# ferdean/lsa-fw

Hardware: AMD Instinct MI355X
Metric: converged eigenpairs/sec (k=20, shift-invert) (higher is better)
Workload: dtype c128

## Files before the change

include/lsa_hip.h:

```cpp
#ifndef LSA_HIP_H
#define LSA_HIP_H

#include <stdint.h>

#ifdef __cplusplus
extern "C" {
#endif

typedef enum { LSA_F64 = 0, LSA_C128 = 1 } lsa_dtype;

typedef enum {
    LSA_OK = 0,
    LSA_ERR_ARG = -1,
    LSA_ERR_HIP = -2,
    LSA_ERR_ZERO_PIVOT = -3,
    LSA_ERR_DIVERGED = -4,
    LSA_ERR_NONFINITE = -5,
    LSA_ERR_TIMEOUT = -6,
    LSA_ERR_COMM = -7,
    LSA_ERR_OOM = -8
} lsa_status;

typedef struct lsa_ctx lsa_ctx;
typedef struct lsa_mat lsa_mat;
typedef struct lsa_vec lsa_vec;
typedef struct lsa_ilu lsa_ilu;
typedef struct lsa_op lsa_op;
typedef struct lsa_krylov lsa_krylov;

typedef struct {
    int64_t op_applies;
    int64_t gmres_iters;
    int64_t spmv_calls;
    int64_t sptrsv_calls;
    double last_rel_res;
    double max_rel_res;
    double seconds_factor;
    double seconds_solve;
    int32_t stagnated_solves;
    int32_t pc_fallback;
    int32_t backward_accepted;
    int32_t analysis_reused;
    int32_t refined_solves;
    int32_t reserved0;
} lsa_stats;

int lsa_ctx_create(int device, lsa_ctx **out);
void lsa_ctx_destroy(lsa_ctx *ctx);
const char *lsa_last_error(const lsa_ctx *ctx);
int lsa_ctx_synchronize(lsa_ctx *ctx);
int lsa_ctx_mem_info(lsa_ctx *ctx, int64_t *free_bytes, int64_t *total_bytes);
const char *lsa_ctx_arch(const lsa_ctx *ctx);

int lsa_vec_create(lsa_ctx *ctx, int64_t n, int dtype, lsa_vec **out);
void lsa_vec_destroy(lsa_vec *v);
int lsa_vec_upload(lsa_ctx *ctx, lsa_vec *v, const void *host);
int lsa_vec_download(lsa_ctx *ctx, const lsa_vec *v, void *host);

int lsa_csr_upload(lsa_ctx *ctx, int32_t n, int64_t nnz, const int32_t *rowptr, const int32_t *col,
                   const void *val, int dtype, lsa_mat **out);
void lsa_mat_destroy(lsa_mat *m);
int lsa_mat_download_values(lsa_ctx *ctx, const lsa_mat *m, void *host_val);
int lsa_csr_axpby(lsa_ctx *ctx, const lsa_mat *A, const lsa_mat *B, const double alpha[2], const double beta[2],
                  int out_dtype, lsa_mat **out);
int lsa_csr_window(lsa_ctx *ctx, const lsa_mat *M, const double *left, const double *right, lsa_mat **out);
int lsa_spmv(lsa_ctx *ctx, const lsa_mat *A, const lsa_vec *x, lsa_vec *y);
int lsa_spmv_transpose(lsa_ctx *ctx, const lsa_mat *A, int conj, const lsa_vec *x, lsa_vec *y);
int lsa_spmv_transpose_batch(lsa_ctx *ctx, int32_t J, const lsa_mat *const *A, int conj, const lsa_vec *const *x, lsa_vec *const *y);
int lsa_spmv_info(lsa_ctx *ctx, const lsa_mat *A, int xdtype, char *kernel, int32_t kernel_len, int64_t *bytes_moved);
int lsa_spmv_time(lsa_ctx *ctx, const lsa_mat *A, const lsa_vec *x, lsa_vec *y, int iters, double *avg_ms);

int lsa_ilu_create(lsa_ctx *ctx, const lsa_mat *C, int levels, double shift_tol, lsa_ilu **out);
void lsa_ilu_destroy(lsa_ilu *pc);
int lsa_ilu_set_algorithm(lsa_ctx *ctx, lsa_ilu *pc, int algo, int32_t block_size);
int lsa_ilu_solve(lsa_ctx *ctx, lsa_ilu *pc, int which, const lsa_vec *b, lsa_vec *x);
int lsa_ilu_solve_time(lsa_ctx *ctx, lsa_ilu *pc, int which, const lsa_vec *b, lsa_vec *x, int iters, double *avg_ms);
int lsa_ilu_info(const lsa_ilu *pc, int64_t *nnz, int32_t *levels_lower, int32_t *levels_upper, int32_t *nshift);
int lsa_ilu_download(lsa_ctx *ctx, const lsa_ilu *pc, int32_t *rowptr, int32_t *col, void *val);

typedef struct lsa_nd_sym lsa_nd_sym;
typedef struct lsa_ndlu lsa_ndlu;
int lsa_nd_analyse(int32_t n, const int32_t *rowptr, const int32_t *col, int32_t leaf_size, const int8_t *constraint, lsa_nd_sym **out);
int lsa_nd_order(int32_t n, const int32_t *rowptr, const int32_t *col, int32_t leaf_size, const int8_t *constraint, lsa_nd_sym **out);
int lsa_nd_analyse_tree(int32_t n, const int32_t *rowptr, const int32_t *col, int32_t ntree, const int32_t *first, const int32_t *size,
                        const int32_t *parent, const int32_t *owner, int32_t rank, int32_t nranks, lsa_nd_sym **out);
const char *lsa_nd_sym_error(const lsa_nd_sym *h);
void lsa_nd_sym_destroy(lsa_nd_sym *h);
int lsa_nd_sym_info(const lsa_nd_sym *h, int32_t *ntree, int32_t *nlevels, int32_t *max_front, int64_t *index_entries,
                    int64_t *factor_entries, int64_t *front_entries, double *flops);
int lsa_nd_sym_memory(const lsa_nd_sym *h, int32_t scalar_bytes, int64_t work_budget_bytes, int64_t *out, int64_t *upd_off, int64_t *work_off,
                      int32_t *chunk_of);
int lsa_nd_sym_export(const lsa_nd_sym *h, int32_t *perm, int32_t *node_start, int32_t *parent, int32_t *level, int32_t *front_size,
                      int32_t *idx);
int lsa_nd_sym_export_tables(const lsa_nd_sym *h, int32_t *cmap, int32_t *gptr, int32_t *gidx, int64_t *asm_dst, int32_t *lvl_ptr,
                             int32_t *lvl_nodes);
int lsa_nd_sym_export_dist(const lsa_nd_sym *h, int32_t *kind, int64_t *front_off, int64_t *u_off, int32_t *asm_src, int32_t *children_ptr,
                           int32_t *children_idx, int64_t *scalars);
int lsa_nd_sym_export_top(const lsa_nd_sym *h, int32_t *owner, int32_t *rows, int64_t *exch, int64_t *totals);
int lsa_ndlu_create(lsa_ctx *ctx, const lsa_mat *C, int32_t leaf_size, lsa_ndlu **out);
int lsa_ndlu_prepare(lsa_ctx *ctx, const lsa_mat *P, int dtype, int32_t leaf_size, const int8_t *constraint);
int lsa_ndlu_prepare_tree(lsa_ctx *ctx, const lsa_mat *P, int dtype, int32_t ntree, const int32_t *first, const int32_t *size,
                          const int32_t *parent);
int lsa_ndlu_create_tree(lsa_ctx *ctx, const lsa_mat *C, int32_t ntree, const int32_t *first, const int32_t *size, const int32_t *parent,
                         const int32_t *owner, lsa_ndlu **out);
int lsa_ndlu_refactor(lsa_ctx *ctx, lsa_ndlu *f, const lsa_mat *C);
void lsa_ndlu_destroy(lsa_ndlu *f);
int lsa_ndlu_solve(lsa_ctx *ctx, lsa_ndlu *f, const lsa_vec *b, lsa_vec *x);
int lsa_ndlu_solve_batch(lsa_ctx *ctx, int32_t J, lsa_ndlu *const *f, const lsa_vec *const *b, lsa_vec *const *x);
int lsa_ndlu_solve_adjoint(lsa_ctx *ctx, lsa_ndlu *f, int conj, const lsa_vec *b, lsa_vec *x);
int lsa_ndlu_solve_batch_adjoint(lsa_ctx *ctx, int32_t J, lsa_ndlu *const *f, int conj, const lsa_vec *const *b, lsa_vec *const *x);
int lsa_ndlu_solve_time(lsa_ctx *ctx, lsa_ndlu *f, const lsa_vec *b, lsa_vec *x, int iters, double *avg_ms);
int lsa_ndlu_solve_multi(lsa_ctx *ctx, lsa_ndlu *f, int trans, int32_t nrhs, const lsa_vec *B, int64_t ldb, lsa_vec *X, int64_t ldx);
int lsa_ndlu_solve_multi_time(lsa_ctx *ctx, lsa_ndlu *f, int trans, int32_t nrhs, const lsa_vec *B, int64_t ldb, lsa_vec *X, int64_t ldx,
                              int iters, double *avg_ms);
int lsa_ndlu_set_multi_transposed(lsa_ctx *ctx, lsa_ndlu *f, int on);
int lsa_ndlu_multi_info(const lsa_ndlu *f, int32_t *width, int64_t *extra_bytes, int32_t *launches_per_pass);
int lsa_ndlu_solve_multi_batch(lsa_ctx *ctx, int32_t J, lsa_ndlu *const *f, int trans, int32_t nrhs, const lsa_vec *const *B, int64_t ldb,
                               lsa_vec *const *X, int64_t ldx);
int lsa_ndlu_solve_multi_batch_time(lsa_ctx *ctx, int32_t J, lsa_ndlu *const *f, int trans, int32_t nrhs, const lsa_vec *const *B,
                                    int64_t ldb, lsa_vec *const *X, int64_t ldx, int iters, double *avg_ms);
int lsa_ndlu_solve_multi_batch_adjoint(lsa_ctx *ctx, int32_t J, lsa_ndlu *const *f, int conj, int32_t nrhs, const lsa_vec *const *B,
                                       int64_t ldb, lsa_vec *const *X, int64_t ldx);
int lsa_ndlu_solve_multi_batch_adjoint_time(lsa_ctx *ctx, int32_t J, lsa_ndlu *const *f, int conj, int32_t nrhs, const lsa_vec *const *B,
                                            int64_t ldb, lsa_vec *const *X, int64_t ldx, int iters, double *avg_ms);
int lsa_ndlu_inertia(lsa_ctx *ctx, lsa_ndlu *f, int64_t *negative, int64_t *zero, int64_t *positive);
int lsa_ndlu_prepared_memory(lsa_ctx *ctx, int64_t *out);
int lsa_ndlu_info(const lsa_ndlu *f, int32_t *ntree, int32_t *nlevels, int32_t *max_front, int64_t *factor_entries,
                  int64_t *front_entries, int64_t *apply_bytes, int32_t *apply_launches, double *seconds_analyse,
                  double *seconds_numeric, int32_t *factor_launches);
int lsa_ndlu_sweep_level(const lsa_ndlu *f, int32_t level, int32_t *nodes, int32_t *max_pivot, int32_t *fwd_rows, int32_t *bwd_rows,
                         int32_t *fwd_tiles, int32_t *bwd_tiles);

int lsa_gmres(lsa_ctx *ctx, const lsa_mat *C, lsa_ilu *pc, const lsa_vec *b, lsa_vec *x, int use_x0, double rtol,
              int restart, int maxit, int32_t *iters, double *rel_res);

typedef struct {
    int32_t ilu_levels;
    double ilu_shift;
    double ksp_rtol;
    int32_t ksp_restart;
    int32_t ksp_maxit;
    int32_t pc_type;
    double antishift[2];
} lsa_op_options;

int lsa_op_create(lsa_ctx *ctx, const lsa_mat *A, const lsa_mat *M, const double sigma[2], int mode,
                  const lsa_op_options *opts, lsa_op **out);
void lsa_op_destroy(lsa_op *op);
int lsa_op_apply(lsa_ctx *ctx, lsa_op *op, const lsa_vec *x, lsa_vec *y);
int lsa_op_stats(const lsa_op *op, lsa_stats *out);
int lsa_op_set_adjoint(lsa_ctx *ctx, lsa_op *op, int on);
int lsa_op_set_projection(lsa_ctx *ctx, lsa_op *op, const double *keep);

int lsa_krylov_create(lsa_ctx *ctx, lsa_op *op, int32_t ncv, lsa_krylov **out);
void lsa_krylov_destroy(lsa_krylov *k);
int lsa_krylov_set_row_permutation(lsa_ctx *ctx, lsa_krylov *k, const int32_t *perm);
int lsa_krylov_set_start(lsa_ctx *ctx, lsa_krylov *k, const void *host_v);
int lsa_krylov_inject(lsa_ctx *ctx, lsa_krylov *k, int32_t j, const void *host_v);
int lsa_krylov_extend(lsa_ctx *ctx, lsa_krylov *k, int32_t j0, int32_t j1, void *H, int32_t ldh, int32_t *breakdown);
int lsa_krylov_restart(lsa_ctx *ctx, lsa_krylov *k, int32_t m, int32_t knew, const void *Q, int32_t ldq);
int lsa_krylov_ritz_vectors(lsa_ctx *ctx, lsa_krylov *k, int32_t m, int32_t nvec, const void *Y, int32_t ldy,
                            int normalise, void *X);
int lsa_krylov_imag_norms(const lsa_krylov *k, int32_t nvec, double *out);
int lsa_eig_residuals(lsa_ctx *ctx, const lsa_mat *A, const lsa_mat *M, int32_t nvec, const void *lam, const void *X,
                      double *res);
int lsa_eig_biorth(lsa_ctx *ctx, const lsa_mat *M, int64_t n, int32_t nvec, const void *X, const void *Z, void *G,
                   double *norm_z, double *norm_mx);

typedef enum {
    LSA_WHICH_LARGEST_MAGNITUDE = 1,
    LSA_WHICH_LARGEST_REAL = 3,
    LSA_WHICH_SMALLEST_REAL = 4,
    LSA_WHICH_LARGEST_IMAGINARY = 5,
    LSA_WHICH_SMALLEST_IMAGINARY = 6,
    LSA_WHICH_TARGET_MAGNITUDE = 7,
    LSA_WHICH_TARGET_REAL = 8,
    LSA_WHICH_TARGET_IMAGINARY = 9
} lsa_which;
typedef struct {
    int32_t nev;
    int32_t max_restarts;
    double tol;
    int32_t which;
    int32_t transform;
    double sigma[2];
    double antishift[2];
    double target[2];
    uint64_t seed;
    double keep_fraction;
} lsa_ks_options;
typedef struct {
    int32_t nconv;
    int32_t nout;
    int32_t restarts;
    int32_t pad;
    int64_t op_applies;
    double next_unconverged;
    double seconds_expand;
    double seconds_dense;
    double seconds_restart;
} lsa_ks_result;
int lsa_krylov_shape(const lsa_krylov *k, int64_t *n, int32_t *ncv);
int64_t lsa_mat_rows(const lsa_mat *m);
int lsa_krylov_solve(lsa_ctx *ctx, lsa_krylov *k, const lsa_ks_options *opts, const void *v0, const double *mask, int32_t max_out,
                     void *theta_out, void *lambda_out, void *X_out, double *est_out, lsa_ks_result *result);
typedef struct {
    int64_t rounds;
    int64_t launches;
    int64_t periods;
    double launches_per_round;
    int64_t lockstep_steps[16];
    int64_t solo_steps[16];
// ... 171 lines not shown
```

lsa-fw_amd/csrc/blas.hip:

```cpp
#include "lsa_internal.h"

namespace {

constexpr int kThreads = 256;
constexpr int kColTile = 8;

template <typename T>
__device__ __forceinline__ T wave_sum(T v);
template <>
__device__ __forceinline__ double wave_sum<double>(double v) {
#pragma unroll
    for (int m = 32; m > 0; m >>= 1) v += __shfl_xor(v, m, 64);
    return v;
}
template <>
__device__ __forceinline__ cplx wave_sum<cplx>(cplx v) {
#pragma unroll
    for (int m = 32; m > 0; m >>= 1) {
        v.re += __shfl_xor(v.re, m, 64);
        v.im += __shfl_xor(v.im, m, 64);
    }
    return v;
}

// ... 354 lines not shown
    }
    T a1, a2, a3;
    if constexpr (sizeof(T) == 16) {
        a1 = cplx{__shfl(acc.re, (lane & 15) + 16), __shfl(acc.im, (lane & 15) + 16)};
        a2 = cplx{__shfl(acc.re, (lane & 15) + 32), __shfl(acc.im, (lane & 15) + 32)};
        a3 = cplx{__shfl(acc.re, (lane & 15) + 48), __shfl(acc.im, (lane & 15) + 48)};
    } else {
        a1 = __shfl(acc, (lane & 15) + 16);
        a2 = __shfl(acc, (lane & 15) + 32);
        a3 = __shfl(acc, (lane & 15) + 48);
    }
    double nrm = 0.0;
    if (q == 0 && i < n) {
        const T tot = s_add(s_add(acc, a1), s_add(a2, a3));
        const T r = s_sub(w_in[i], tot);
        w[i] = r;
        nrm = s_abs2(r);
    }
    if (nrm_part) {
        nrm = wave_sum_dpp(nrm);
        if (lane == 0) wn[wave] = nrm;
        __syncthreads();
        if (threadIdx.x == 0) nrm_part[blockIdx.x] = (wn[0] + wn[1]) + (wn[2] + wn[3]);
    }
}

template <typename T>
__global__ __launch_bounds__(kThreads) void cgs_scale_kernel(int64_t n, const T* __restrict__ x, const double* __restrict__ nrm_part, int nparts,
                                                             T* __restrict__ y, int j, const T* __restrict__ h1, const T* __restrict__ h2,
                                                             T* __restrict__ hout) {
    __shared__ double smem[4];
    __shared__ double tot_s;
    double a = 0.0;
    for (int k = threadIdx.x; k < nparts; k += kThreads) a += nrm_part[k];
    const double t = block_sum<double>(a, smem);
    if (threadIdx.x == 0) tot_s = t;
    __syncthreads();
    const double tot = tot_s;
    if (blockIdx.x == 0) {
        for (int c = threadIdx.x; c < j; c += kThreads) hout[c] = s_add(h1[c], h2[c]);
        if (threadIdx.x == 0) s_from(hout[j], sqrt(tot), 0.0);
    }
    const double s = 1.0 / sqrt(tot);
    const int64_t stride = (int64_t)gridDim.x * blockDim.x;
    for (int64_t i = (int64_t)blockIdx.x * blockDim.x + threadIdx.x; i < n; i += stride) y[i] = s_mul(s, x[i]);
}

__device__ __forceinline__ double parts_sum(const double* __restrict__ nrm_part, int nparts, double* smem ) {
    double a = 0.0;
    for (int k = threadIdx.x; k < nparts; k += kThreads) a += nrm_part[k];
    return block_sum<double>(a, smem);
}

template <typename MT, int LPR, bool DELAYED = false>
__global__ __launch_bounds__(kThreads) void cgs_tail_kernel(int32_t n, const int32_t* __restrict__ rp, const int32_t* __restrict__ ci,
                                                            const MT* __restrict__ mval, const cplx* __restrict__ cval,
                                                            const cplx* __restrict__ w, const cplx* __restrict__ y,
                                                            const double* __restrict__ nrm_part, int nparts, cplx* __restrict__ vnext, cplx* t,
                                                            int j, const cplx* __restrict__ h1, const cplx* __restrict__ h2,
                                                            cplx* __restrict__ hout, double* __restrict__ chk_part) {
    __shared__ double smem[4];
    __shared__ double tot_s;
    __shared__ double csum[4][2];
    double s = 1.0;
    if constexpr (DELAYED) {
        if (blockIdx.x == 0) {
            const double tsum = parts_sum(nrm_part, nparts, smem);
            if (threadIdx.x == 0) s_from(hout[0], sqrt(tsum), 0.0);
        }
    } else {
        const double tsum = parts_sum(nrm_part, nparts, smem);
        if (threadIdx.x == 0) tot_s = tsum;
        __syncthreads();
        const double tot = tot_s;
        if (blockIdx.x == 0) {
            for (int c = threadIdx.x; c < j; c += kThreads) hout[c] = s_add(h1[c], h2[c]);
            if (threadIdx.x == 0) s_from(hout[j], sqrt(tot), 0.0);
        }
        s = 1.0 / sqrt(tot);
    }
    const int64_t gid = (int64_t)blockIdx.x * blockDim.x + threadIdx.x;
    const int32_t lane = (int32_t)(gid % LPR);
    const int64_t row_stride = ((int64_t)gridDim.x * blockDim.x) / LPR;
    double rw = 0.0, rb = 0.0;
    for (int64_t row = gid / LPR; row < n; row += row_stride) {
        const int32_t p0 = rp[row], p1 = rp[row + 1];
        cplx am = cplx{0.0, 0.0}, ac = cplx{0.0, 0.0};
        for (int32_t p = p0 + lane; p < p1; p += 3 * LPR) {
            int32_t c[3];
            MT vm[3];
            cplx vc[3], xw[3], xy[3];
#pragma unroll
            for (int u = 0; u < 3; ++u) {
                const bool in = p + u * LPR < p1;
                c[u] = in ? ci[p + u * LPR] : 0;
                vm[u] = in ? mval[p + u * LPR] : scalar_traits<MT>::zero();
                vc[u] = in ? cval[p + u * LPR] : cplx{0.0, 0.0};
            }
#pragma unroll
            for (int u = 0; u < 3; ++u) {
                const bool in = p + u * LPR < p1;
                xw[u] = in ? w[c[u]] : cplx{0.0, 0.0};
                xy[u] = in ? y[c[u]] : cplx{0.0, 0.0};
            }
#pragma unroll
            for (int u = 0; u < 3; ++u)
                if (p + u * LPR < p1) {
                    if constexpr (DELAYED) fma_acc(am, vm[u], xw[u]);
                    else fma_acc(am, vm[u], s_mul(s, xw[u]));
                    fma_acc(ac, vc[u], xy[u]);
                }
        }
#pragma unroll
        for (int m = LPR / 2; m > 0; m >>= 1) {
            am = s_add(am, cplx{__shfl_xor(am.re, m, 64), __shfl_xor(am.im, m, 64)});
            ac = s_add(ac, cplx{__shfl_xor(ac.re, m, 64), __shfl_xor(ac.im, m, 64)});
        }
        if (lane == 0) {
            const cplx told = t[row];
            rw += s_abs2(s_sub(told, ac));
            rb += s_abs2(told);
            t[row] = am;
            if constexpr (!DELAYED) vnext[row] = s_mul(s, w[row]);
        }
    }
    rw = wave_sum_dpp(rw);
    rb = wave_sum_dpp(rb);
    const int wave = threadIdx.x >> 6;
    if ((threadIdx.x & 63) == 0) {
        csum[wave][0] = rw;
        csum[wave][1] = rb;
    }
    __syncthreads();
    if (threadIdx.x < 2) chk_part[2 * blockIdx.x + threadIdx.x] = (csum[0][threadIdx.x] + csum[1][threadIdx.x]) + (csum[2][threadIdx.x] + csum[3][threadIdx.x]);
}

struct DcgsBatchArgs {
    cplx* V[kKrylovGroupMax];
    const cplx* y[kKrylovGroupMax];
    cplx* part[kKrylovGroupMax];
    cplx* slot[kKrylovGroupMax];
    double* nrm_part[kKrylovGroupMax];
    int32_t j[kKrylovGroupMax];
    int32_t first[kKrylovGroupMax];
};
struct TailBatchArgs {
    const int32_t* rp[kKrylovGroupMax];
    const int32_t* ci[kKrylovGroupMax];
    const void* mval[kKrylovGroupMax];
    const cplx* cval[kKrylovGroupMax];
    const cplx* w[kKrylovGroupMax];
    const cplx* y[kKrylovGroupMax];
    const double* nrm_part[kKrylovGroupMax];
    cplx* t[kKrylovGroupMax];
    cplx* hout[kKrylovGroupMax];
    double* chk_part[kKrylovGroupMax];
};

template <typename MT, int LPR>
__global__ __launch_bounds__(kThreads) void cgs_tail_batch_kernel(int32_t n, int nparts, TailBatchArgs a) {
    __shared__ double smem[4];
    __shared__ double csum[4][2];
    const int z = blockIdx.z;
    const int32_t* __restrict__ rp = a.rp[z];
    const int32_t* __restrict__ ci = a.ci[z];
    const MT* __restrict__ mval = (const MT*)a.mval[z];
    const cplx* __restrict__ cval = a.cval[z];
    const cplx* __restrict__ w = a.w[z];
    const cplx* __restrict__ y = a.y[z];
    cplx* t = a.t[z];
    if (blockIdx.x == 0) {
        const double tsum = parts_sum(a.nrm_part[z], nparts, smem);
        if (threadIdx.x == 0) s_from(a.hout[z][0], sqrt(tsum), 0.0);
    }
    const int64_t gid = (int64_t)blockIdx.x * blockDim.x + threadIdx.x;
    const int32_t lane = (int32_t)(gid % LPR);
    const int64_t row_stride = ((int64_t)gridDim.x * blockDim.x) / LPR;
    double rw = 0.0, rb = 0.0;
    for (int64_t row = gid / LPR; row < n; row += row_stride) {
        const int32_t p0 = rp[row], p1 = rp[row + 1];
        cplx am = cplx{0.0, 0.0}, ac = cplx{0.0, 0.0};
        for (int32_t p = p0 + lane; p < p1; p += 3 * LPR) {
            int32_t c[3];
            MT vm[3];
            cplx vc[3], xw[3], xy[3];
#pragma unroll
            for (int u = 0; u < 3; ++u) {
                const bool in = p + u * LPR < p1;
                c[u] = in ? ci[p + u * LPR] : 0;
                vm[u] = in ? mval[p + u * LPR] : scalar_traits<MT>::zero();
                vc[u] = in ? cval[p + u * LPR] : cplx{0.0, 0.0};
            }
#pragma unroll
            for (int u = 0; u < 3; ++u) {
                const bool in = p + u * LPR < p1;
                xw[u] = in ? w[c[u]] : cplx{0.0, 0.0};
                xy[u] = in ? y[c[u]] : cplx{0.0, 0.0};
            }
#pragma unroll
            for (int u = 0; u < 3; ++u)
                if (p + u * LPR < p1) {
                    fma_acc(am, vm[u], xw[u]);
                    fma_acc(ac, vc[u], xy[u]);
                }
        }
#pragma unroll
        for (int m = LPR / 2; m > 0; m >>= 1) {
            am = s_add(am, cplx{__shfl_xor(am.re, m, 64), __shfl_xor(am.im, m, 64)});
            ac = s_add(ac, cplx{__shfl_xor(ac.re, m, 64), __shfl_xor(ac.im, m, 64)});
        }
        if (lane == 0) {
            const cplx told = t[row];
            rw += s_abs2(s_sub(told, ac));
            rb += s_abs2(told);
            t[row] = am;
        }
    }
    rw = wave_sum_dpp(rw);
    rb = wave_sum_dpp(rb);
    const int wave = threadIdx.x >> 6;
    if ((threadIdx.x & 63) == 0) {
        csum[wave][0] = rw;
        csum[wave][1] = rb;
    }
    __syncthreads();
    if (threadIdx.x < 2) a.chk_part[z][2 * blockIdx.x + threadIdx.x] = (csum[0][threadIdx.x] + csum[1][threadIdx.x]) + (csum[2][threadIdx.x] + csum[3][threadIdx.x]);
}

__global__ __launch_bounds__(kThreads) void cgs_tail_checks_kernel(int nparts, const double* __restrict__ parts, double* __restrict__ checks) {
    __shared__ double smem[4];
    const double* p = parts + (size_t)blockIdx.x * 2 * (size_t)nparts;
    double a = 0.0, b = 0.0;
    for (int k = threadIdx.x; k < nparts; k += kThreads) {
        a += p[2 * k];
        b += p[2 * k + 1];
    }
    const double sa = block_sum<double>(a, smem);
    const double sb = block_sum<double>(b, smem);
    if (threadIdx.x == 0) {
        checks[2 * blockIdx.x] = sa;
        checks[2 * blockIdx.x + 1] = sb;
    }
}

template <bool Y>
__device__ __forceinline__ void dcgs_dot_body(const int bx, const int by, int64_t n, int jc, int64_t rows_per_block, const cplx* __restrict__ V,
                                              int64_t ldv, const cplx* __restrict__ y, cplx* __restrict__ part, int ldp,
                                              const cplx* __restrict__ chk_b, const cplx* __restrict__ chk_z, double* __restrict__ chk_part) {
    __shared__ cplx wsum[4][2 * kColTile];
    __shared__ double dsm[4][2];
    const cplx* __restrict__ p = V + (int64_t)(jc - 1) * ldv;
    const int chunk = bx;
    const int c0 = by * kColTile;
    const int wave = threadIdx.x >> 6, lane = threadIdx.x & 63;
    const int64_t r0 = (int64_t)chunk * rows_per_block;
    const int64_t r1 = (r0 + rows_per_block < n) ? r0 + rows_per_block : n;
    cplx ap[kColTile], ay[kColTile];
#pragma unroll
    for (int c = 0; c < kColTile; ++c) ap[c] = ay[c] = cplx{0.0, 0.0};
    const int nc = (jc - c0 < kColTile) ? (jc - c0) : kColTile;
    if (nc == kColTile) {
        int64_t i = r0 + threadIdx.x;
        for (; i + kThreads < r1; i += 2 * kThreads) {
// ... 703 lines not shown
    static size_t head_bytes(size_t esz) { return 2 * part_bytes(esz) + 2 * esz * kFuseCols + sizeof(double) * 2 * kFuseChunks; }
    FusedWork(void* work, size_t esz) {
        char* p = (char*)work;
        part1 = p;
        part2 = p + part_bytes(esz);
        h1 = p + 2 * part_bytes(esz);
        h2 = p + 2 * part_bytes(esz) + esz * kFuseCols;
        nrm_part = (double*)(p + head_bytes(esz));
        chk_part = nrm_part - 2 * kFuseChunks;
    }
};

size_t k_cgs2_fused_work_bytes(lsa_ctx* ctx, int64_t n, int jmax) {
    (void)ctx;
    (void)jmax;
    return FusedWork::head_bytes(16) + sizeof(double) * (size_t)((n + 63) / 64 + 8);
}

static bool cgs2_fused_shape(int64_t n, int j, int64_t* rpb_out) {
    if (j <= 0 || j > kFuseCols || n <= 0) return false;
    int64_t rpb = (n + kFuseChunks - 1) / kFuseChunks;
    rpb = ((rpb + kThreads - 1) / kThreads) * kThreads;
    if (rpb < 1024) rpb = 1024;
    if (rpb > 4096) return false;
    if (rpb_out) *rpb_out = rpb;
    return true;
}

int k_cgs2_fused(lsa_ctx* ctx, int dtype, int64_t n, int j, const void* V, int64_t ldv, void* w, void* vnext, void* hcol_dev, void* work,
                 const void* chk_b, const void* chk_z, double* chk_out) {
    int64_t rpb = 0;
    if (!cgs2_fused_shape(n, j, &rpb)) return 1;
    const int nchunks = (int)((n + rpb - 1) / rpb);
    const int blocks = (int)((n + 63) / 64);
    const FusedWork fw(work, dtype == LSA_C128 ? 16 : 8);
    void *part1 = fw.part1, *part2 = fw.part2, *h1 = fw.h1, *h2 = fw.h2;
    double *chk_part = fw.chk_part, *nrm_part = fw.nrm_part;
    const dim3 dgrid(nchunks, (j + kColTile - 1) / kColTile);
    DISPATCH_T(dtype, {
        hipLaunchKernelGGL((cgs_dot_kernel<T>), dgrid, dim3(kThreads), 0, ctx->stream, n, j, rpb, (const T*)V, ldv, (const T*)w, (T*)part1, kFuseCols,
                           (const T*)chk_b, (const T*)chk_z, chk_out ? chk_part : (double*)nullptr);
        hipLaunchKernelGGL((cgs_axpy_kernel<T>), dim3(blocks), dim3(kThreads), 0, ctx->stream, n, j, (const T*)V, ldv, (const T*)part1, nchunks, kFuseCols,
                           (const T*)w, (T*)w, (T*)h1, (double*)nullptr, (const double*)chk_part, chk_out);
        hipLaunchKernelGGL((cgs_dot_kernel<T>), dgrid, dim3(kThreads), 0, ctx->stream, n, j, rpb, (const T*)V, ldv, (const T*)w, (T*)part2, kFuseCols,
                           (const T*)nullptr, (const T*)nullptr, (double*)nullptr);
        hipLaunchKernelGGL((cgs_axpy_kernel<T>), dim3(blocks), dim3(kThreads), 0, ctx->stream, n, j, (const T*)V, ldv, (const T*)part2, nchunks, kFuseCols,
                           (const T*)w, (T*)w, (T*)h2, nrm_part, (const double*)nullptr, (double*)nullptr);
        hipLaunchKernelGGL((cgs_scale_kernel<T>), dim3(stream_blocks(ctx, n)), dim3(kThreads), 0, ctx->stream, n, (const T*)w, (const double*)nrm_part, blocks, (T*)vnext,
                           j, (const T*)h1, (const T*)h2, (T*)hcol_dev);
    });
    return check_launch(ctx, "cgs2_fused");
}

bool k_cgs2_tail_fits(lsa_ctx* ctx, int64_t n, int jmax, const lsa_mat* M, const lsa_mat* C) {
    (void)ctx;
    if (!M || !C || !cgs2_fused_shape(n, jmax, nullptr)) return false;
    if (C->dtype != LSA_C128 || M->n != n || C->n != n || M->ncols != n || C->ncols != n || M->row0 != 0 || C->row0 != 0) return false;
    const bool same_dev = M->rp == C->rp && M->ci == C->ci;
    const bool same_host = M->h_rp.size() > 0 && M->h_rp.same_object(C->h_rp) && M->h_ci.same_object(C->h_ci);
    if (M->nnz != C->nnz || !(same_dev || same_host)) return false;
    return k_spmv_plain_subwave_lanes(M) == 16 && k_spmv_plain_subwave_lanes(C) == 16;
}

int k_cgs2_tail_parts(int64_t n) { return (int)((n * 16 + kThreads - 1) / kThreads); }

int k_cgs2_fused_tail(lsa_ctx* ctx, int64_t n, int j, const void* V, int64_t ldv, const void* y, void* w, void* vnext, void* hcol_dev, void* work,
                      const lsa_mat* M, const lsa_mat* C, void* t, double* tail_part) {
    typedef cplx T;
    int64_t rpb = 0;
    if (!cgs2_fused_shape(n, j, &rpb)) return lsa_set_error(ctx, LSA_ERR_ARG, "k_cgs2_fused_tail: shape outside the fused form");
    const int nchunks = (int)((n + rpb - 1) / rpb);
    const int blocks = (int)((n + 63) / 64);
    const FusedWork fw(work, 16);
    void *part1 = fw.part1, *part2 = fw.part2, *h1 = fw.h1, *h2 = fw.h2;
    double* nrm_part = fw.nrm_part;
    const dim3 dgrid(nchunks, (j + kColTile - 1) / kColTile);
    hipLaunchKernelGGL((cgs_dot_kernel<T>), dgrid, dim3(kThreads), 0, ctx->stream, n, j, rpb, (const T*)V, ldv, (const T*)y, (T*)part1, kFuseCols,
                       (const T*)nullptr, (const T*)nullptr, (double*)nullptr);
    hipLaunchKernelGGL((cgs_axpy_kernel<T>), dim3(blocks), dim3(kThreads), 0, ctx->stream, n, j, (const T*)V, ldv, (const T*)part1, nchunks, kFuseCols,
                       (const T*)y, (T*)w, (T*)h1, (double*)nullptr, (const double*)nullptr, (double*)nullptr);
    hipLaunchKernelGGL((cgs_dot_kernel<T>), dgrid, dim3(kThreads), 0, ctx->stream, n, j, rpb, (const T*)V, ldv, (const T*)w, (T*)part2, kFuseCols,
                       (const T*)nullptr, (const T*)nullptr, (double*)nullptr);
    hipLaunchKernelGGL((cgs_axpy_kernel<T>), dim3(blocks), dim3(kThreads), 0, ctx->stream, n, j, (const T*)V, ldv, (const T*)part2, nchunks, kFuseCols,
                       (const T*)w, (T*)w, (T*)h2, nrm_part, (const double*)nullptr, (double*)nullptr);
    const int tparts = k_cgs2_tail_parts(n);
    if (M->dtype == LSA_C128)
        hipLaunchKernelGGL((cgs_tail_kernel<cplx, 16>), dim3(tparts), dim3(kThreads), 0, ctx->stream, (int32_t)n, C->rp, C->ci, (const cplx*)M->val,
                           (const cplx*)C->val, (const T*)w, (const T*)y, (const double*)nrm_part, blocks, (T*)vnext, (T*)t, j, (const T*)h1, (const T*)h2,
                           (T*)hcol_dev, tail_part);
    else
        hipLaunchKernelGGL((cgs_tail_kernel<double, 16>), dim3(tparts), dim3(kThreads), 0, ctx->stream, (int32_t)n, C->rp, C->ci, (const double*)M->val,
                           (const cplx*)C->val, (const T*)w, (const T*)y, (const double*)nrm_part, blocks, (T*)vnext, (T*)t, j, (const T*)h1, (const T*)h2,
                           (T*)hcol_dev, tail_part);
    return check_launch(ctx, "cgs2_fused_tail");
}

int k_cgs2_tail_checks(lsa_ctx* ctx, int nslots, int nparts, const double* tail_parts, double* checks) {
    if (nslots <= 0) return LSA_OK;
    hipLaunchKernelGGL(cgs_tail_checks_kernel, dim3(nslots), dim3(kThreads), 0, ctx->stream, nparts, tail_parts, checks);
    return check_launch(ctx, "cgs2_tail_checks");
}

bool k_dcgs2_fits(int64_t n, int ncv) { return cgs2_fused_shape(n, ncv + 1, nullptr); }

int k_dcgs2_step(lsa_ctx* ctx, int64_t n, int j, void* V, int64_t ldv, const void* y, int first, void* slot, int lds, void* work,
                 const void* chk_b, const void* chk_z, double* chk_out) {
    int64_t rpb = 0;
    if (!cgs2_fused_shape(n, j + 1, &rpb) || j < 0 || j + 1 > lds + 1 || (first && !y))
        return lsa_set_error(ctx, LSA_ERR_ARG, "k_dcgs2_step: shape outside the fused form");
    const int nchunks = (int)((n + rpb - 1) / rpb);
    const int blocks = (int)((n + 63) / 64);
    const FusedWork fw(work, 16);
    cplx* part = (cplx*)fw.part1;
    double *chk_part = fw.chk_part, *nrm_part = fw.nrm_part;
    const dim3 dgrid(nchunks, (j + 1 + kColTile - 1) / kColTile);
    const int ldp = 2 * kFuseCols;
    if (y) {
        hipLaunchKernelGGL((dcgs_dot_kernel<true>), dgrid, dim3(kThreads), 0, ctx->stream, n, j + 1, rpb, (const cplx*)V, ldv, (const cplx*)y, part, ldp,
                           (const cplx*)chk_b, (const cplx*)chk_z, chk_out ? chk_part : (double*)nullptr);
        hipLaunchKernelGGL((dcgs_update_kernel<true>), dim3(blocks), dim3(kThreads), 0, ctx->stream, n, j, (cplx*)V, ldv, (const cplx*)part, nchunks, ldp,
                           (const cplx*)y, first, nrm_part, (cplx*)slot, lds, (const double*)chk_part, chk_out);
    } else {
        hipLaunchKernelGGL((dcgs_dot_kernel<false>), dgrid, dim3(kThreads), 0, ctx->stream, n, j + 1, rpb, (const cplx*)V, ldv, (const cplx*)nullptr, part,
                           ldp, (const cplx*)nullptr, (const cplx*)nullptr, (double*)nullptr);
        hipLaunchKernelGGL((dcgs_update_kernel<false>), dim3(blocks), dim3(kThreads), 0, ctx->stream, n, j, (cplx*)V, ldv, (const cplx*)part, nchunks, ldp,
                           (const cplx*)nullptr, 0, (double*)nullptr, (cplx*)slot, lds, (const double*)nullptr, (double*)nullptr);
    }
    return check_launch(ctx, "dcgs2_step");
}

int k_dcgs2_norm(lsa_ctx* ctx, int64_t n, void* work, void* slot, int lds) {
    double* nrm_part = FusedWork(work, 16).nrm_part;
    hipLaunchKernelGGL(dcgs_norm_kernel, dim3(1), dim3(kThreads), 0, ctx->stream, (const double*)nrm_part, (int)((n + 63) / 64),
                       (cplx*)slot + 2 * (size_t)lds + 2);
    return check_launch(ctx, "dcgs2_norm");
}

int k_dcgs2_tail(lsa_ctx* ctx, int64_t n, int j, const void* V, int64_t ldv, const void* y, void* work, const lsa_mat* M, const lsa_mat* C, void* t,
                 double* tail_part, void* slot, int lds) {
    const int blocks = (int)((n + 63) / 64);
    double* nrm_part = FusedWork(work, 16).nrm_part;
    const cplx* w = (const cplx*)V + (size_t)(j + 1) * (size_t)ldv;
    cplx* nout = (cplx*)slot + 2 * (size_t)lds + 2;
    const int tparts = k_cgs2_tail_parts(n);
    if (M->dtype == LSA_C128)
        hipLaunchKernelGGL((cgs_tail_kernel<cplx, 16, true>), dim3(tparts), dim3(kThreads), 0, ctx->stream, (int32_t)n, C->rp, C->ci, (const cplx*)M->val,
                           (const cplx*)C->val, w, (const cplx*)y, (const double*)nrm_part, blocks, (cplx*)nullptr, (cplx*)t, 0, (const cplx*)nullptr,
                           (const cplx*)nullptr, nout, tail_part);
    else
        hipLaunchKernelGGL((cgs_tail_kernel<double, 16, true>), dim3(tparts), dim3(kThreads), 0, ctx->stream, (int32_t)n, C->rp, C->ci,
                           (const double*)M->val, (const cplx*)C->val, w, (const cplx*)y, (const double*)nrm_part, blocks, (cplx*)nullptr, (cplx*)t, 0,
                           (const cplx*)nullptr, (const cplx*)nullptr, nout, tail_part);
    return check_launch(ctx, "dcgs2_tail");
}

int k_dcgs2_step_batch(lsa_ctx* ctx, int J, int64_t n, const int32_t* j, void* const* V, int64_t ldv, const void* const* y, const int32_t* first,
                       void* const* slot, int lds, void* const* work) {
    if (J < 1 || J > kKrylovGroupMax) return lsa_set_error(ctx, LSA_ERR_ARG, "k_dcgs2_step_batch: J = %d outside [1, %d]", J, kKrylovGroupMax);
    int64_t rpb = 0;
    int jmax = 0;
    DcgsBatchArgs a;
    memset(&a, 0, sizeof a);
    for (int z = 0; z < J; ++z) {
        if (j[z] < 0 || j[z] + 1 > lds + 1 || !cgs2_fused_shape(n, j[z] + 1, &rpb) || !y[z])
            return lsa_set_error(ctx, LSA_ERR_ARG, "k_dcgs2_step_batch: shape outside the fused form (problem %d)", z);
        jmax = std::max(jmax, (int)j[z]);
        const FusedWork fw(work[z], 16);
        a.V[z] = (cplx*)V[z];
        a.y[z] = (const cplx*)y[z];
        a.part[z] = (cplx*)fw.part1;
        a.slot[z] = (cplx*)slot[z];
        a.nrm_part[z] = fw.nrm_part;
        a.j[z] = j[z];
        a.first[z] = first[z];
    }
    const int nchunks = (int)((n + rpb - 1) / rpb);
    const int blocks = (int)((n + 63) / 64);
    const int ldp = 2 * kFuseCols;
    hipLaunchKernelGGL(dcgs_dot_batch_kernel, dim3(nchunks, (jmax + 1 + kColTile - 1) / kColTile, J), dim3(kThreads), 0, ctx->stream, n, rpb, ldv, ldp, a);
    hipLaunchKernelGGL(dcgs_update_batch_kernel, dim3(blocks, 1, J), dim3(kThreads), 0, ctx->stream, n, ldv, nchunks, ldp, lds, a);
    return check_launch(ctx, "dcgs2_step_batch");
}

int k_dcgs2_tail_batch(lsa_ctx* ctx, int J, int64_t n, const int32_t* j, void* const* V, int64_t ldv, const void* const* y, void* const* work,
                       const lsa_mat* const* M, const lsa_mat* const* C, void* const* t, double* const* tail_part, void* const* slot, int lds) {
    if (J < 1 || J > kKrylovGroupMax) return lsa_set_error(ctx, LSA_ERR_ARG, "k_dcgs2_tail_batch: J = %d outside [1, %d]", J, kKrylovGroupMax);
    TailBatchArgs a;
    memset(&a, 0, sizeof a);
    for (int z = 0; z < J; ++z) {
        if (M[z]->dtype != M[0]->dtype) return lsa_set_error(ctx, LSA_ERR_ARG, "k_dcgs2_tail_batch: real and complex M in one round (problem %d)", z);
        a.rp[z] = C[z]->rp;
        a.ci[z] = C[z]->ci;
        a.mval[z] = M[z]->val;
        a.cval[z] = (const cplx*)C[z]->val;
        a.w[z] = (const cplx*)V[z] + (size_t)(j[z] + 1) * (size_t)ldv;
        a.y[z] = (const cplx*)y[z];
        a.nrm_part[z] = FusedWork(work[z], 16).nrm_part;
        a.t[z] = (cplx*)t[z];
        a.hout[z] = (cplx*)slot[z] + 2 * (size_t)lds + 2;
        a.chk_part[z] = tail_part[z];
    }
    const int blocks = (int)((n + 63) / 64);
    const dim3 grid(k_cgs2_tail_parts(n), 1, J);
    if (M[0]->dtype == LSA_C128) hipLaunchKernelGGL((cgs_tail_batch_kernel<cplx, 16>), grid, dim3(kThreads), 0, ctx->stream, (int32_t)n, blocks, a);
    else hipLaunchKernelGGL((cgs_tail_batch_kernel<double, 16>), grid, dim3(kThreads), 0, ctx->stream, (int32_t)n, blocks, a);
    return check_launch(ctx, "dcgs2_tail_batch");
}
```

lsa-fw_amd/csrc/core.hip:

```cpp
#include <algorithm>
#include <cmath>

#include "lsa_internal.h"

int lsa_set_error(lsa_ctx* ctx, int code, const char* fmt, ...) {
    char buf[1024];
    va_list ap;
    va_start(ap, fmt);
    vsnprintf(buf, sizeof buf, fmt, ap);
    va_end(ap);
    if (ctx) ctx->err = buf;
    return code;
}

void lsa_name_problem(lsa_ctx* ctx, int32_t z) {
    if (ctx) ctx->err = "problem " + std::to_string(z) + ": " + ctx->err;
}

int lsa_ensure_scratch(lsa_ctx* ctx, size_t dbytes, size_t hbytes) {
    if (dbytes > ctx->dscratch_bytes) {
        LSA_HIP_CHECK(ctx, hipStreamSynchronize(ctx->stream));
        if (ctx->dscratch) (void)hipFree(ctx->dscratch);
        ctx->dscratch = nullptr;
        ctx->dscratch_bytes = 0;
// ... 163 lines not shown
    m->nnz = nnz;
    m->dtype = dtype;
    m->owns_index = true;
    m->rp = nullptr;
    m->ci = nullptr;
    m->val = nullptr;
    m->h_rp.assign(rowptr, rowptr + n_local + 1);
    m->h_ci.assign(col, col + nnz);
    size_t vb = (size_t)(nnz > 0 ? nnz : 1) * dtype_size(dtype);
    hipError_t e1 = hipMalloc(&m->rp, sizeof(int32_t) * (size_t)(n_local + 1));
    hipError_t e2 = hipMalloc(&m->ci, sizeof(int32_t) * (size_t)(nnz > 0 ? nnz : 1));
    hipError_t e3 = hipMalloc(&m->val, vb);
    if (e1 != hipSuccess || e2 != hipSuccess || e3 != hipSuccess) {
        lsa_mat_destroy(m);
        return lsa_set_error(ctx, LSA_ERR_HIP, "hipMalloc(CSR n=%d nnz=%lld) failed", n_local, (long long)nnz);
    }
    hipError_t e = hipMemcpyAsync(m->rp, rowptr, sizeof(int32_t) * (size_t)(n_local + 1), hipMemcpyHostToDevice, ctx->stream);
    if (e == hipSuccess && nnz > 0) e = hipMemcpyAsync(m->ci, col, sizeof(int32_t) * (size_t)nnz, hipMemcpyHostToDevice, ctx->stream);
    if (e == hipSuccess && nnz > 0) e = hipMemcpyAsync(m->val, val, (size_t)nnz * dtype_size(dtype), hipMemcpyHostToDevice, ctx->stream);
    if (e == hipSuccess) e = hipStreamSynchronize(ctx->stream);
    if (e != hipSuccess) {
        lsa_mat_destroy(m);
        return lsa_set_error(ctx, LSA_ERR_HIP, "CSR upload failed: %s", hipGetErrorString(e));
    }
    *out = m;
    return LSA_OK;
}

int lsa_csr_upload(lsa_ctx* ctx, int32_t n, int64_t nnz, const int32_t* rowptr, const int32_t* col, const void* val,
                   int dtype, lsa_mat** out) {
    return csr_upload_impl(ctx, n, n, 0, nnz, rowptr, col, val, dtype, out);
}

int lsa_csr_upload_shard(lsa_ctx* ctx, int32_t n_global, int32_t row0, int32_t row1, int64_t nnz_local,
                         const int32_t* rowptr_local, const int32_t* col, const void* val, int dtype, lsa_mat** out) {
    if (row0 < 0 || row1 < row0 || row1 > n_global) return lsa_set_error(ctx, LSA_ERR_ARG, "lsa_csr_upload_shard: bad row range");
    return csr_upload_impl(ctx, row1 - row0, n_global, row0, nnz_local, rowptr_local, col, val, dtype, out);
}

int64_t lsa_mat_rows(const lsa_mat* m) { return m ? (int64_t)m->n : 0; }

void lsa_mat_destroy(lsa_mat* m) {
    if (!m) return;
    if (m->ctx && m->ctx->stream) (void)hipStreamSynchronize(m->ctx->stream);
    if (m->owns_index) {
        if (m->rp) (void)hipFree(m->rp);
        if (m->ci) (void)hipFree(m->ci);
    }
    if (m->val && m->owns_values) (void)hipFree(m->val);
    if (!m->owns_extras) m->ci16 = nullptr, m->cbase = nullptr, m->grp_start = nullptr;
    if (m->grp_start) (void)hipFree(m->grp_start);
    if (m->ci16) (void)hipFree(m->ci16);
    if (m->cbase) (void)hipFree(m->cbase);
    delete m;
}

int lsa_mat_download_values(lsa_ctx* ctx, const lsa_mat* m, void* host_val) {
    if (!ctx || !m || !host_val) return lsa_set_error(ctx, LSA_ERR_ARG, "lsa_mat_download_values: null argument");
    LSA_HIP_CHECK(ctx, hipMemcpyAsync(host_val, m->val, (size_t)m->nnz * dtype_size(m->dtype), hipMemcpyDeviceToHost, ctx->stream));
    LSA_HIP_CHECK(ctx, hipStreamSynchronize(ctx->stream));
    return LSA_OK;
}

}

template <typename TA, typename TB, typename TC>
__global__ void axpby_kernel(int64_t nnz, const TA* __restrict__ a, const TB* __restrict__ b, cplx alpha, cplx beta,
                             TC* __restrict__ c) {
    int64_t stride = (int64_t)gridDim.x * blockDim.x;
    for (int64_t p = (int64_t)blockIdx.x * blockDim.x + threadIdx.x; p < nnz; p += stride) {
        cplx acc{0.0, 0.0};
        fma_acc(acc, alpha, to_cplx(a[p]));
        fma_acc(acc, beta, to_cplx(b[p]));
        s_from(c[p], acc.re, acc.im);
    }
}

template <typename TA, typename TB, typename TC>
static void launch_axpby(lsa_ctx* ctx, int64_t nnz, const void* a, const void* b, cplx alpha, cplx beta, void* c) {
    int threads = 256;
    int64_t want = (nnz + threads - 1) / threads;
    int blocks = (int)(want < 1 ? 1 : (want > 4096 ? 4096 : want));
    hipLaunchKernelGGL((axpby_kernel<TA, TB, TC>), dim3(blocks), dim3(threads), 0, ctx->stream, nnz, (const TA*)a, (const TB*)b,
                       alpha, beta, (TC*)c);
}

extern "C" int lsa_csr_axpby(lsa_ctx* ctx, const lsa_mat* A, const lsa_mat* B, const double alpha[2], const double beta[2],
                             int out_dtype, lsa_mat** out) {
    if (!ctx || !A || !B || !alpha || !beta || !out) return lsa_set_error(ctx, LSA_ERR_ARG, "lsa_csr_axpby: null argument");
    if (A->n != B->n || A->nnz != B->nnz || A->ncols != B->ncols || A->row0 != B->row0)
        return lsa_set_error(ctx, LSA_ERR_ARG, "lsa_csr_axpby: operands must share one sparsity pattern (n %d vs %d, nnz %lld vs %lld)",
                             A->n, B->n, (long long)A->nnz, (long long)B->nnz);
    if (!A->h_rp.same_object(B->h_rp) || !A->h_ci.same_object(B->h_ci)) {
        if (A->h_rp != B->h_rp || A->h_ci != B->h_ci)
            return lsa_set_error(ctx, LSA_ERR_ARG, "lsa_csr_axpby: operands must share one sparsity pattern (index arrays differ)");
        B->h_rp = A->h_rp;
        B->h_ci = A->h_ci;
        if (!A->h_hash) A->h_hash = B->h_hash ? B->h_hash : std::make_shared<uint64_t>(0);
        B->h_hash = A->h_hash;
        if (!A->h_shared) A->h_shared = B->h_shared ? B->h_shared : std::make_shared<PatternShared>();
        B->h_shared = A->h_shared;
    }
    if (out_dtype == LSA_F64 && (A->dtype != LSA_F64 || B->dtype != LSA_F64 || alpha[1] != 0.0 || beta[1] != 0.0))
        return lsa_set_error(ctx, LSA_ERR_ARG, "lsa_csr_axpby: a real result needs real operands and real coefficients");
    lsa_mat* C = new lsa_mat();
    C->ctx = ctx;
// ... 53 lines not shown
extern "C" int lsa_csr_window(lsa_ctx* ctx, const lsa_mat* M, const double* left, const double* right, lsa_mat** out) {
    if (!ctx || !M || !left || !out) return lsa_set_error(ctx, LSA_ERR_ARG, "lsa_csr_window: null argument");
    if (M->dtype != LSA_F64) return lsa_set_error(ctx, LSA_ERR_ARG, "lsa_csr_window: the matrix is complex: a window weighs a real symmetric matrix");
    if (M->row0 != 0 || M->n != M->ncols || !M->owns_values)
        return lsa_set_error(ctx, LSA_ERR_ARG, "lsa_csr_window: the matrix is a shard or a row view (%d rows of %d from row %d): whole square matrices only",
                             M->n, M->ncols, M->row0);
    const int32_t n = M->n;
    for (const double* v : {left, right})
        for (int32_t i = 0; v && i < n; ++i)
            if (!std::isfinite(v[i]))
                return lsa_set_error(ctx, LSA_ERR_ARG, "lsa_csr_window: %s[%d] = %.3e is not finite", v == left ? "left" : "right", i, v[i]);
    lsa_mat* W = new lsa_mat();
    W->ctx = ctx;
    W->n = n;
    W->ncols = M->ncols;
    W->row0 = 0;
    W->nnz = M->nnz;
    W->dtype = LSA_F64;
    W->rp = M->rp;
    W->ci = M->ci;
    W->owns_index = false;
    W->h_rp = M->h_rp;
    W->h_ci = M->h_ci;
    if (!M->h_hash) M->h_hash = std::make_shared<uint64_t>(0);
    W->h_hash = M->h_hash;
    if (!M->h_shared) M->h_shared = std::make_shared<PatternShared>();
    W->h_shared = M->h_shared;
    W->val = nullptr;
    spmv_share_extras(M, W);
    double* dwin = nullptr;
    const size_t wb = (size_t)std::max(n, 1) * sizeof(double);
    hipError_t e = hipMalloc(&W->val, (size_t)(W->nnz > 0 ? W->nnz : 1) * sizeof(double));
    if (e == hipSuccess) e = hipMalloc((void**)&dwin, 2 * wb);
    if (e == hipSuccess && n > 0) e = hipMemcpyAsync(dwin, left, (size_t)n * sizeof(double), hipMemcpyHostToDevice, ctx->stream);
    if (e == hipSuccess && n > 0) e = hipMemcpyAsync(dwin + n, right ? right : left, (size_t)n * sizeof(double), hipMemcpyHostToDevice, ctx->stream);
    if (e == hipSuccess && n > 0 && W->nnz > 0) {
        const int threads = 256;
        const int64_t want = ((int64_t)n * kWindowLanes + threads - 1) / threads;
        const int blocks = (int)(want < 1 ? 1 : (want > 4096 ? 4096 : want));
        hipLaunchKernelGGL(window_values_kernel, dim3(blocks), dim3(threads), 0, ctx->stream, n, M->rp, M->ci, (const double*)M->val, (const double*)dwin,
                           (const double*)(dwin + n), (double*)W->val);
        e = hipGetLastError();
    }
    if (e == hipSuccess) e = hipStreamSynchronize(ctx->stream);
    if (dwin) (void)hipFree(dwin);
    if (e != hipSuccess) {
        (void)hipGetLastError();
        lsa_mat_destroy(W);
        return lsa_set_error(ctx, e == hipErrorOutOfMemory ? LSA_ERR_OOM : LSA_ERR_HIP, "lsa_csr_window: %s", hipGetErrorString(e));
    }
    *out = W;
    return LSA_OK;
}
```

lsa-fw_amd/csrc/lsa_internal.h:

```cpp
#pragma once

#include <hip/hip_runtime.h>

#include <algorithm>
#include <cmath>
#include <cstdarg>
#include <cstdint>
#include <cstdio>
#include <cstdlib>
#include <cstring>
#include <memory>
#include <string>
#include <vector>

#include "../../include/lsa_hip.h"

struct cplx {
    double re, im;
};
static_assert(sizeof(cplx) == 16, "complex128 layout");

__host__ __device__ inline cplx make_cplx(double r, double i) { return cplx{r, i}; }

template <typename T>
// ... 95 lines not shown
};

struct SharedInts {
    std::shared_ptr<const std::vector<int32_t>> p;
    const int32_t* data() const { return p ? p->data() : nullptr; }
    size_t size() const { return p ? p->size() : 0; }
    const int32_t& operator[](size_t i) const { return (*p)[i]; }
    const std::vector<int32_t>& vec() const {
        static const std::vector<int32_t> none;
        return p ? *p : none;
    }
    void assign(const int32_t* b, const int32_t* e) { p = std::make_shared<const std::vector<int32_t>>(b, e); }
    bool same_object(const SharedInts& o) const { return p == o.p; }
    bool operator==(const SharedInts& o) const { return p == o.p || vec() == o.vec(); }
    bool operator!=(const SharedInts& o) const { return !(*this == o); }
};

struct TransposeIndex {
    int32_t *rp = nullptr, *ci = nullptr, *src = nullptr;
    int32_t ncols = 0;
    int64_t nnz = 0;
    ~TransposeIndex() {
        for (void* p : {(void*)rp, (void*)ci, (void*)src})
            if (p) (void)hipFree(p);
    }
};

struct PatternShared {
    std::shared_ptr<TransposeIndex> tr;
};

struct lsa_mat {
    lsa_ctx* ctx;
    int32_t n;
    int32_t ncols;
    int32_t row0;
    int64_t nnz;
    int dtype;
    int32_t* rp;
    int32_t* ci;
    void* val;
    bool owns_index;
    bool owns_values = true;
    mutable SharedInts h_rp, h_ci;
    mutable std::shared_ptr<uint64_t> h_hash;
    mutable std::shared_ptr<PatternShared> h_shared;
    mutable uint16_t* ci16 = nullptr;
    mutable int32_t* cbase = nullptr;
    mutable int ci16_state = 0;
    mutable int32_t* grp_start = nullptr;
    mutable int32_t ngroups = 0;
    mutable int grp_state = 0;
    bool owns_extras = true;
};

int lsa_set_error(lsa_ctx* ctx, int code, const char* fmt, ...);
lsa_mat* mat_row_view(const lsa_mat* full, int32_t r0, int32_t r1);
void comm_release(lsa_ctx* ctx);
int k_agree_status(lsa_ctx* ctx, int rc);
int k_agree_min_i64(lsa_ctx* ctx, int64_t* value);
int k_agree_in_step(lsa_ctx* ctx, const char* where);
int lsa_ensure_scratch(lsa_ctx* ctx, size_t dbytes, size_t hbytes);
inline bool env_flag(const char* name, bool dflt) {
    const char* e = getenv(name);
    return e ? atoi(e) != 0 : dflt;
}
inline int lsa_check_launch(lsa_ctx* ctx, const char* what) {
    const hipError_t e = hipGetLastError();
    if (e != hipSuccess) return lsa_set_error(ctx, LSA_ERR_HIP, "%s: kernel launch failed: %s", what, hipGetErrorString(e));
    return LSA_OK;
}
constexpr int kDotMaxChunks = 2048;
inline int dot_chunks(int64_t n, int64_t* rows_per_chunk) {
    int64_t rows = ((n + kDotMaxChunks - 1) / kDotMaxChunks + 255) / 256 * 256;
    rows = std::max<int64_t>(rows, 512);
    *rows_per_chunk = rows;
    return (int)std::max<int64_t>((n + rows - 1) / rows, 1);
}

#define LSA_HIP_CHECK(ctx, expr)                                                                         \
    do {                                                                                                 \
        hipError_t _e = (expr);                                                                          \
        if (_e != hipSuccess)                                                                            \
            return lsa_set_error((ctx), LSA_ERR_HIP, "%s failed: %s (%s:%d)", #expr, hipGetErrorString(_e), \
                                 __FILE__, __LINE__);                                                    \
    } while (0)

#define LSA_HIP_ALLOC(ctx, expr)                                                                                    \
    do {                                                                                                            \
        hipError_t _e = (expr);                                                                                     \
        if (_e != hipSuccess) {                                                                                     \
            (void)hipGetLastError();                                                                                \
            return lsa_set_error((ctx), _e == hipErrorOutOfMemory ? LSA_ERR_OOM : LSA_ERR_HIP, "%s failed: %s (%s:%d)", #expr, \
                                 hipGetErrorString(_e), __FILE__, __LINE__);                                        \
        }                                                                                                           \
    } while (0)

#define LSA_CHECK(expr)            \
    do {                           \
        int _rc = (expr);          \
        if (_rc != LSA_OK) return _rc; \
    } while (0)

template <typename F>
int lsa_time_runs(lsa_ctx* ctx, bool warm, int iters, double* avg_ms, F&& run) {
    if (warm) LSA_CHECK(run());
    LSA_HIP_CHECK(ctx, hipEventRecord(ctx->ev0, ctx->stream));
    for (int i = 0; i < iters; ++i) LSA_CHECK(run());
    LSA_HIP_CHECK(ctx, hipEventRecord(ctx->ev1, ctx->stream));
    LSA_HIP_CHECK(ctx, hipEventSynchronize(ctx->ev1));
    float ms = 0.f;
    LSA_HIP_CHECK(ctx, hipEventElapsedTime(&ms, ctx->ev0, ctx->ev1));
    *avg_ms = (double)ms / iters;
    return LSA_OK;
}

constexpr int kKrylovGroupMax = 16;


int k_spmv(lsa_ctx* ctx, const lsa_mat* A, int xdtype, const void* x, void* y);
int k_spmv_transpose(lsa_ctx* ctx, const lsa_mat* A, int conj, int xdtype, const void* x, void* y);
int k_transpose_index(lsa_ctx* ctx, const lsa_mat* A, const TransposeIndex** out);
int k_spmv_transpose_batch(lsa_ctx* ctx, int32_t J, const lsa_mat* const* mats, int conj, int xdtype, const void* const* xs, void* const* ys);
void spmv_share_extras(const lsa_mat* from, lsa_mat* to);

int k_spmm(lsa_ctx* ctx, const lsa_mat* A, int32_t ncols, const void* X, int64_t ldx, void* Y, int64_t ldy);
int k_spmm_transpose(lsa_ctx* ctx, const lsa_mat* A, int conj, int32_t ncols, const void* X, int64_t ldx, void* Y, int64_t ldy);
int k_block_gram(lsa_ctx* ctx, int64_t n, int32_t p, const void* U, int64_t ldu, int32_t q, const void* W, int64_t ldw, void* G_host);

bool dense_lu_solve(int32_t r, void* Mh, void* Ah);

int k_copy(lsa_ctx* ctx, int dtype, int64_t n, const void* x, void* y);
int k_set_zero(lsa_ctx* ctx, int dtype, int64_t n, void* x);
int k_axpy(lsa_ctx* ctx, int dtype, int64_t n, const double alpha[2], const void* x, void* y);
int k_multi_dot(lsa_ctx* ctx, int dtype, int64_t n, int j, const void* V, int64_t ldv, const void* w, void* h_dev);
int k_multi_axpy_dot(lsa_ctx* ctx, int dtype, int64_t n, int j, const void* V, int64_t ldv, const void* h1_dev, void* w, void* h2_dev);
int k_multi_axpy(lsa_ctx* ctx, int dtype, int64_t n, int j, const void* V, int64_t ldv, const void* h_dev, void* w,
                 double* nrm2_dev);
int k_columns_canonical(lsa_ctx* ctx, int64_t n, int ncols, void* X, int64_t ldx, int unit, double* imag2_dev);
int k_nrm2(lsa_ctx* ctx, int dtype, int64_t n, const void* x, double* nrm2_dev);
int k_pair_nrm2(lsa_ctx* ctx, int dtype, int64_t n, const void* x, const void* y, double* nrm2_dev);
int k_mask(lsa_ctx* ctx, int dtype, int64_t n, const double* keep_dev, void* y);
int k_residual_norms(lsa_ctx* ctx, int dtype, int64_t n, const void* b, const void* z, void* w, double* nrm2_dev);
int k_scale_by_inv_norm(lsa_ctx* ctx, int dtype, int64_t n, const void* x, const double* nrm2_dev, void* y);
int k_hess_column(lsa_ctx* ctx, int dtype, int j, const void* h1, const void* h2, const double* nrm2_dev, void* hout);
size_t k_cgs2_fused_work_bytes(lsa_ctx* ctx, int64_t n, int jmax);
int k_cgs2_fused(lsa_ctx* ctx, int dtype, int64_t n, int j, const void* V, int64_t ldv, void* w, void* vnext, void* hcol_dev, void* work,
                 const void* chk_b, const void* chk_z, double* chk_out);
bool k_cgs2_tail_fits(lsa_ctx* ctx, int64_t n, int jmax, const lsa_mat* M, const lsa_mat* C);
int k_cgs2_tail_parts(int64_t n);
int k_cgs2_fused_tail(lsa_ctx* ctx, int64_t n, int j, const void* V, int64_t ldv, const void* y, void* w, void* vnext, void* hcol_dev, void* work,
                      const lsa_mat* M, const lsa_mat* C, void* t, double* tail_part);
int k_cgs2_tail_checks(lsa_ctx* ctx, int nslots, int nparts, const double* tail_parts, double* checks);
bool k_dcgs2_fits(int64_t n, int ncv);
int k_dcgs2_step(lsa_ctx* ctx, int64_t n, int j, void* V, int64_t ldv, const void* y, int first, void* slot, int lds, void* work,
                 const void* chk_b, const void* chk_z, double* chk_out);
int k_dcgs2_norm(lsa_ctx* ctx, int64_t n, void* work, void* slot, int lds);
int k_dcgs2_tail(lsa_ctx* ctx, int64_t n, int j, const void* V, int64_t ldv, const void* y, void* work, const lsa_mat* M, const lsa_mat* C, void* t,
                 double* tail_part, void* slot, int lds);
int k_dcgs2_step_batch(lsa_ctx* ctx, int J, int64_t n, const int32_t* j, void* const* V, int64_t ldv, const void* const* y, const int32_t* first,
                       void* const* slot, int lds, void* const* work);
int k_dcgs2_tail_batch(lsa_ctx* ctx, int J, int64_t n, const int32_t* j, void* const* V, int64_t ldv, const void* const* y, void* const* work,
                       const lsa_mat* const* M, const lsa_mat* const* C, void* const* t, double* const* tail_part, void* const* slot, int lds);
int k_spmv_plain_subwave_lanes(const lsa_mat* A);
int k_basis_gemm_max_cols(int dtype);
int k_basis_gemm(lsa_ctx* ctx, int dtype, int64_t n, int m, int k, const void* V, int64_t ldv, const void* Q, int ldq,
                 void* Out, int64_t ldo);
int k_scatter_rows(lsa_ctx* ctx, int dtype, int64_t n, int ncols, const int32_t* perm, const void* In, void* Out);

int basis_upload_row_permutation(lsa_ctx* ctx, const char* who, int64_t n, const int32_t* perm, int32_t** row_perm);
int basis_times_host_matrix(lsa_ctx* ctx, int dtype, int64_t n, int m, int k, const void* V, const void* Q, int ldq, void* qdev, void* Out,
                            size_t pinned_extra);
int basis_columns_to_host(lsa_ctx* ctx, int dtype, int64_t n, int ncols, const int32_t* row_perm, const void* dev, void** xtmp, int xtmp_cols, void* host);
int direct_solve_enqueue(lsa_ctx* ctx, lsa_op* op, int dtype, const void* rhs, void* y, void* z, void* r, bool refine, double* norms,
                         int direction = -1);
void stats_book_direct_solve(lsa_stats* st, int products, bool refine, double res, double bnorm);

void krylov_arm_preapply(lsa_krylov* k, bool on);
int krylov_preapply(lsa_ctx* ctx, lsa_krylov* k, int32_t m);
int krylov_restart_queued(lsa_ctx* ctx, lsa_krylov* k, int32_t m, int32_t knew, const void* Q, int32_t ldq);

struct KrylovGroupBuf {
    int32_t J, slots, nparts;
    void* Hdev;
    double *checks, *tail_parts;
};
int krylov_group_check(lsa_ctx* ctx, int32_t J, lsa_krylov* const* ks);
int krylov_group_alloc(lsa_ctx* ctx, int32_t J, lsa_krylov* const* ks, KrylovGroupBuf* gb);
void krylov_group_free(KrylovGroupBuf* gb);
int krylov_extend_batch(lsa_ctx* ctx, KrylovGroupBuf* gb, lsa_krylov* const* ks, const uint8_t* active, const int32_t* j0, int32_t j1, void* const* Hs,
                        int32_t ldh, int32_t* breakdown, int32_t* status, std::string* errs, lsa_ks_batch_info* info);
void lsa_name_problem(lsa_ctx* ctx, int32_t z);

struct lsa_ndlu;
struct lsa_op_parts {
    int64_t n;
    const lsa_mat *Kmul, *Kfac;
    lsa_ndlu* nd;
    bool plain;
    bool shift_invert, adjoint, projected, one_rank;
    double ksp_rtol;
    double normF;
    double sigma[2];
    bool* refine;
    lsa_stats* st;
};
int lsa_op_get_parts(lsa_op* op, lsa_op_parts* out);
inline int direct_solve_verdict(double ksp_rtol, double normF, bool refine, double res, double bnorm, double xnorm, bool* backward) {
    *backward = refine && res > ksp_rtol * bnorm && normF > 0.0 && res <= 1e-12 * normF * xnorm;
    if (res <= ksp_rtol * bnorm || *backward) return 0;
    return (!refine && std::isfinite(res)) ? 1 : -1;
}
// ... 84 lines not shown
```

lsa-fw_amd/csrc/solver.hip:

```cpp
#include <algorithm>
#include <chrono>
#include <cmath>
#include <complex>

#include "ndlu_internal.h"

int ilu_check_abort(lsa_ctx* ctx, lsa_ilu* pc);

namespace {

using zc = std::complex<double>;

struct KrylovSwitches {
    bool fused;
    bool four_passes;
    bool tail;
    bool delayed;
    bool timing;
    bool preapply;
};
const KrylovSwitches& krylov_switches() {
    static const KrylovSwitches sw = [] {
        const char* passes = getenv("LSA_KRYLOV_PASSES");
        return KrylovSwitches{env_flag("LSA_KRYLOV_FUSED", true), passes && atoi(passes) == 4, env_flag("LSA_KRYLOV_TAIL", true),
                              env_flag("LSA_KRYLOV_DELAYED", true), getenv("LSA_KRYLOV_TIMING") != nullptr, env_flag("LSA_KRYLOV_PREAPPLY", true)};
    }();
    return sw;
}

struct OrthWork {
    void *h1 = nullptr, *h2 = nullptr, *hcol = nullptr;
    double* nrm2 = nullptr;
    void* fused = nullptr;
    int cap = 0;
    int ensure_fused(lsa_ctx* ctx, int64_t n) {
        if (fused) return LSA_OK;
        LSA_HIP_ALLOC(ctx, hipMalloc(&fused, k_cgs2_fused_work_bytes(ctx, n, cap)));
        return LSA_OK;
    }
    int alloc(lsa_ctx* ctx, int cap_, int dtype) {
        cap = cap_;
        const size_t b = (size_t)(cap + 2) * esize(dtype);
        LSA_HIP_CHECK(ctx, hipMalloc(&h1, b));
        LSA_HIP_CHECK(ctx, hipMalloc(&h2, b));
        LSA_HIP_CHECK(ctx, hipMalloc(&hcol, b));
        LSA_HIP_CHECK(ctx, hipMalloc((void**)&nrm2, 4 * sizeof(double)));
        return LSA_OK;
    }
    void release() {
        for (void* p : {h1, h2, hcol, (void*)nrm2, fused})
            if (p) (void)hipFree(p);
        h1 = h2 = hcol = fused = nullptr;
        nrm2 = nullptr;
    }
};

struct SolveCheck {
    const void *b, *z;
    void* r;
    double* out;
};

int orthonormalize_enqueue(lsa_ctx* ctx, int dtype, int64_t n, const void* V, int64_t ldv, int j, void* w, void* vnext, OrthWork& ow,
                           void* hcol_dev, const SolveCheck* chk = nullptr) {
    const KrylovSwitches& sw = krylov_switches();
    if (sw.fused) {
        LSA_CHECK(ow.ensure_fused(ctx, n));
        const int frc = k_cgs2_fused(ctx, dtype, n, j, V, ldv, w, vnext, hcol_dev, ow.fused, chk ? chk->b : nullptr, chk ? chk->z : nullptr,
                                     chk ? chk->out : nullptr);
        if (frc <= 0) return frc;
    }
    if (chk) LSA_CHECK(k_residual_norms(ctx, dtype, n, chk->b, chk->z, chk->r, chk->out));
    LSA_CHECK(k_multi_dot(ctx, dtype, n, j, V, ldv, w, ow.h1));
    const int arc = sw.four_passes ? 1 : k_multi_axpy_dot(ctx, dtype, n, j, V, ldv, ow.h1, w, ow.h2);
    if (arc < 0) return arc;
    if (arc > 0) {
        LSA_CHECK(k_multi_axpy(ctx, dtype, n, j, V, ldv, ow.h1, w, nullptr));
        LSA_CHECK(k_multi_dot(ctx, dtype, n, j, V, ldv, w, ow.h2));
// ... 289 lines not shown
    if (!converged)
        return lsa_set_error(ctx, LSA_ERR_DIVERGED, "GMRES did not reach rtol %.1e in %d iterations (relative residual %.3e)", rtol,
                             total, relres);
    return LSA_OK;
}

template <typename T>
__global__ void shift_diag_kernel(int32_t n, int32_t row0, const int32_t* __restrict__ rp, const int32_t* __restrict__ ci,
                                  T* __restrict__ val, cplx shift, int32_t* __restrict__ missing) {
    const int64_t stride = (int64_t)gridDim.x * blockDim.x;
    for (int64_t i = (int64_t)blockIdx.x * blockDim.x + threadIdx.x; i < n; i += stride) {
        const int32_t target = (int32_t)i + row0;
        int32_t lo = rp[i], hi = rp[i + 1];
        while (lo < hi) {
            const int32_t mid = (lo + hi) >> 1;
            if (ci[mid] < target) lo = mid + 1;
            else hi = mid;
        }
        if (lo < rp[i + 1] && ci[lo] == target) {
            cplx v = to_cplx(val[lo]);
            s_from(val[lo], v.re - shift.re, v.im - shift.im);
        } else {
            atomicAdd(missing, 1);
        }
    }
}

}

static_assert(sizeof(lsa_op_options) == 56, "lsa_op_options layout is part of the C-ABI (tests/test_abi.py)");

struct TreeArg {
    int32_t nt;
    const int32_t *first, *size, *parent, *owner;
    int32_t row0, row1;
};

struct lsa_op {
    lsa_ctx* ctx;
    int64_t n;
    const lsa_mat* Kmul;
    const lsa_mat* Kfac;
    lsa_mat* owned;
    lsa_mat* owned_mul = nullptr;
    lsa_mat* owned_diag;
    lsa_ilu* pc;
    lsa_ndlu* nd = nullptr;
    bool nd_dist = false;
    bool adjoint = false;
    double normF = 0.0;
    double sigma[2] = {0.0, 0.0};
    lsa_mat *view_fac = nullptr, *view_mul = nullptr;
    const lsa_mat* M_whole = nullptr;
    lsa_op_options opts;
    GmresWork gw;
    bool gw_ready;
    void* t;
    double* keep = nullptr;
    bool refine = false;
    lsa_stats st;
};

static PcRef pc_of(const lsa_op* op) {
    PcRef pc;
    pc.ilu = op->pc;
    pc.nd = op->nd;
    pc.nd_dist = op->nd_dist;
    pc.adjoint = op->adjoint;
    pc.normF = op->normF;
    return pc;
}

struct lsa_krylov {
    lsa_ctx* ctx;
    lsa_op* op;
    int64_t n;
    int32_t ncv;
    int32_t* row_perm = nullptr;
    void *V, *V2, *w, *qdev;
    OrthWork ow;
    std::vector<zc> hcol;
    double* imag2 = nullptr;
    void* xtmp = nullptr;
    std::vector<double> imag_norms;
    void* Hdev = nullptr;
    double* checks = nullptr;
    int32_t batch = 0;
    bool pipeline = false;
    void* w2 = nullptr;
    double* tail_parts = nullptr;
    int32_t tail_nparts = 0;
    int32_t t_for = -1;
    bool pre_armed = false;
    int32_t pre_col = -1, pre_for = -1;
    const lsa_op* pre_op = nullptr;
    void drop_preapply() { pre_col = pre_for = -1; }
    hipEvent_t ev_read[2] = {nullptr, nullptr};
    int ensure_events(lsa_ctx* ctx_) {
        for (hipEvent_t& e : ev_read)
            if (!e) LSA_HIP_CHECK(ctx_, hipEventCreateWithFlags(&e, hipEventDisableTiming));
        return LSA_OK;
    }
};

static size_t krylov_slot_bytes(int32_t ncv) { return (size_t)(2 * ncv + 4) * 16; }

static void krylov_free(lsa_krylov* k) {
    for (void* p : {k->V, k->V2, k->w, k->qdev, k->Hdev, (void*)k->checks, (void*)k->imag2, k->xtmp, (void*)k->row_perm, k->w2, (void*)k->tail_parts})
        if (p) (void)hipFree(p);
    for (hipEvent_t e : k->ev_read)
        if (e) (void)hipEventDestroy(e);
    k->ow.release();
    delete k;
}

extern "C" {

int lsa_gmres(lsa_ctx* ctx, const lsa_mat* C, lsa_ilu* pc, const lsa_vec* b, lsa_vec* x, int use_x0, double rtol, int restart,
              int maxit, int32_t* iters, double* rel_res) {
    if (!ctx || !C || !b || !x) return lsa_set_error(ctx, LSA_ERR_ARG, "lsa_gmres: null argument");
    if (C->n != C->ncols || b->n != C->n || x->n != C->n || b->dtype != x->dtype)
        return lsa_set_error(ctx, LSA_ERR_ARG, "lsa_gmres: shape/dtype mismatch");
    if (C->dtype == LSA_C128 && b->dtype != LSA_C128) return lsa_set_error(ctx, LSA_ERR_ARG, "lsa_gmres: complex matrix needs complex vectors");
    if (restart < 1 || maxit < 1 || !(rtol > 0.0)) return lsa_set_error(ctx, LSA_ERR_ARG, "lsa_gmres: restart, maxit, rtol must be positive");
    restart = std::min(restart, maxit);
    if (restart > k_basis_gemm_max_cols(b->dtype))
        return lsa_set_error(ctx, LSA_ERR_ARG, "lsa_gmres: restart=%d, the basis product handles at most %d basis vectors", restart, k_basis_gemm_max_cols(b->dtype));
    GmresWork W;
    int rc = W.alloc(ctx, C->n, restart, b->dtype);
    PcRef pcr;
    pcr.ilu = pc;
    if (rc == LSA_OK) rc = gmres_run(ctx, C, pcr, b->dtype, b->d, x->d, use_x0 != 0, rtol, maxit, W, iters, rel_res, nullptr);
    (void)hipStreamSynchronize(ctx->stream);
    W.release();
    return rc;
}

static int build_shifted(lsa_ctx* ctx, const lsa_mat* A, const lsa_mat* M, const double sigma[2], bool cdt, lsa_mat** out) {
    const bool zshift = sigma[0] == 0.0 && sigma[1] == 0.0;
    const double one[2] = {1.0, 0.0}, ms[2] = {-sigma[0], -sigma[1]}, zero[2] = {0.0, 0.0};
    lsa_mat* C = nullptr;
    int rc;
    if (M) rc = lsa_csr_axpby(ctx, A, M, one, ms, cdt ? LSA_C128 : LSA_F64, &C);
    else {
        rc = lsa_csr_axpby(ctx, A, A, one, zero, cdt ? LSA_C128 : LSA_F64, &C);
        if (rc == LSA_OK && !zshift) {
            int32_t* miss = (int32_t*)ctx->dscratch;
            (void)hipMemsetAsync(miss, 0, sizeof(int32_t), ctx->stream);
            const int blocks = std::max(1, std::min((int)((C->n + 255) / 256), ctx->num_cu * 8));
            if (cdt) hipLaunchKernelGGL((shift_diag_kernel<cplx>), dim3(blocks), dim3(256), 0, ctx->stream, C->n, C->row0, C->rp, C->ci, (cplx*)C->val, cplx{sigma[0], sigma[1]}, miss);
            else hipLaunchKernelGGL((shift_diag_kernel<double>), dim3(blocks), dim3(256), 0, ctx->stream, C->n, C->row0, C->rp, C->ci, (double*)C->val, cplx{sigma[0], sigma[1]}, miss);
            int32_t hm = 0;
            (void)hipMemcpyAsync(&hm, miss, sizeof hm, hipMemcpyDeviceToHost, ctx->stream);
            if (hipStreamSynchronize(ctx->stream) != hipSuccess) rc = lsa_set_error(ctx, LSA_ERR_HIP, "diagonal shift failed");
            else if (hm != 0) rc = lsa_set_error(ctx, LSA_ERR_ARG, "A - sigma*I needs a structurally present diagonal (%d rows have none)", hm);
        }
    }
    if (rc != LSA_OK) {
        if (C) lsa_mat_destroy(C);
        return rc;
    }
    *out = C;
    return LSA_OK;
}

static int op_build(lsa_ctx* ctx, const lsa_mat* A, const lsa_mat* M, const lsa_mat* Ad, const lsa_mat* Md, const double sigma[2],
                    int mode, const lsa_op_options* opts, lsa_op** out, const TreeArg* tree = nullptr) {
    if (!ctx || !A || !sigma || !opts || !out) return lsa_set_error(ctx, LSA_ERR_ARG, "lsa_op_create: null argument");
    const bool sharded = Ad != nullptr;
    if (tree) {
        const int nr = std::max(1, ctx->nranks);
        if (sharded || A->n != A->ncols || A->row0 != 0 || (mode != 0 && mode != 2) || opts->pc_type != 2)
            return lsa_set_error(ctx, LSA_ERR_ARG, "lsa_op_create_dist: needs the whole square matrices, a factorising mode (0 or 2) and pc_type 2");
        if (A->ncols % nr != 0 || tree->row0 != (int64_t)ctx->rank * (A->ncols / nr) || tree->row1 < tree->row0 || tree->row1 > tree->row0 + A->ncols / nr)
            return lsa_set_error(ctx, LSA_ERR_ARG, "lsa_op_create_dist: this rank's rows do not sit on its block of the padded layout");
    }
    if (!sharded && A->n != A->ncols) return lsa_set_error(ctx, LSA_ERR_ARG, "lsa_op_create: A must be square (got %d x %d)", A->n, A->ncols);
    if (M && (M->n != A->n || M->ncols != A->ncols || M->row0 != A->row0)) return lsa_set_error(ctx, LSA_ERR_ARG, "lsa_op_create: M does not match A's shape");
    if (mode < 0 || mode > 2) return lsa_set_error(ctx, LSA_ERR_ARG, "lsa_op_create: mode must be 0 (sinvert), 1 (shift) or 2 (Cayley)");
    if (sharded) {
        if (Ad->n != Ad->ncols || Ad->n != A->n || (Md && (Md->n != Ad->n || Md->ncols != Ad->ncols)) || (M != nullptr) != (Md != nullptr))
            return lsa_set_error(ctx, LSA_ERR_ARG, "lsa_op_create_sharded: diagonal blocks must be square with the shard's row count");
        if (A->ncols % std::max(1, ctx->nranks) != 0 || A->row0 != (int64_t)ctx->rank * (A->ncols / std::max(1, ctx->nranks)))
            return lsa_set_error(ctx, LSA_ERR_ARG, "lsa_op_create_sharded: shard does not sit on this rank's block of the padded layout");
        if (A->n > A->ncols / std::max(1, ctx->nranks)) return lsa_set_error(ctx, LSA_ERR_ARG, "lsa_op_create_sharded: shard larger than its padded block");
    }
    const double t0 = now_s();
    lsa_op* op = new lsa_op();
    op->ctx = ctx;
    op->n = A->ncols;
    op->Kmul = op->Kfac = nullptr;
    op->owned = op->owned_diag = nullptr;
    op->pc = nullptr;
    op->opts = *opts;
    op->sigma[0] = sigma[0];
    op->sigma[1] = sigma[1];
    op->gw_ready = false;
    op->t = nullptr;
    memset(&op->st, 0, sizeof op->st);
    const bool zshift = sigma[0] == 0.0 && sigma[1] == 0.0;
    const bool cdt = sigma[1] != 0.0 || A->dtype == LSA_C128 || (M && M->dtype == LSA_C128);
    int rc = LSA_OK;
    lsa_mat* C = nullptr;
    if (!(mode == 1 && zshift)) {
        rc = build_shifted(ctx, A, M, sigma, cdt, &C);
        if (rc != LSA_OK) {
            delete op;
            return rc;
        }
        op->owned = C;
    }
    const lsa_mat* fac_src = nullptr;
    if (mode == 0 || mode == 2) {
        op->Kfac = C;
        op->Kmul = M;
        op->M_whole = M;
        bool shard_rows = false;
        if (tree) {
            const char* e = getenv("LSA_DIST_SPMV");
            shard_rows = (e && *e) ? (e[0] == 's') : (C->nnz > 60 * (int64_t)C->n);
        }
        if (tree && shard_rows) {
            op->view_fac = mat_row_view(C, tree->row0, tree->row1);
            op->Kfac = op->view_fac;
            if (M) {
                op->view_mul = mat_row_view(M, tree->row0, tree->row1);
                op->Kmul = op->view_mul;
            }
        }
        if (mode == 2) {
            const double mnu[2] = {-opts->antishift[0], -opts->antishift[1]};
            const bool cmul = cdt || opts->antishift[1] != 0.0;
            rc = build_shifted(ctx, A, M, mnu, cmul, &op->owned_mul);
            if (rc != LSA_OK) {
                lsa_op_destroy(op);
                return rc;
            }
            if (tree && shard_rows) {
                if (op->view_mul) lsa_mat_destroy(op->view_mul);
                op->view_mul = mat_row_view(op->owned_mul, tree->row0, tree->row1);
                op->Kmul = op->view_mul;
            } else op->Kmul = op->owned_mul;
        }
        if (sharded) {
            rc = build_shifted(ctx, Ad, Md, sigma, cdt, &op->owned_diag);
            if (rc != LSA_OK) {
                lsa_op_destroy(op);
                return rc;
            }
            fac_src = op->owned_diag;
        } else fac_src = C;
    } else {
        op->Kmul = C ? C : A;
        op->Kfac = M;
        fac_src = sharded ? Md : M;
    }
    bool lu_fell_back = false;
    if (opts->pc_type == 3) {
        lsa_op_destroy(op);
        return lsa_set_error(ctx, LSA_ERR_ARG, "lsa_op_create: pc_type 3 (the banded block LU of round 1) left the product library; it lives on as a "
                                               "cross-check library for the tests (tests/xcheck).  Use pc_type 2, the nested-dissection LU");
    }
    if (op->Kfac && fac_src && opts->pc_type == 2) {
        if (tree) {
            rc = lsa_ndlu_create_tree(ctx, fac_src, tree->nt, tree->first, tree->size, tree->parent, tree->owner, &op->nd);
            op->nd_dist = rc == LSA_OK;
            if (rc == LSA_ERR_OOM) {
                lsa_op_destroy(op);
                return rc;
// ... 314 lines not shown

int lsa_krylov_set_row_permutation(lsa_ctx* ctx, lsa_krylov* k, const int32_t* perm) {
    if (!ctx || !k) return lsa_set_error(ctx, LSA_ERR_ARG, "lsa_krylov_set_row_permutation: null argument");
    return basis_upload_row_permutation(ctx, "lsa_krylov_set_row_permutation", k->n, perm, &k->row_perm);
}

int lsa_krylov_set_start(lsa_ctx* ctx, lsa_krylov* k, const void* host_v) {
    if (!ctx || !k || !host_v) return lsa_set_error(ctx, LSA_ERR_ARG, "lsa_krylov_set_start: null argument");
    k->pre_armed = false;
    k->drop_preapply();
    LSA_HIP_CHECK(ctx, hipMemcpyAsync(k->w, host_v, (size_t)k->n * 16, hipMemcpyHostToDevice, ctx->stream));
    double nrm = 0.0;
    LSA_CHECK(device_norm(ctx, LSA_C128, k->n, k->w, k->ow.nrm2, &nrm));
    if (!(nrm > 0.0) || !std::isfinite(nrm)) return lsa_set_error(ctx, LSA_ERR_ARG, "lsa_krylov_set_start: start vector is zero or not finite");
    LSA_CHECK(k_scale_by_inv_norm(ctx, LSA_C128, k->n, k->w, k->ow.nrm2, k->V));
    LSA_HIP_CHECK(ctx, hipStreamSynchronize(ctx->stream));
    k->pipeline = true;
    return LSA_OK;
}

int lsa_krylov_inject(lsa_ctx* ctx, lsa_krylov* k, int32_t j, const void* host_v) {
    if (!ctx || !k || !host_v) return lsa_set_error(ctx, LSA_ERR_ARG, "lsa_krylov_inject: null argument");
    if (j < 0 || j > k->ncv) return lsa_set_error(ctx, LSA_ERR_ARG, "lsa_krylov_inject: index %d out of range", j);
    if (j == 0) return lsa_krylov_set_start(ctx, k, host_v);
    k->drop_preapply();
    const size_t vb = (size_t)k->n * 16;
    LSA_HIP_CHECK(ctx, hipMemcpyAsync(k->w, host_v, vb, hipMemcpyHostToDevice, ctx->stream));
    LSA_CHECK(orthonormalize(ctx, LSA_C128, k->n, k->V, k->n, j, k->w, (char*)k->V + (size_t)j * vb, k->ow, k->hcol.data()));
    const double beta = k->hcol[j].real();
    if (!(beta > 0.0) || !std::isfinite(beta)) return lsa_set_error(ctx, LSA_ERR_ARG, "lsa_krylov_inject: vector lies in the span of the basis");
    return LSA_OK;
}

enum class Orth {
    cgs2_fused,
    cgs2_staged,
    dcgs2,
};
struct StepPlan {
    bool pipelined = false;
    Orth orth = Orth::cgs2_fused;
    bool tail = false;
};

static StepPlan step_plan(lsa_ctx* ctx, const lsa_krylov* k) {
    const KrylovSwitches& sw = krylov_switches();
    const lsa_op* op = k->op;
    StepPlan p;
    if (!sw.fused) p.orth = Orth::cgs2_staged;
    else if (sw.delayed && ctx->nranks == 1 && !op->adjoint && op->n == k->n && k_dcgs2_fits(k->n, k->ncv)) p.orth = Orth::dcgs2;
    p.pipelined = k->pipeline && (k->batch > 1 || p.orth == Orth::dcgs2) && op->Kfac && op->nd && !op->pc &&
                  !(ctx->nranks > 1 && (!op->nd_dist || ctx->host_gather));
    p.tail = p.pipelined && sw.tail && sw.fused && op->Kmul && !op->adjoint && !op->keep && !op->refine && op->n == k->n &&
             k_cgs2_tail_fits(ctx, k->n, k->ncv, op->Kmul, op->Kfac);
    return p;
}

static int krylov_enqueue_step(lsa_ctx* ctx, lsa_krylov* k, const StepPlan& plan, int32_t j, int32_t slot, bool first) {
    lsa_op* op = k->op;
    const int dtype = LSA_C128;
    const size_t vb = (size_t)k->n * 16;
    const void* vj = (char*)k->V + (size_t)j * vb;
    void* vn = (char*)k->V + (size_t)(j + 1) * vb;
    void* sl = (char*)k->Hdev + (size_t)slot * krylov_slot_bytes(k->ncv);
    double* chk = k->checks + 2 * (size_t)slot;
    const bool dcgs2 = plan.orth == Orth::dcgs2;
    if (plan.orth != Orth::cgs2_staged) LSA_CHECK(k->ow.ensure_fused(ctx, k->n));
    const bool ahead = plan.tail && dcgs2 && first && k->pre_for == j && k->pre_op == op;
    k->drop_preapply();
    if (plan.tail) {
        if (!ahead && k->t_for != j) LSA_CHECK(spmv_global(ctx, op->Kmul, dtype, vj, op->t, false));
        k->t_for = -1;
        if (!ahead) LSA_CHECK(pc_global(ctx, pc_of(op), op->Kfac->row0, op->n, dtype, op->t, k->w));
        double* parts = k->tail_parts + (size_t)slot * 2 * (size_t)k->tail_nparts;
        if (dcgs2) {
            LSA_CHECK(k_dcgs2_step(ctx, k->n, j, k->V, k->n, k->w, first ? 1 : 0, sl, k->ncv, k->ow.fused, nullptr, nullptr, nullptr));
            LSA_CHECK(k_dcgs2_tail(ctx, k->n, j, k->V, k->n, k->w, k->ow.fused, op->Kmul, op->Kfac, op->t, parts, sl, k->ncv));
        } else {
            LSA_CHECK(k_cgs2_fused_tail(ctx, k->n, j + 1, k->V, k->n, k->w, k->w2, vn, sl, k->ow.fused, op->Kmul, op->Kfac, op->t, parts));
        }
        k->t_for = j + 1;
        return LSA_OK;
    }
    k->t_for = -1;
    const void* rhs = vj;
    if (op->Kmul) {
        LSA_CHECK(spmv_global(ctx, op->Kmul, dtype, vj, op->t, op->adjoint));
        rhs = op->t;
    }
    LSA_CHECK(direct_solve_enqueue(ctx, op, dtype, rhs, k->w, op->gw.z, op->gw.w, op->refine, chk));
    const SolveCheck check{rhs, op->gw.z, op->gw.w, chk};
    const bool rides = plan.orth != Orth::cgs2_staged;
    if (!rides) LSA_CHECK(k_residual_norms(ctx, dtype, op->n, check.b, check.z, check.r, check.out));
    if (op->keep) LSA_CHECK(k_mask(ctx, dtype, op->n, op->keep, k->w));
    if (dcgs2) {
        LSA_CHECK(k_dcgs2_step(ctx, k->n, j, k->V, k->n, k->w, first ? 1 : 0, sl, k->ncv, k->ow.fused, check.b, check.z, check.out));
        return k_dcgs2_norm(ctx, k->n, k->ow.fused, sl, k->ncv);
    }
    return orthonormalize_enqueue(ctx, dtype, k->n, k->V, k->n, j + 1, k->w, vn, k->ow, sl, rides ? &check : nullptr);
}

struct HessView {
    cplx* Hh;
    int32_t ldh, j0, ncv;
    cplx* col(int32_t j) const { return Hh + (size_t)j * ldh; }
};

static int judge_norm(double beta, const cplx* col, int32_t rows) {
    if (!std::isfinite(beta)) return -1;
    double colmax = 0.0;
    for (int32_t i = 0; i < rows; ++i) colmax = std::max(colmax, std::hypot(col[i].re, col[i].im));
    return beta <= 1e-14 * std::max(colmax, 1e-300) ? 1 : 0;
}

static int take_column(const HessView& H, int32_t j, const cplx* h) {
    cplx* Hj = H.col(j);
    for (int32_t i = 0; i < H.ldh; ++i) Hj[i] = i <= j + 1 ? h[i] : cplx{0.0, 0.0};
    return judge_norm(h[j + 1].re, h, j + 1);
}

static int finish_column(const HessView& H, int32_t jc, const cplx* sl) {
    cplx* Hp = H.col(jc - 1);
    const double nu = sl[2 * H.ncv].re;
    for (int32_t i = 0; i < jc; ++i) Hp[i] = cplx{Hp[i].re + sl[i].re, Hp[i].im + sl[i].im};
    Hp[jc] = cplx{nu, 0.0};
    return judge_norm(nu, Hp, jc);
}

static int provisional_column(const HessView& H, int32_t jc, const cplx* sl, bool first, cplx* h) {
    const int32_t ncv = H.ncv;
    const double inv = 1.0 / sl[2 * ncv].re;
    for (int32_t i = 0; i < jc; ++i) h[i] = sl[ncv + i];
    h[jc] = sl[2 * ncv + 1];
    if (!first) {
        for (int32_t c = 0; c < jc; ++c) {
            const cplx a = sl[c];
            const cplx* Hc = H.col(c);
            const int32_t rows = std::min(jc, std::max(H.j0, c + 1));
            for (int32_t i = 0; i <= rows; ++i) {
                h[i].re -= Hc[i].re * a.re - Hc[i].im * a.im;
                h[i].im -= Hc[i].re * a.im + Hc[i].im * a.re;
            }
        }
        for (int32_t i = 0; i <= jc; ++i) h[i] = cplx{h[i].re * inv, h[i].im * inv};
    }
    h[jc + 1] = cplx{sl[2 * ncv + 2].re, 0.0};
    return take_column(H, jc, h);
}

static int arnoldi_nonfinite(lsa_ctx* ctx, int32_t j) { return lsa_set_error(ctx, LSA_ERR_NONFINITE, "Arnoldi: non-finite norm at step %d", j); }

struct ExtendCursor {
    int32_t j;
    bool pending;
};

static int pipelined_prepare(lsa_ctx* ctx, lsa_krylov* k, const StepPlan& plan) {
    lsa_op* op = k->op;
    if (!op->gw_ready) {
        LSA_CHECK(op->gw.alloc(ctx, op->n, std::max(1, std::min({op->opts.ksp_restart, op->opts.ksp_maxit, 40})), LSA_C128));
        op->gw_ready = true;
    }
    if (plan.tail && !k->tail_parts) {
        const int32_t slots = 2 * std::max(k->batch, 1);
        k->tail_nparts = k_cgs2_tail_parts(k->n);
        LSA_HIP_ALLOC(ctx, hipMalloc(&k->w2, (size_t)k->n * 16));
        LSA_HIP_ALLOC(ctx, hipMalloc((void**)&k->tail_parts, (size_t)slots * 2 * (size_t)k->tail_nparts * sizeof(double)));
    }
    return LSA_OK;
}

static int preapply_enqueue(lsa_ctx* ctx, lsa_krylov* k, int32_t m) {
    if (k->pre_col == m && k->pre_op == k->op) return LSA_OK;
    k->drop_preapply();
    if (!krylov_switches().preapply || m < 1 || m > k->ncv) return LSA_OK;
    const StepPlan plan = step_plan(ctx, k);
    if (!(plan.pipelined && plan.tail && plan.orth == Orth::dcgs2)) return LSA_OK;
    LSA_CHECK(pipelined_prepare(ctx, k, plan));
    lsa_op* op = k->op;
    k->t_for = -1;
    LSA_CHECK(spmv_global(ctx, op->Kmul, LSA_C128, (char*)k->V + (size_t)m * (size_t)k->n * 16, op->t, false));
    LSA_CHECK(pc_global(ctx, pc_of(op), op->Kfac->row0, op->n, LSA_C128, op->t, k->w));
    k->pre_col = m;
    k->pre_op = op;
    return LSA_OK;
}

static int accept_steps(lsa_ctx* ctx, lsa_krylov* k, const HessView& H, bool delayed, const char* slots, size_t slot_stride, const double* chk,
                        size_t chk_stride, int32_t nb, ExtendCursor* c, int32_t* breakdown, int32_t* accepted_out) {
    lsa_op* op = k->op;
    const double rtol = op->opts.ksp_rtol;
    cplx* hwork = (cplx*)k->hcol.data();
    const int32_t j = c->j;
    int32_t accepted = 0;
    *accepted_out = 0;
    for (int32_t s = 0; s < nb; ++s, ++accepted) {
        const cplx* hc = (const cplx*)(slots + (size_t)s * slot_stride);
        const bool first = s == 0 && !c->pending;
        if (delayed && !first) {
            c->pending = false;
            const int what = finish_column(H, j + s, hc);
            if (what < 0) return arnoldi_nonfinite(ctx, j + s - 1);
            if (what > 0) {
                *breakdown = j + s - 1;
                return LSA_OK;
            }
        }
        const double beta0 = std::sqrt(chk[(size_t)s * chk_stride]), bnorm = std::sqrt(chk[(size_t)s * chk_stride + 1]);
        if (!(beta0 <= rtol * bnorm)) {
            if (!op->refine && std::isfinite(beta0)) op->refine = true;
            else k->pipeline = false;
            break;
        }
        stats_book_direct_solve(&op->st, op->Kmul ? 2 : 1, op->refine, beta0, bnorm);
        const int what = delayed ? provisional_column(H, j + s, hc, first, hwork) : take_column(H, j + s, hc);
        c->pending = delayed;
        if (what < 0) return arnoldi_nonfinite(ctx, j + s);
        if (what > 0) {
            *breakdown = j + s;
            return LSA_OK;
        }
    }
    c->j = j + accepted;
    *accepted_out = accepted;
    if (accepted < nb) k->t_for = -1;
    return LSA_OK;
}

static int extend_pipelined(lsa_ctx* ctx, lsa_krylov* k, const HessView& H, ExtendCursor* c, int32_t j1, int32_t* breakdown) {
    StepPlan plan = step_plan(ctx, k);
    LSA_CHECK(pipelined_prepare(ctx, k, plan));
    const int32_t slots = std::max(k->batch, 1);
    const size_t colb = krylov_slot_bytes(k->ncv);
    const size_t region = (size_t)slots * (colb + 2 * sizeof(double));
    LSA_CHECK(lsa_ensure_scratch(ctx, 0, 2 * region));
    const bool delayed = plan.orth == Orth::dcgs2;
    const bool ahead = krylov_switches().preapply;
    if (ahead) LSA_CHECK(k->ensure_events(ctx));
    k->t_for = -1;
    struct Queued {
        int32_t j, nb, set;
    };
    auto host_of = [&](int32_t set) { return (char*)ctx->pinned + (size_t)set * region; };
    auto slot_of = [&](int32_t set) { return (char*)k->Hdev + (size_t)set * (size_t)slots * colb; };
    auto queued = [&](int32_t set) -> int {
        if (ahead) LSA_HIP_CHECK(ctx, hipEventRecord(k->ev_read[set], ctx->stream));
        return LSA_OK;
    };
    auto wait_for = [&](const Queued& q) -> int {
        const double tw = now_s();
        if (ahead) LSA_HIP_CHECK(ctx, hipEventSynchronize(k->ev_read[q.set]));
        else LSA_HIP_CHECK(ctx, hipStreamSynchronize(ctx->stream));
        if (krylov_switches().timing) fprintf(stderr, "[lsa_krylov] %d steps from %d: waited %.3f ms\n", q.nb, q.j, 1e3 * (now_s() - tw));
        return LSA_OK;
    };
    auto queue_batch = [&](const StepPlan& p, int32_t j, bool first, int32_t set, Queued* q) -> int {
        const int32_t nb = std::min<int32_t>(slots, j1 - j);
        const double tq = now_s();
        for (int32_t s = 0; s < nb; ++s) {
            const int rc = krylov_enqueue_step(ctx, k, p, j + s, set * slots + s, s == 0 && first);
            if (rc != LSA_OK) {
                (void)hipStreamSynchronize(ctx->stream);
                return rc;
            }
        }
        double* chk = k->checks + 2 * (size_t)set * (size_t)slots;
        if (p.tail) LSA_CHECK(k_cgs2_tail_checks(ctx, nb, k->tail_nparts, k->tail_parts + (size_t)set * (size_t)slots * 2 * (size_t)k->tail_nparts, chk));
        LSA_HIP_CHECK(ctx, hipMemcpyAsync(host_of(set), slot_of(set), (size_t)nb * colb, hipMemcpyDeviceToHost, ctx->stream));
        LSA_HIP_CHECK(ctx, hipMemcpyAsync(host_of(set) + (size_t)slots * colb, chk, (size_t)nb * 2 * sizeof(double), hipMemcpyDeviceToHost, ctx->stream));
        LSA_CHECK(queued(set));
        if (krylov_switches().timing) fprintf(stderr, "[lsa_krylov] %d steps from %d queued in %.3f ms\n", nb, j, 1e3 * (now_s() - tq));
        *q = Queued{j, nb, set};
        return LSA_OK;
    };
    auto queue_flush = [&](int32_t j, int32_t set, Queued* q) -> int {
        LSA_CHECK(k_dcgs2_step(ctx, k->n, j, k->V, k->n, nullptr, 0, slot_of(set), k->ncv, k->ow.fused, nullptr, nullptr, nullptr));
        LSA_HIP_CHECK(ctx, hipMemcpyAsync(host_of(set), slot_of(set), colb, hipMemcpyDeviceToHost, ctx->stream));
        LSA_CHECK(queued(set));
        if (k->pre_armed && j == k->ncv) LSA_CHECK(preapply_enqueue(ctx, k, j));
        *q = Queued{j, 0, set};
        return LSA_OK;
    };
    auto drain = [&]() -> int {
        k->t_for = -1;
        k->drop_preapply();
        LSA_HIP_CHECK(ctx, hipStreamSynchronize(ctx->stream));
        return LSA_OK;
    };
    Queued cur{0, 0, 0}, next{0, 0, 0};
    bool have = false, flushed = false;
    if (c->j < j1 && plan.pipelined) {
        LSA_CHECK(queue_batch(plan, c->j, !c->pending, 0, &cur));
        have = true;
    }
    while (have) {
        bool have_next = false;
        if (ahead) {
            const int32_t jn = cur.j + cur.nb;
            if (jn < j1) LSA_CHECK(queue_batch(plan, jn, !delayed, cur.set ^ 1, &next));
            else if (delayed) LSA_CHECK(queue_flush(jn, cur.set ^ 1, &next));
            have_next = jn < j1 || delayed;
        }
        LSA_CHECK(wait_for(cur));
        int32_t accepted = 0;
        const char* host = host_of(cur.set);
        const int arc = accept_steps(ctx, k, H, delayed, host, colb, (const double*)(host + (size_t)slots * colb), 2, cur.nb, c, breakdown, &accepted);
        if (arc != LSA_OK || *breakdown >= 0) {
            if (have_next) (void)drain();
            return arc;
        }
        if (accepted == cur.nb && have_next) {
            cur = next;
            if (cur.nb == 0) {
                flushed = true;
                break;
            }
            continue;
        }
        if (have_next) LSA_CHECK(drain());
        plan = step_plan(ctx, k);
        have = c->j < j1 && plan.pipelined;
        if (have) LSA_CHECK(queue_batch(plan, c->j, !c->pending, 0, &cur));
    }
    if (c->pending) {
        const int32_t j = c->j;
        if (!flushed) LSA_CHECK(queue_flush(j, 0, &cur));
        LSA_CHECK(wait_for(cur));
        c->pending = false;
        const int what = finish_column(H, j, (const cplx*)host_of(cur.set));
        if (what != 0) k->drop_preapply();
        if (what < 0) return arnoldi_nonfinite(ctx, j - 1);
        if (what > 0) *breakdown = j - 1;
    }
    return LSA_OK;
}

static int extend_one_step(lsa_ctx* ctx, lsa_krylov* k, const HessView& H, int32_t j, int32_t j1, int32_t* breakdown) {
    const size_t vb = (size_t)k->n * 16;
    k->t_for = -1;
    if (j < j1) k->drop_preapply();
    for (; j < j1; ++j) {
        const void* vj = (char*)k->V + (size_t)j * vb;
        void* vn = (char*)k->V + (size_t)(j + 1) * vb;
        LSA_CHECK(op_apply_dev(ctx, k->op, vj, k->w));
        LSA_CHECK(orthonormalize(ctx, LSA_C128, k->n, k->V, k->n, j + 1, k->w, vn, k->ow, k->hcol.data()));
        const int what = take_column(H, j, (const cplx*)k->hcol.data());
        if (what < 0) return arnoldi_nonfinite(ctx, j);
        if (what > 0) {
            *breakdown = j;
            break;
        }
    }
    return LSA_OK;
}

static int extend_rest(lsa_ctx* ctx, lsa_krylov* k, const HessView& H, ExtendCursor* c, int32_t j1, int32_t* bd) {
    int rc = LSA_OK;
    if (step_plan(ctx, k).pipelined) rc = extend_pipelined(ctx, k, H, c, j1, bd);
    if (rc == LSA_OK && *bd < 0) rc = extend_one_step(ctx, k, H, c->j, j1, bd);
    return rc;
}

int lsa_krylov_extend(lsa_ctx* ctx, lsa_krylov* k, int32_t j0, int32_t j1, void* H, int32_t ldh, int32_t* breakdown) {
    if (!ctx || !k || !H) return lsa_set_error(ctx, LSA_ERR_ARG, "lsa_krylov_extend: null argument");
    if (j0 < 0 || j1 < j0 || j1 > k->ncv || ldh < j1 + 1) return lsa_set_error(ctx, LSA_ERR_ARG, "lsa_krylov_extend: bad step range [%d, %d) for ncv %d", j0, j1, k->ncv);
    const double t0 = now_s();
    const HessView Hv{(cplx*)H, ldh, j0, k->ncv};
    ExtendCursor c{j0, false};
    int32_t bd = -1;
    if (k->pre_for != j0 || j0 >= j1) k->drop_preapply();
    const int rc = extend_rest(ctx, k, Hv, &c, j1, &bd);
    k->pre_for = -1;
    if (breakdown) *breakdown = bd;
    k->op->st.seconds_solve += now_s() - t0;
    return rc;
}

}

void krylov_arm_preapply(lsa_krylov* k, bool on) { k->pre_armed = on && krylov_switches().preapply; }

int krylov_preapply(lsa_ctx* ctx, lsa_krylov* k, int32_t m) { return k->pre_armed ? preapply_enqueue(ctx, k, m) : (int)LSA_OK; }

static int krylov_restart_impl(lsa_ctx* ctx, lsa_krylov* k, int32_t m, int32_t knew, const void* Q, int32_t ldq, bool queued) {
    const size_t vb = (size_t)k->n * 16;
    const int32_t ahead = k->pre_col == m && k->pre_op == k->op ? knew : -1;
    k->drop_preapply();
    if (knew > 0) LSA_CHECK(basis_times_host_matrix(ctx, LSA_C128, k->n, m, knew, k->V, Q, ldq, k->qdev, k->V2, 0));
    LSA_CHECK(k_copy(ctx, LSA_C128, k->n, (char*)k->V + (size_t)m * vb, (char*)k->V2 + (size_t)knew * vb));
    if (!queued) LSA_HIP_CHECK(ctx, hipStreamSynchronize(ctx->stream));
    std::swap(k->V, k->V2);
    k->pre_for = ahead;
    return LSA_OK;
}

int krylov_restart_queued(lsa_ctx* ctx, lsa_krylov* k, int32_t m, int32_t knew, const void* Q, int32_t ldq) {
    return krylov_restart_impl(ctx, k, m, knew, Q, ldq, krylov_switches().preapply && step_plan(ctx, k).pipelined);
}

int krylov_group_alloc(lsa_ctx* ctx, int32_t J, lsa_krylov* const* ks, KrylovGroupBuf* gb) {
    memset(gb, 0, sizeof *gb);
    gb->J = J;
    gb->slots = std::max(ks[0]->batch, 1);
    gb->nparts = k_cgs2_tail_parts(ks[0]->n);
    const size_t cells = (size_t)J * (size_t)gb->slots;
    LSA_HIP_ALLOC(ctx, hipMalloc(&gb->Hdev, cells * krylov_slot_bytes(ks[0]->ncv)));
    LSA_HIP_ALLOC(ctx, hipMalloc((void**)&gb->checks, cells * 2 * sizeof(double)));
    LSA_HIP_ALLOC(ctx, hipMalloc((void**)&gb->tail_parts, cells * 2 * (size_t)gb->nparts * sizeof(double)));
    LSA_HIP_CHECK(ctx, hipMemsetAsync(gb->tail_parts, 0, cells * 2 * (size_t)gb->nparts * sizeof(double), ctx->stream));
    return LSA_OK;
}

void krylov_group_free(KrylovGroupBuf* gb) {
    for (void* p : {gb->Hdev, (void*)gb->checks, (void*)gb->tail_parts})
        if (p) (void)hipFree(p);
    memset(gb, 0, sizeof *gb);
}

int krylov_group_check(lsa_ctx* ctx, int32_t J, lsa_krylov* const* ks) {
    for (int32_t z = 0; z < J; ++z) {
        if (!ks[z] || !ks[z]->op) return lsa_set_error(ctx, LSA_ERR_ARG, "lsa_krylov_solve_batch: null workspace (problem %d)", z);
        if (ks[z]->ctx != ctx) return lsa_set_error(ctx, LSA_ERR_ARG, "lsa_krylov_solve_batch: the workspace of problem %d lives in another context", z);
        if (ks[z]->n != ks[0]->n || ks[z]->ncv != ks[0]->ncv || ks[z]->batch != ks[0]->batch)
            return lsa_set_error(ctx, LSA_ERR_ARG, "lsa_krylov_solve_batch: problem %d has another shape (n = %lld, ncv = %d) than problem 0 (n = %lld, ncv = %d)", z,
                                 (long long)ks[z]->n, ks[z]->ncv, (long long)ks[0]->n, ks[0]->ncv);
        for (int32_t y = 0; y < z; ++y)
            if (ks[y] == ks[z] || ks[y]->op == ks[z]->op)
                return lsa_set_error(ctx, LSA_ERR_ARG, "lsa_krylov_solve_batch: problems %d and %d share a workspace or an operator", y, z);
    }
    return LSA_OK;
}

int krylov_extend_batch(lsa_ctx* ctx, KrylovGroupBuf* gb, lsa_krylov* const* ks, const uint8_t* active, const int32_t* j0, int32_t j1, void* const* Hs,
                        int32_t ldh, int32_t* breakdown, int32_t* status, std::string* errs, lsa_ks_batch_info* info) {
    const int32_t J = gb->J, slots = gb->slots;
    const double t0 = now_s();
    auto fail = [&](int32_t z, int rc) {
        status[z] = rc;
        lsa_name_problem(ctx, z);
        errs[z] = ctx->err;
    };
    struct Member {
        ExtendCursor c;
        HessView H;
        bool lock;
        int32_t nb;
    } mem[kKrylovGroupMax];
    int32_t nactive = 0;
    int32_t ncv = 0;
    for (int32_t z = 0; z < J; ++z) {
        mem[z] = Member{ExtendCursor{0, false}, HessView{nullptr, 0, 0, 0}, false, 0};
        if (!active[z]) continue;
        ++nactive;
        ncv = ks[z]->ncv;
        breakdown[z] = -1;
        status[z] = LSA_OK;
        mem[z] = Member{ExtendCursor{j0[z], false}, HessView{(cplx*)Hs[z], ldh, j0[z], ks[z]->ncv}, true, 0};
        ks[z]->t_for = -1;
        ks[z]->drop_preapply();
    }
    const size_t colb = krylov_slot_bytes(ncv);
    const size_t cells = (size_t)J * (size_t)slots;
    while (true) {
        int32_t lead = -1, rounds = 0;
        for (int32_t z = 0; z < J; ++z) {
            Member& m = mem[z];
            m.nb = 0;
            if (!active[z] || !m.lock || status[z] != LSA_OK || breakdown[z] >= 0 || m.c.j >= j1) continue;
            lsa_krylov* k = ks[z];
            const StepPlan plan = step_plan(ctx, k);
            bool in = plan.pipelined && plan.orth == Orth::dcgs2 && plan.tail;
            if (in && lead >= 0)
                in = nd_batch_compatible(ks[lead]->op->nd, k->op->nd) && ks[lead]->op->Kmul->dtype == k->op->Kmul->dtype;
            if (!in) {
                m.lock = false;
                continue;
            }
            int rc = pipelined_prepare(ctx, k, plan);
            if (rc == LSA_OK) rc = k->ow.ensure_fused(ctx, k->n);
            if (rc != LSA_OK) {
                fail(z, rc);
                continue;
            }
            if (lead < 0) lead = z;
            m.nb = std::min<int32_t>(slots, j1 - m.c.j);
            rounds = std::max(rounds, m.nb);
        }
        if (lead < 0) break;
        int rc = lsa_ensure_scratch(ctx, 0, cells * (colb + 2 * sizeof(double)));
        int32_t sweep_launches = 0;
        (void)lsa_ndlu_info(ks[lead]->op->nd, nullptr, nullptr, nullptr, nullptr, nullptr, nullptr, &sweep_launches, nullptr, nullptr, nullptr);
        for (int32_t s = 0; s < rounds && rc == LSA_OK; ++s) {
            int32_t R = 0, jr[kKrylovGroupMax], fr[kKrylovGroupMax];
            lsa_ndlu* nd[kKrylovGroupMax];
            const lsa_mat *Mr[kKrylovGroupMax], *Cr[kKrylovGroupMax];
            const void *rhs[kKrylovGroupMax], *yr[kKrylovGroupMax];
            void *xr[kKrylovGroupMax], *Vr[kKrylovGroupMax], *slot[kKrylovGroupMax], *work[kKrylovGroupMax], *tr[kKrylovGroupMax];
            double* parts[kKrylovGroupMax];
            int32_t products = 0;
            for (int32_t z = 0; z < J && rc == LSA_OK; ++z) {
                if (s >= mem[z].nb) continue;
                lsa_krylov* k = ks[z];
                lsa_op* op = k->op;
                const int32_t j = mem[z].c.j + s;
                const size_t cell = (size_t)s * (size_t)J + (size_t)z;
                if (k->t_for != j) {
                    rc = spmv_global(ctx, op->Kmul, LSA_C128, (char*)k->V + (size_t)j * (size_t)k->n * 16, op->t, false);
                    ++products;
                }
                k->t_for = -1;
                jr[R] = j;
                fr[R] = (s == 0 && !mem[z].c.pending) ? 1 : 0;
                nd[R] = op->nd;
                Mr[R] = op->Kmul;
                Cr[R] = op->Kfac;
                rhs[R] = op->t;
                xr[R] = k->w;
                yr[R] = k->w;
                Vr[R] = k->V;
                slot[R] = (char*)gb->Hdev + cell * colb;
                work[R] = k->ow.fused;
                tr[R] = op->t;
                parts[R] = gb->tail_parts + cell * 2 * (size_t)gb->nparts;
                ++R;
            }
            const NdSolve sweeps = {R, nd, true, 0, LSA_C128, 1, rhs, 0, xr, 0, "lsa_krylov_solve_batch"};
            if (rc == LSA_OK) rc = ndlu_solve_run(ctx, sweeps);
            if (rc == LSA_OK) rc = k_dcgs2_step_batch(ctx, R, ks[lead]->n, jr, Vr, ks[lead]->n, yr, fr, slot, ncv, work);
            if (rc == LSA_OK) rc = k_dcgs2_tail_batch(ctx, R, ks[lead]->n, jr, Vr, ks[lead]->n, yr, work, Mr, Cr, tr, parts, slot, ncv);
            for (int32_t z = 0; z < J; ++z)
                if (s < mem[z].nb) ks[z]->t_for = mem[z].c.j + s + 1;
            if (info) {
                ++info->rounds;
                info->launches += sweep_launches + 3 + products;
            }
        }
        if (rc == LSA_OK) rc = k_cgs2_tail_checks(ctx, rounds * J, gb->nparts, gb->tail_parts, gb->checks);
        char* host = (char*)ctx->pinned;
        if (rc == LSA_OK && (hipMemcpyAsync(host, gb->Hdev, (size_t)rounds * J * colb, hipMemcpyDeviceToHost, ctx->stream) != hipSuccess ||
                             hipMemcpyAsync(host + cells * colb, gb->checks, (size_t)rounds * J * 2 * sizeof(double), hipMemcpyDeviceToHost, ctx->stream) != hipSuccess))
            rc = lsa_set_error(ctx, LSA_ERR_HIP, "lsa_krylov_solve_batch: read-back of a period failed");
        if (hipStreamSynchronize(ctx->stream) != hipSuccess && rc == LSA_OK) rc = lsa_set_error(ctx, LSA_ERR_HIP, "lsa_krylov_solve_batch: a lockstep period failed on the device");
        if (info) ++info->periods;
        if (rc != LSA_OK) {
            const std::string text = ctx->err;
            for (int32_t z = 0; z < J; ++z)
                if (mem[z].nb > 0) {
                    ctx->err = text;
                    fail(z, rc);
                }
            break;
        }
        const double* chk = (const double*)(host + cells * colb);
        for (int32_t z = 0; z < J; ++z) {
            Member& m = mem[z];
            if (m.nb == 0) continue;
            int32_t accepted = 0;
            const int arc = accept_steps(ctx, ks[z], m.H, true, host + (size_t)z * colb, (size_t)J * colb, chk + 2 * (size_t)z, 2 * (size_t)J, m.nb, &m.c,
                                         &breakdown[z], &accepted);
            if (breakdown[z] >= 0) accepted = breakdown[z] + 1 - m.c.j;
            if (arc != LSA_OK) fail(z, arc);
            else if (info) info->lockstep_steps[z] += accepted;
        }
    }
    for (int32_t z = 0; z < J; ++z) {
        if (!active[z] || status[z] != LSA_OK || breakdown[z] >= 0) continue;
        const int32_t jb = mem[z].c.j;
// ... 140 lines not shown
```

lsa-fw_amd/csrc/spmv.hip:

```cpp
#include <algorithm>

#include "lsa_internal.h"

template <typename T>
__device__ __forceinline__ T shfl_xor_t(T v, int mask);
template <>
__device__ __forceinline__ double shfl_xor_t<double>(double v, int mask) {
    return __shfl_xor(v, mask, 64);
}
template <>
__device__ __forceinline__ cplx shfl_xor_t<cplx>(cplx v, int mask) {
    return cplx{__shfl_xor(v.re, mask, 64), __shfl_xor(v.im, mask, 64)};
}

template <bool NT, typename T>
__device__ __forceinline__ T stream_load(const T* p) {
    if constexpr (NT) {
        if constexpr (sizeof(T) == 16) {
            typedef double v2d __attribute__((ext_vector_type(2)));
            const v2d v = __builtin_nontemporal_load((const v2d*)p);
            T out;
            s_from(out, v.x, v.y);
            return out;
        } else {
// ... 199 lines not shown
        pairs[(size_t)4 * q + 3] = A->h_rp[(size_t)r0 + 1] - A->h_rp[r0];
    }
    gs.swap(pairs);
    if (hipMalloc((void**)&A->grp_start, gs.size() * sizeof(int32_t)) != hipSuccess) return false;
    if (hipMemcpy(A->grp_start, gs.data(), gs.size() * sizeof(int32_t), hipMemcpyHostToDevice) != hipSuccess) {
        (void)hipFree(A->grp_start);
        A->grp_start = nullptr;
        return false;
    }
    A->ngroups = ng;
    A->grp_state = 1;
    return true;
}

static bool ensure_ci16(const lsa_mat* A) {
    if (A->ci16_state != 0) return A->ci16_state > 0;
    A->ci16_state = -1;
    const int32_t n = A->n;
    if ((int64_t)A->h_rp.size() != (int64_t)n + 1 || (int64_t)A->h_ci.size() != A->nnz) return false;
    std::vector<uint16_t> d((size_t)std::max<int64_t>(A->nnz, 1));
    std::vector<int32_t> base((size_t)std::max(n, 1), 0);
    for (int32_t r = 0; r < n; ++r) {
        const int32_t p0 = A->h_rp[r], p1 = A->h_rp[r + 1];
        if (p0 == p1) continue;
        int32_t lo = A->h_ci[p0];
        for (int32_t p = p0; p < p1; ++p) lo = std::min(lo, A->h_ci[p]);
        base[r] = lo;
        for (int32_t p = p0; p < p1; ++p) {
            const int32_t delta = A->h_ci[p] - lo;
            if (delta > 65535) return false;
            d[p] = (uint16_t)delta;
        }
    }
    if (hipMalloc((void**)&A->ci16, d.size() * sizeof(uint16_t)) != hipSuccess) return false;
    if (hipMalloc((void**)&A->cbase, base.size() * sizeof(int32_t)) != hipSuccess) {
        (void)hipFree(A->ci16);
        A->ci16 = nullptr;
        return false;
    }
    if (hipMemcpy(A->ci16, d.data(), d.size() * sizeof(uint16_t), hipMemcpyHostToDevice) != hipSuccess ||
        hipMemcpy(A->cbase, base.data(), base.size() * sizeof(int32_t), hipMemcpyHostToDevice) != hipSuccess) {
        (void)hipFree(A->ci16);
        (void)hipFree(A->cbase);
        A->ci16 = nullptr;
        A->cbase = nullptr;
        return false;
    }
    A->ci16_state = 1;
    return true;
}

static int spmv_lanes_per_row(const lsa_mat* A, int variant) {
    int lpr = variant & 0xff;
    if (lpr == 0) {
        const double mean = A->n > 0 ? (double)A->nnz / (double)A->n : 0.0;
        lpr = mean <= 6.0 ? 4 : mean <= 12.0 ? 8 : mean <= 48.0 ? 16 : mean <= 96.0 ? 32 : 64;
    }
    return (lpr == 4 || lpr == 8 || lpr == 32 || lpr == 64) ? lpr : 16;
}
static bool spmv_wants_groups(const lsa_mat* A, int variant) {
    if (variant & 0x4000) return false;
    if (variant & (0x100 | 0x200 | 0x400)) return false;
    return (variant & 0x2000) || A->nnz >= (int64_t)4 << 20;
}
static bool spmv_wants_ci16(const lsa_mat* A, int variant) {
    const size_t msize = A->dtype == LSA_C128 ? 16 : 8;
    return ((variant & 0x800) || (variant == 0 && msize == 16 && A->nnz >= (int64_t)4 << 20)) && !(variant & 0x100) && !(variant & 0x200);
}

template <typename MT, typename VT, int LPR, bool NT>
static void launch_spmv(lsa_ctx* ctx, const lsa_mat* A, const void* x, void* y, int variant) {
    const int threads = 256;
    int64_t want = ((int64_t)A->n * LPR + threads - 1) / threads;
    const int per_cu = (variant >> 16) > 0 ? (variant >> 16) : 64;
    int64_t cap = (int64_t)ctx->num_cu * per_cu;
    int blocks = (int)(want < 1 ? 1 : (want > cap ? cap : want));
    if ((variant & 0x200) && A->n >= 8 * (256 / LPR)) {
        const int rows_per_pass = 256 / LPR;
        int G = (int)(((blocks + 7) / 8) * 8);
        int64_t rows_per_wg = ((int64_t)A->n + G - 1) / G;
        rows_per_wg = ((rows_per_wg + rows_per_pass - 1) / rows_per_pass) * rows_per_pass;
        hipLaunchKernelGGL((spmv_xcd_kernel<MT, VT, LPR, NT>), dim3(G), dim3(threads), 0, ctx->stream, A->n, (int32_t)rows_per_wg, A->rp,
                           A->ci, (const MT*)A->val, (const VT*)x, (VT*)y);
        return;
    }
    if (!NT && spmv_wants_groups(A, variant) && ensure_groups(A)) {
        const bool c16 = (variant & 0x800) && ensure_ci16(A);
        int64_t gwant = ((int64_t)A->ngroups * LPR + threads - 1) / threads;
        const int64_t gcap = (variant >> 16) > 0 ? cap : (int64_t)ctx->num_cu * 256;
        const int gblocks = (int)(gwant < 1 ? 1 : (gwant > gcap ? gcap : gwant));
        if ((variant & 0x8000) && !c16 && A->ngroups >= 8 * 64) {
            const int G = ((gblocks + 7) / 8) * 8;
            const int32_t chunk = (A->ngroups + G - 1) / G;
            hipLaunchKernelGGL((spmv_group_kernel<MT, VT, LPR, false, true>), dim3(G), dim3(threads), 0, ctx->stream, A->ngroups, chunk, (const int4*)A->grp_start, A->rp,
                               A->ci, (const uint16_t*)nullptr, (const int32_t*)nullptr, (const MT*)A->val, (const VT*)x, (VT*)y);
            return;
        }
        if (c16)
            hipLaunchKernelGGL((spmv_group_kernel<MT, VT, LPR, true, false>), dim3(gblocks), dim3(threads), 0, ctx->stream, A->ngroups, 0, (const int4*)A->grp_start, A->rp,
                               A->ci, (const uint16_t*)A->ci16, (const int32_t*)A->cbase, (const MT*)A->val, (const VT*)x, (VT*)y);
        else
            hipLaunchKernelGGL((spmv_group_kernel<MT, VT, LPR, false, false>), dim3(gblocks), dim3(threads), 0, ctx->stream, A->ngroups, 0, (const int4*)A->grp_start, A->rp,
                               A->ci, (const uint16_t*)nullptr, (const int32_t*)nullptr, (const MT*)A->val, (const VT*)x, (VT*)y);
        return;
    }
    if (spmv_wants_ci16(A, variant) && !NT && ensure_ci16(A)) {
        hipLaunchKernelGGL((spmv_subwave16_kernel<MT, VT, LPR>), dim3(blocks), dim3(threads), 0, ctx->stream, A->n, A->rp, (const uint16_t*)A->ci16,
                           (const int32_t*)A->cbase, (const MT*)A->val, (const VT*)x, (VT*)y);
        return;
    }
    if (variant & 0x400) {
        blocks = (blocks + 1) / 2;
        hipLaunchKernelGGL((spmv_subwave2_kernel<MT, VT, LPR, NT>), dim3(blocks), dim3(threads), 0, ctx->stream, A->n, A->rp, A->ci,
                           (const MT*)A->val, (const VT*)x, (VT*)y);
        return;
    }
    hipLaunchKernelGGL((spmv_subwave_kernel<MT, VT, LPR, NT>), dim3(blocks), dim3(threads), 0, ctx->stream, A->n, A->rp, A->ci,
                       (const MT*)A->val, (const VT*)x, (VT*)y);
}

template <typename MT, typename VT, bool NT>
static void dispatch_lpr(lsa_ctx* ctx, const lsa_mat* A, const void* x, void* y, int variant) {
    switch (spmv_lanes_per_row(A, variant)) {
        case 4: launch_spmv<MT, VT, 4, NT>(ctx, A, x, y, variant); break;
        case 8: launch_spmv<MT, VT, 8, NT>(ctx, A, x, y, variant); break;
        case 32: launch_spmv<MT, VT, 32, NT>(ctx, A, x, y, variant); break;
        case 64: launch_spmv<MT, VT, 64, NT>(ctx, A, x, y, variant); break;
        default: launch_spmv<MT, VT, 16, NT>(ctx, A, x, y, variant); break;
    }
}

static int spmv_variant() {
    const char* e = getenv("LSA_SPMV_VARIANT");
    return e ? (int)strtol(e, nullptr, 0) : 0;
}

void spmv_share_extras(const lsa_mat* from, lsa_mat* to) {
    const int variant = spmv_variant();
    if (!(variant & 0x100)) {
        if (spmv_wants_groups(from, variant) && ensure_groups(from)) {
            if (variant & 0x800) (void)ensure_ci16(from);
        } else if (spmv_wants_ci16(from, variant))
            (void)ensure_ci16(from);
    }
    to->grp_start = from->grp_state > 0 ? from->grp_start : nullptr;
    to->ngroups = from->grp_state > 0 ? from->ngroups : 0;
    to->grp_state = from->grp_state > 0 ? 1 : -1;
    to->ci16 = from->ci16_state > 0 ? from->ci16 : nullptr;
    to->cbase = from->ci16_state > 0 ? from->cbase : nullptr;
    to->ci16_state = from->ci16_state > 0 ? 1 : -1;
    to->owns_extras = false;
}

int k_spmv_plain_subwave_lanes(const lsa_mat* A) {
    const int variant = spmv_variant();
    if (variant != 0 || spmv_wants_groups(A, variant) || spmv_wants_ci16(A, variant)) return 0;
    return spmv_lanes_per_row(A, variant);
}

template <typename MT, typename VT>
static void dispatch_spmv(lsa_ctx* ctx, const lsa_mat* A, const void* x, void* y) {
    const int variant = spmv_variant();
    if (variant & 0x100) dispatch_lpr<MT, VT, true>(ctx, A, x, y, variant);
    else dispatch_lpr<MT, VT, false>(ctx, A, x, y, variant);
}

int k_spmv(lsa_ctx* ctx, const lsa_mat* A, int xdtype, const void* x, void* y) {
    if (A->dtype == LSA_F64 && xdtype == LSA_F64) dispatch_spmv<double, double>(ctx, A, x, y);
    else if (A->dtype == LSA_F64 && xdtype == LSA_C128) dispatch_spmv<double, cplx>(ctx, A, x, y);
    else if (A->dtype == LSA_C128 && xdtype == LSA_C128) dispatch_spmv<cplx, cplx>(ctx, A, x, y);
    else return lsa_set_error(ctx, LSA_ERR_ARG, "spmv: a complex matrix needs complex vectors");
    hipError_t e = hipGetLastError();
    if (e != hipSuccess) return lsa_set_error(ctx, LSA_ERR_HIP, "spmv launch failed: %s", hipGetErrorString(e));
    return LSA_OK;
}

template <typename MT, typename VT>
__device__ __forceinline__ void spmv_transpose_pull(int32_t ncols, int conj, const int32_t* __restrict__ rp, const int32_t* __restrict__ ci,
                                                    const int32_t* __restrict__ src, const MT* __restrict__ val, const VT* __restrict__ x,
                                                    VT* __restrict__ y) {
    constexpr int LPR = 16;
    const int64_t gid = (int64_t)blockIdx.x * blockDim.x + threadIdx.x;
    const int32_t lane = (int32_t)(gid % LPR);
    const int64_t stride = ((int64_t)gridDim.x * blockDim.x) / LPR;
    for (int64_t c = gid / LPR; c < ncols; c += stride) {
        VT acc = scalar_traits<VT>::zero();
        for (int32_t q = rp[c] + lane; q < rp[c + 1]; q += LPR) {
            MT a = val[src[q]];
            if (conj) a = s_conj(a);
            fma_acc(acc, a, x[ci[q]]);
        }
#pragma unroll
        for (int m = LPR / 2; m > 0; m >>= 1) acc = s_add(acc, shfl_xor_t<VT>(acc, m));
        if (lane == 0) y[c] = acc;
    }
}

template <typename MT, typename VT>
__global__ __launch_bounds__(256) void spmv_transpose_pull_kernel(int32_t ncols, int conj, const int32_t* __restrict__ rp, const int32_t* __restrict__ ci,
                                                                  const int32_t* __restrict__ src, const MT* __restrict__ val,
                                                                  const VT* __restrict__ x, VT* __restrict__ y) {
    spmv_transpose_pull<MT, VT>(ncols, conj, rp, ci, src, val, x, y);
}

constexpr int kSpmvBatchMax = 16;
// ... 195 lines not shown
```

lsa-fw_amd/lsa_hip/__init__.py:

```python

from __future__ import annotations

import ctypes
import os
from pathlib import Path

import numpy as np

LSA_F64, LSA_C128 = 0, 1

_STATUS_NAMES = {
    0: "LSA_OK",
    -1: "LSA_ERR_ARG",
    -2: "LSA_ERR_HIP",
    -3: "LSA_ERR_ZERO_PIVOT",
    -4: "LSA_ERR_DIVERGED",
    -5: "LSA_ERR_NONFINITE",
    -6: "LSA_ERR_TIMEOUT",
    -7: "LSA_ERR_COMM",
    -8: "LSA_ERR_OOM",
}

globals().update({name: code for code, name in _STATUS_NAMES.items()})

# ... 124 lines not shown
        ("seconds_gram", ctypes.c_double),
        ("seconds_dense", ctypes.c_double),
    ]


class lsa_contour_batch_stats(ctypes.Structure):
    _fields_ = [
        ("enabled", ctypes.c_int32),
        ("pad0", ctypes.c_int32),
        ("groups", ctypes.c_int64),
        ("batched_columns", ctypes.c_int64),
        ("serial_columns", ctypes.c_int64),
    ]


class lsa_stochastic_stats(ctypes.Structure):
    _fields_ = [
        ("nodes", ctypes.c_int32),
        ("kind", ctypes.c_int32),
        ("bytes", ctypes.c_int64),
        ("seconds_factor", ctypes.c_double),
        ("seconds_solve", ctypes.c_double),
        ("seconds_product", ctypes.c_double),
        ("seconds_dense", ctypes.c_double),
        ("solver", lsa_stats),
        ("batch_adjoint", ctypes.c_int32),
        ("adjoint_batches", ctypes.c_int64),
        ("forward_batches", ctypes.c_int64),
        ("seconds_solve_adjoint", ctypes.c_double),
        ("seconds_product_adjoint", ctypes.c_double),
    ]


_P = ctypes.c_void_p
_I32, _I64, _DBL = ctypes.c_int32, ctypes.c_int64, ctypes.c_double
_PP = ctypes.POINTER(ctypes.c_void_p)

SIGNATURES = {
    "lsa_ctx_create": (ctypes.c_int, [ctypes.c_int, _PP]),
    "lsa_ctx_destroy": (None, [_P]),
    "lsa_last_error": (ctypes.c_char_p, [_P]),
    "lsa_ctx_synchronize": (ctypes.c_int, [_P]),
    "lsa_ctx_mem_info": (ctypes.c_int, [_P, ctypes.POINTER(_I64), ctypes.POINTER(_I64)]),
    "lsa_ctx_arch": (ctypes.c_char_p, [_P]),
    "lsa_vec_create": (ctypes.c_int, [_P, _I64, ctypes.c_int, _PP]),
    "lsa_vec_destroy": (None, [_P]),
    "lsa_vec_upload": (ctypes.c_int, [_P, _P, _P]),
    "lsa_vec_download": (ctypes.c_int, [_P, _P, _P]),
    "lsa_csr_upload": (ctypes.c_int, [_P, _I32, _I64, _P, _P, _P, ctypes.c_int, _PP]),
    "lsa_mat_destroy": (None, [_P]),
    "lsa_mat_download_values": (ctypes.c_int, [_P, _P, _P]),
    "lsa_csr_axpby": (ctypes.c_int, [_P, _P, _P, _DBL * 2, _DBL * 2, ctypes.c_int, _PP]),
    "lsa_csr_window": (ctypes.c_int, [_P, _P, _P, _P, _PP]),
    "lsa_spmv": (ctypes.c_int, [_P, _P, _P, _P]),
    "lsa_spmv_transpose": (ctypes.c_int, [_P, _P, ctypes.c_int, _P, _P]),
    "lsa_spmv_transpose_batch": (ctypes.c_int, [_P, _I32, _PP, ctypes.c_int, _PP, _PP]),
    "lsa_spmv_info": (ctypes.c_int, [_P, _P, ctypes.c_int, ctypes.c_char_p, _I32, ctypes.POINTER(_I64)]),
    "lsa_spmv_time": (ctypes.c_int, [_P, _P, _P, _P, ctypes.c_int, ctypes.POINTER(_DBL)]),
    "lsa_ilu_create": (ctypes.c_int, [_P, _P, ctypes.c_int, _DBL, _PP]),
    "lsa_ilu_destroy": (None, [_P]),
    "lsa_ilu_set_algorithm": (ctypes.c_int, [_P, _P, ctypes.c_int, _I32]),
    "lsa_ilu_solve": (ctypes.c_int, [_P, _P, ctypes.c_int, _P, _P]),
    "lsa_ilu_solve_time": (ctypes.c_int, [_P, _P, ctypes.c_int, _P, _P, ctypes.c_int, ctypes.POINTER(_DBL)]),
    "lsa_ilu_info": (ctypes.c_int, [_P, ctypes.POINTER(_I64), ctypes.POINTER(_I32), ctypes.POINTER(_I32), ctypes.POINTER(_I32)]),
    "lsa_ilu_download": (ctypes.c_int, [_P, _P, _P, _P, _P]),
    "lsa_nd_analyse": (ctypes.c_int, [_I32, _P, _P, _I32, _P, _PP]),
    "lsa_nd_order": (ctypes.c_int, [_I32, _P, _P, _I32, _P, _PP]),
    "lsa_nd_analyse_tree": (ctypes.c_int, [_I32, _P, _P, _I32, _P, _P, _P, _P, _I32, _I32, _PP]),
    "lsa_nd_sym_export_dist": (ctypes.c_int, [_P, _P, _P, _P, _P, _P, _P, _P]),
    "lsa_nd_sym_export_top": (ctypes.c_int, [_P, _P, _P, _P, _P]),
    "lsa_ndlu_inertia": (ctypes.c_int, [_P, _P, ctypes.POINTER(_I64), ctypes.POINTER(_I64), ctypes.POINTER(_I64)]),
    "lsa_dense_sym_inertia": (ctypes.c_int, [_I32, _P, _I32, _DBL, ctypes.POINTER(_I64), ctypes.POINTER(_I64), ctypes.POINTER(_I64)]),
    "lsa_nd_sym_error": (ctypes.c_char_p, [_P]),
    "lsa_nd_sym_destroy": (None, [_P]),
    "lsa_nd_sym_info": (ctypes.c_int, [_P, ctypes.POINTER(_I32), ctypes.POINTER(_I32), ctypes.POINTER(_I32), ctypes.POINTER(_I64),
                                       ctypes.POINTER(_I64), ctypes.POINTER(_I64), ctypes.POINTER(_DBL)]),
    "lsa_nd_sym_export": (ctypes.c_int, [_P, _P, _P, _P, _P, _P, _P]),
    "lsa_nd_sym_memory": (ctypes.c_int, [_P, _I32, _I64, _P, _P, _P, _P]),
    "lsa_nd_sym_export_tables": (ctypes.c_int, [_P, _P, _P, _P, _P, _P, _P]),
    "lsa_ndlu_create": (ctypes.c_int, [_P, _P, _I32, _PP]),
    "lsa_ndlu_prepare": (ctypes.c_int, [_P, _P, ctypes.c_int, _I32, _P]),
    "lsa_ndlu_prepare_tree": (ctypes.c_int, [_P, _P, ctypes.c_int, _I32, _P, _P, _P]),
    "lsa_ndlu_create_tree": (ctypes.c_int, [_P, _P, _I32, _P, _P, _P, _P, _PP]),
    "lsa_ndlu_refactor": (ctypes.c_int, [_P, _P, _P]),
    "lsa_ndlu_destroy": (None, [_P]),
    "lsa_ndlu_solve": (ctypes.c_int, [_P, _P, _P, _P]),
    "lsa_ndlu_solve_batch": (ctypes.c_int, [_P, _I32, _PP, _PP, _PP]),
    "lsa_ndlu_solve_batch_adjoint": (ctypes.c_int, [_P, _I32, _PP, ctypes.c_int, _PP, _PP]),
    "lsa_ndlu_prepared_memory": (ctypes.c_int, [_P, _P]),
    "lsa_ndlu_solve_adjoint": (ctypes.c_int, [_P, _P, ctypes.c_int, _P, _P]),
    "lsa_ndlu_solve_time": (ctypes.c_int, [_P, _P, _P, _P, ctypes.c_int, ctypes.POINTER(_DBL)]),
    "lsa_ndlu_solve_multi": (ctypes.c_int, [_P, _P, ctypes.c_int, _I32, _P, _I64, _P, _I64]),
    "lsa_ndlu_solve_multi_time": (ctypes.c_int, [_P, _P, ctypes.c_int, _I32, _P, _I64, _P, _I64, ctypes.c_int, ctypes.POINTER(_DBL)]),
    "lsa_ndlu_solve_multi_batch": (ctypes.c_int, [_P, _I32, _PP, ctypes.c_int, _I32, _PP, _I64, _PP, _I64]),
    "lsa_ndlu_solve_multi_batch_time": (ctypes.c_int, [_P, _I32, _PP, ctypes.c_int, _I32, _PP, _I64, _PP, _I64, ctypes.c_int, ctypes.POINTER(_DBL)]),
    "lsa_ndlu_solve_multi_batch_adjoint": (ctypes.c_int, [_P, _I32, _PP, ctypes.c_int, _I32, _PP, _I64, _PP, _I64]),
    "lsa_ndlu_solve_multi_batch_adjoint_time": (ctypes.c_int, [_P, _I32, _PP, ctypes.c_int, _I32, _PP, _I64, _PP, _I64, ctypes.c_int, ctypes.POINTER(_DBL)]),
    "lsa_ndlu_set_multi_transposed": (ctypes.c_int, [_P, _P, ctypes.c_int]),
    "lsa_ndlu_multi_info": (ctypes.c_int, [_P, ctypes.POINTER(_I32), ctypes.POINTER(_I64), ctypes.POINTER(_I32)]),
    "lsa_ndlu_info": (ctypes.c_int, [_P, ctypes.POINTER(_I32), ctypes.POINTER(_I32), ctypes.POINTER(_I32), ctypes.POINTER(_I64),
                                     ctypes.POINTER(_I64), ctypes.POINTER(_I64), ctypes.POINTER(_I32), ctypes.POINTER(_DBL), ctypes.POINTER(_DBL),
                                     ctypes.POINTER(_I32)]),
    "lsa_ndlu_sweep_level": (ctypes.c_int, [_P, _I32] + [ctypes.POINTER(_I32)] * 6),
    "lsa_gmres": (ctypes.c_int, [_P, _P, _P, _P, _P, ctypes.c_int, _DBL, ctypes.c_int, ctypes.c_int, ctypes.POINTER(_I32), ctypes.POINTER(_DBL)]),
    "lsa_op_create": (ctypes.c_int, [_P, _P, _P, _DBL * 2, ctypes.c_int, ctypes.POINTER(lsa_op_options), _PP]),
    "lsa_op_create_sharded": (ctypes.c_int, [_P, _P, _P, _P, _P, _DBL * 2, ctypes.c_int, ctypes.POINTER(lsa_op_options), _PP]),
    "lsa_op_create_dist": (ctypes.c_int, [_P, _P, _P, _I32, _I32, _I32, _P, _P, _P, _P, _DBL * 2, ctypes.c_int, ctypes.POINTER(lsa_op_options), _PP]),
    "lsa_op_destroy": (None, [_P]),
    "lsa_op_apply": (ctypes.c_int, [_P, _P, _P, _P]),
    "lsa_op_stats": (ctypes.c_int, [_P, ctypes.POINTER(lsa_stats)]),
    "lsa_op_set_adjoint": (ctypes.c_int, [_P, _P, ctypes.c_int]),
    "lsa_op_set_projection": (ctypes.c_int, [_P, _P, _P]),
    "lsa_krylov_create": (ctypes.c_int, [_P, _P, _I32, _PP]),
    "lsa_krylov_destroy": (None, [_P]),
    "lsa_krylov_set_row_permutation": (ctypes.c_int, [_P, _P, _P]),
    "lsa_krylov_set_start": (ctypes.c_int, [_P, _P, _P]),
    "lsa_krylov_inject": (ctypes.c_int, [_P, _P, _I32, _P]),
    "lsa_krylov_extend": (ctypes.c_int, [_P, _P, _I32, _I32, _P, _I32, ctypes.POINTER(_I32)]),
    "lsa_krylov_restart": (ctypes.c_int, [_P, _P, _I32, _I32, _P, _I32]),
    "lsa_krylov_ritz_vectors": (ctypes.c_int, [_P, _P, _I32, _I32, _P, _I32, ctypes.c_int, _P]),
    "lsa_krylov_imag_norms": (ctypes.c_int, [_P, _I32, _P]),
    "lsa_krylov_shape": (ctypes.c_int, [_P, ctypes.POINTER(_I64), ctypes.POINTER(_I32)]),
    "lsa_mat_rows": (_I64, [_P]),
    "lsa_krylov_solve": (ctypes.c_int, [_P, _P, _P, _P, _P, _I32, _P, _P, _P, _P, _P]),
    "lsa_krylov_solve_batch": (ctypes.c_int, [_P, _I32, _PP, _PP, _PP, _I32, _PP, _PP, _PP, _PP, _P, _P, _P]),
    "lsa_eigs_sinvert": (ctypes.c_int, [_P, _P, _P, _DBL * 2, _I32, _I32, _DBL, _I32, ctypes.POINTER(lsa_op_options), _P, _P, _I32, _P, _P, _P, _P, _P]),
    "lsa_dense_schur": (ctypes.c_int, [_I32, _P, _I32, _P, _I32]),
    "lsa_dense_schur_reorder": (ctypes.c_int, [_I32, _P, _I32, _P, _I32, _P, ctypes.POINTER(_I32)]),
    "lsa_dense_tri_eigenvectors": (ctypes.c_int, [_I32, _P, _I32, _P, _I32]),
    "lsa_eig_residuals": (ctypes.c_int, [_P, _P, _P, _I32, _P, _P, _P]),
    "lsa_eig_biorth": (ctypes.c_int, [_P, _P, _I64, _I32, _P, _P, _P, _P, _P]),
    "lsa_lanczos_create": (ctypes.c_int, [_P, _P, _I32, _PP]),
    "lsa_lanczos_destroy": (None, [_P]),
    "lsa_lanczos_set_row_permutation": (ctypes.c_int, [_P, _P, _P]),
    "lsa_lanczos_set_start": (ctypes.c_int, [_P, _P, _P]),
    "lsa_lanczos_extend": (ctypes.c_int, [_P, _P, _I32, _I32, _P, _I32, ctypes.POINTER(_I32)]),
    "lsa_lanczos_basis": (ctypes.c_int, [_P, _P, _I32, _P]),
    "lsa_lanczos_solve": (ctypes.c_int, [_P, _P, ctypes.POINTER(lsa_ks_options), _P, _I32, _P, _P, _P, _P, ctypes.POINTER(lsa_ks_result)]),
    "lsa_dense_syev": (ctypes.c_int, [_I32, _P, _I32, _P]),
    "lsa_resolvent_create": (ctypes.c_int, [_P, _P, _I32, _PP]),
    "lsa_resolvent_destroy": (None, [_P]),
    "lsa_resolvent_set_row_permutation": (ctypes.c_int, [_P, _P, _P]),
    "lsa_resolvent_set_block_forcings": (ctypes.c_int, [_P, _P, ctypes.c_int]),
    "lsa_resolvent_set_weights": (ctypes.c_int, [_P, _P, _P, _P]),
    "lsa_resolvent_set_start": (ctypes.c_int, [_P, _P, _P]),
    "lsa_resolvent_extend": (ctypes.c_int, [_P, _P, _I32, _I32, _P, _I32, ctypes.POINTER(_I32)]),
    "lsa_resolvent_basis": (ctypes.c_int, [_P, _P, _I32, _P]),
    "lsa_resolvent_solve": (ctypes.c_int, [_P, _P, ctypes.POINTER(lsa_ks_options), _P, _I32, _P, _P, _P, _P, _P, ctypes.POINTER(lsa_ks_result), _P]),
    "lsa_growth_create": (ctypes.c_int, [_P, _P, _I32, _I32, _P, _PP]),
    "lsa_growth_destroy": (None, [_P]),
    "lsa_growth_set_row_permutation": (ctypes.c_int, [_P, _P, _P]),
    "lsa_growth_set_steps": (ctypes.c_int, [_P, _P, _I32]),
    "lsa_growth_set_scheme": (ctypes.c_int, [_P, _P, _I32]),
    "lsa_growth_set_response_weight": (ctypes.c_int, [_P, _P, _P]),
    "lsa_growth_response_energy": (ctypes.c_int, [_P, _P, _I32, _P]),
    "lsa_growth_set_start": (ctypes.c_int, [_P, _P, _P]),
    "lsa_growth_extend": (ctypes.c_int, [_P, _P, _I32, _I32, _P, _I32, ctypes.POINTER(_I32)]),
    "lsa_growth_basis": (ctypes.c_int, [_P, _P, _I32, _P]),
    "lsa_growth_solve": (ctypes.c_int, [_P, _P, ctypes.POINTER(lsa_ks_options), _P, _I32, _P, _P, _P, _P, _P, _P, ctypes.POINTER(lsa_ks_result), _P]),
    "lsa_spmm": (ctypes.c_int, [_P, _P, _I32, _P, _I64, _P, _I64]),
    "lsa_spmm_transpose": (ctypes.c_int, [_P, _P, ctypes.c_int, _I32, _P, _I64, _P, _I64]),
    "lsa_block_gram": (ctypes.c_int, [_P, _I64, _I32, _P, _I64, _I32, _P, _I64, _P]),
    "lsa_contour_create": (ctypes.c_int, [_P, _P, _P, _I32, _DBL * 2, _DBL * 2, _I32, ctypes.c_int, _DBL, _PP]),
    "lsa_contour_destroy": (None, [_P]),
    "lsa_contour_set_row_permutation": (ctypes.c_int, [_P, _P, _P]),
    "lsa_contour_solve": (ctypes.c_int, [_P, _P, _DBL, _I32, _P, _I32, _P, _P, _P, ctypes.POINTER(lsa_contour_result)]),
    "lsa_contour_info": (ctypes.c_int, [_P, ctypes.POINTER(lsa_contour_stats)]),
    "lsa_contour_set_batch_nodes": (ctypes.c_int, [_P, _P, ctypes.c_int]),
    "lsa_contour_batch_info": (ctypes.c_int, [_P, ctypes.POINTER(lsa_contour_batch_stats)]),
    "lsa_contour_solve_left": (ctypes.c_int, [_P, _P, _DBL, _I32, _P, _I32, _P, _P, _P, ctypes.POINTER(lsa_contour_result)]),
    "lsa_contour_left_info": (ctypes.c_int, [_P, ctypes.POINTER(lsa_contour_left_stats)]),
# ... 234 lines not shown
                ctx.handle, n_global, row0, row0 + A.shape[0], A.nnz, _ptr(rp), _ptr(ci), _ptr(val), _dtype_code(dt), ctypes.byref(h)
            )
        )
        return cls(ctx, h, (A.shape[0], n_global), A.nnz, dt)

    def prepare_lu(self, complex_factors: bool, leaf_size: int = 0, constraint=None) -> None:
        flags = None if constraint is None else np.ascontiguousarray(constraint, dtype=np.int8)
        self.ctx.check(self.ctx._lib.lsa_ndlu_prepare(self.ctx.handle, self.handle, LSA_C128 if complex_factors else LSA_F64, int(leaf_size),
                                                      None if flags is None else _ptr(flags)))

    def prepare_lu_tree(self, complex_factors: bool, first, size, parent) -> None:
        first, size, parent = (np.ascontiguousarray(a, dtype=np.int32) for a in (first, size, parent))
        self.ctx.check(self.ctx._lib.lsa_ndlu_prepare_tree(self.ctx.handle, self.handle, LSA_C128 if complex_factors else LSA_F64, len(parent),
                                                           _ptr(first), _ptr(size), _ptr(parent)))

    def axpby(self, other: "CsrMatrix", alpha: complex, beta: complex, dtype=None) -> "CsrMatrix":
        alpha, beta = complex(alpha), complex(beta)
        if dtype is None:
            cplx = alpha.imag != 0 or beta.imag != 0 or self.dtype.kind == "c" or other.dtype.kind == "c"
            dtype = np.complex128 if cplx else np.float64
        h = ctypes.c_void_p()
        self.ctx.check(
            self.ctx._lib.lsa_csr_axpby(
                self.ctx.handle, self.handle, other.handle, (_DBL * 2)(alpha.real, alpha.imag), (_DBL * 2)(beta.real, beta.imag),
                _dtype_code(dtype), ctypes.byref(h),
            )
        )
        return CsrMatrix(self.ctx, h, self.shape, self.nnz, dtype, keep=(self, other))

    def windowed(self, left, right=None) -> "CsrMatrix":
        n = self.shape[0]
        vecs = []
        for name, v in (("left", left), ("right", right)):
            if v is None and name == "right":
                vecs.append(None)
                continue
            a = np.asarray(v)
            if a.dtype.kind == "c":
                raise ValueError(f"lsa_csr_window: {name} is complex")
            a = np.ascontiguousarray(a, dtype=np.float64)
            if a.shape != (n,):
                raise ValueError(f"lsa_csr_window: {name} must have shape ({n},), got {a.shape}")
            vecs.append(a)
        h = ctypes.c_void_p()
        self.ctx.check(self.ctx._lib.lsa_csr_window(self.ctx.handle, self.handle, _ptr(vecs[0]), None if vecs[1] is None else _ptr(vecs[1]),
                                                    ctypes.byref(h)))
        return CsrMatrix(self.ctx, h, self.shape, self.nnz, np.float64, keep=(self,))

    def values(self) -> np.ndarray:
        out = np.empty(self.nnz, dtype=self.dtype)
        self.ctx.check(self.ctx._lib.lsa_mat_download_values(self.ctx.handle, self.handle, _ptr(out)))
        return out

    def matvec(self, x: DeviceVector, y: DeviceVector) -> None:
        self.ctx.check(self.ctx._lib.lsa_spmv(self.ctx.handle, self.handle, x.handle, y.handle))

    def rmatvec(self, x: DeviceVector, y: DeviceVector, conj: bool = True) -> None:
        self.ctx.check(self.ctx._lib.lsa_spmv_transpose(self.ctx.handle, self.handle, int(conj), x.handle, y.handle))

    @staticmethod
    def spmv_transpose_batch(mats: "list[CsrMatrix]", xs: "list[DeviceVector]", ys: "list[DeviceVector]", conj: bool = False) -> None:
        J = len(mats)
        if J == 0 or len(xs) != J or len(ys) != J:
            raise ValueError("spmv_transpose_batch needs as many inputs and outputs as matrices (at least one)")
        ctx = mats[0].ctx
        if any(m.ctx is not ctx for m in mats) or any(v.ctx is not ctx for v in list(xs) + list(ys)):
            raise ValueError("spmv_transpose_batch: the matrices and vectors must live in one context")
        arr = lambda objs: (ctypes.c_void_p * J)(*[o.handle.value for o in objs])
        ctx.check(ctx._lib.lsa_spmv_transpose_batch(ctx.handle, J, arr(mats), int(conj), arr(xs), arr(ys)))

    def matmat(self, X: DeviceVector, Y: DeviceVector, ncols: int, ldx: int | None = None, ldy: int | None = None) -> None:
        n = self.shape[0]
        self.ctx.check(self.ctx._lib.lsa_spmm(self.ctx.handle, self.handle, int(ncols), X.handle, int(n if ldx is None else ldx), Y.handle,
                                              int(n if ldy is None else ldy)))

    def matmat_transpose(self, X: DeviceVector, Y: DeviceVector, ncols: int, conj: bool = True, ldx: int | None = None,
                         ldy: int | None = None) -> None:
        n = self.shape[0]
        self.ctx.check(self.ctx._lib.lsa_spmm_transpose(self.ctx.handle, self.handle, int(bool(conj)), int(ncols), X.handle,
                                                        int(n if ldx is None else ldx), Y.handle, int(n if ldy is None else ldy)))

    def matvec_info(self, vector_dtype=np.complex128) -> dict:
        name = ctypes.create_string_buffer(128)
        nbytes = _I64(0)
        self.ctx.check(self.ctx._lib.lsa_spmv_info(self.ctx.handle, self.handle, _dtype_code(vector_dtype), name, 128, ctypes.byref(nbytes)))
        return {"kernel": name.value.decode(), "bytes_moved": nbytes.value}

    def time_matvec(self, x: DeviceVector, y: DeviceVector, iters: int) -> float:
        ms = _DBL(0.0)
        self.ctx.check(self.ctx._lib.lsa_spmv_time(self.ctx.handle, self.handle, x.handle, y.handle, int(iters), ctypes.byref(ms)))
        return ms.value

    def __del__(self):
        if getattr(self, "handle", None) and getattr(self.ctx, "handle", None):
            self.ctx._lib.lsa_mat_destroy(self.handle)
            self.handle = None


class Ilu:

    def __init__(self, ctx: Context, C: CsrMatrix, levels: int = 0, shift_tol: float = 0.0):
        self.ctx, self._C = ctx, C
        h = ctypes.c_void_p()
        ctx.check(ctx._lib.lsa_ilu_create(ctx.handle, C.handle, int(levels), float(shift_tol), ctypes.byref(h)))
        self.handle = h
        self.n = C.shape[0]
        self.dtype = C.dtype

    def info(self) -> dict:
        nnz, ll, lu, ns = _I64(0), _I32(0), _I32(0), _I32(0)
        self.ctx._lib.lsa_ilu_info(self.handle, ctypes.byref(nnz), ctypes.byref(ll), ctypes.byref(lu), ctypes.byref(ns))
        return {"nnz": nnz.value, "levels_lower": ll.value, "levels_upper": lu.value, "nshift": ns.value}

    def set_algorithm(self, algo: int, block_size: int = 0) -> None:
        self.ctx.check(self.ctx._lib.lsa_ilu_set_algorithm(self.ctx.handle, self.handle, int(algo), int(block_size)))

    def solve(self, b: DeviceVector, x: DeviceVector, which: int = 2) -> None:
        self.ctx.check(self.ctx._lib.lsa_ilu_solve(self.ctx.handle, self.handle, int(which), b.handle, x.handle))

    def time_solve(self, b: DeviceVector, x: DeviceVector, iters: int, which: int = 2) -> float:
        ms = _DBL(0.0)
        self.ctx.check(self.ctx._lib.lsa_ilu_solve_time(self.ctx.handle, self.handle, int(which), b.handle, x.handle, int(iters), ctypes.byref(ms)))
        return ms.value

    def factors(self):
        nnz = self.info()["nnz"]
        rp = np.empty(self.n + 1, dtype=np.int32)
        ci = np.empty(nnz, dtype=np.int32)
        val = np.empty(nnz, dtype=self.dtype)
        self.ctx.check(self.ctx._lib.lsa_ilu_download(self.ctx.handle, self.handle, _ptr(rp), _ptr(ci), _ptr(val)))
        return rp, ci, val

    def __del__(self):
        if getattr(self, "handle", None) and getattr(self.ctx, "handle", None):
            self.ctx._lib.lsa_ilu_destroy(self.handle)
            self.handle = None


class NdAnalysis:

    def __init__(self, A, leaf_size: int = 0, constraint=None, tree=None, rank: int = 0, nranks: int = 1, order_only: bool = False):
        import scipy.sparse as sp

        A = sp.csr_matrix(A)
        if A.shape[0] != A.shape[1]:
            raise ValueError("the analysis needs a square pattern")
        self._lib = load_library()
        self.n, self.nnz = A.shape[0], A.nnz
        rp = np.ascontiguousarray(A.indptr, dtype=np.int32)
# ... 930 lines not shown
```

Baseline: 610.6.

## Compact mass matrix and decouple tail product from the residual check

Adds a compacted copy of the mass matrix M with explicit zeros dropped and uses it for the Krylov step multiply (step_mul). The fused tail kernel now walks M's own sparsity instead of sharing C's pattern, and the check product C·y becomes optional (a CHECK template flag). It can also run in a separate cgs_check_kernel on a side stream. The aim is to cut wasted nonzero traffic in the M·w product and to take the check off the critical path. The cost is extra index and pattern reads and a second stream that has to be synchronised.

After: 609.0 (median of 3 runs). No clear change (-0.3%).

```diff
diff --git a/include/lsa_hip.h b/include/lsa_hip.h
--- a/include/lsa_hip.h
+++ b/include/lsa_hip.h
@@ -64,6 +64,9 @@
 int lsa_csr_axpby(lsa_ctx *ctx, const lsa_mat *A, const lsa_mat *B, const double alpha[2], const double beta[2],
                   int out_dtype, lsa_mat **out);
 int lsa_csr_window(lsa_ctx *ctx, const lsa_mat *M, const double *left, const double *right, lsa_mat **out);
+int lsa_csr_compact(lsa_ctx *ctx, const lsa_mat *M, const lsa_mat **out, int64_t *nnz_out);
+int64_t lsa_csr_compact_host(int32_t n, const int32_t *rowptr, const int32_t *col, const void *val, int dtype, int32_t *rowptr_out,
+                             int32_t *col_out, void *val_out);
 int lsa_spmv(lsa_ctx *ctx, const lsa_mat *A, const lsa_vec *x, lsa_vec *y);
 int lsa_spmv_transpose(lsa_ctx *ctx, const lsa_mat *A, int conj, const lsa_vec *x, lsa_vec *y);
 int lsa_spmv_transpose_batch(lsa_ctx *ctx, int32_t J, const lsa_mat *const *A, int conj, const lsa_vec *const *x, lsa_vec *const *y);
@@ -158,6 +161,8 @@
 int lsa_krylov_set_start(lsa_ctx *ctx, lsa_krylov *k, const void *host_v);
 int lsa_krylov_inject(lsa_ctx *ctx, lsa_krylov *k, int32_t j, const void *host_v);
 int lsa_krylov_extend(lsa_ctx *ctx, lsa_krylov *k, int32_t j0, int32_t j1, void *H, int32_t ldh, int32_t *breakdown);
+int lsa_krylov_tail_probe(lsa_ctx *ctx, const lsa_mat *M, const lsa_mat *C, const lsa_vec *w, const lsa_vec *y, const lsa_vec *t,
+                          lsa_vec *tnext, double pairs[2]);
 int lsa_krylov_restart(lsa_ctx *ctx, lsa_krylov *k, int32_t m, int32_t knew, const void *Q, int32_t ldq);
 int lsa_krylov_ritz_vectors(lsa_ctx *ctx, lsa_krylov *k, int32_t m, int32_t nvec, const void *Y, int32_t ldy,
                             int normalise, void *X);
diff --git a/lsa-fw_amd/csrc/blas.hip b/lsa-fw_amd/csrc/blas.hip
--- a/lsa-fw_amd/csrc/blas.hip
+++ b/lsa-fw_amd/csrc/blas.hip
@@ -430,13 +430,54 @@
     return block_sum<double>(a, smem);
 }
 
-template <typename MT, int LPR, bool DELAYED = false>
+template <int LPR>
+__device__ __forceinline__ cplx check_row_product(const int32_t* __restrict__ rp, const int32_t* __restrict__ ci, const cplx* __restrict__ cval,
+                                                  const cplx* __restrict__ y, int64_t row, int32_t lane) {
+    const int32_t p0 = rp[row], p1 = rp[row + 1];
+    cplx ac = cplx{0.0, 0.0};
+    for (int32_t p = p0 + lane; p < p1; p += 3 * LPR) {
+        int32_t c[3];
+        cplx vc[3], xy[3];
+#pragma unroll
+        for (int u = 0; u < 3; ++u) {
+            const bool in = p + u * LPR < p1;
+            c[u] = in ? ci[p + u * LPR] : 0;
+            vc[u] = in ? cval[p + u * LPR] : cplx{0.0, 0.0};
+        }
+#pragma unroll
+        for (int u = 0; u < 3; ++u) {
+            const bool in = p + u * LPR < p1;
+            xy[u] = in ? y[c[u]] : cplx{0.0, 0.0};
+        }
+#pragma unroll
+        for (int u = 0; u < 3; ++u)
+            if (p + u * LPR < p1) fma_acc(ac, vc[u], xy[u]);
+    }
+#pragma unroll
+    for (int m = LPR / 2; m > 0; m >>= 1) ac = s_add(ac, cplx{__shfl_xor(ac.re, m, 64), __shfl_xor(ac.im, m, 64)});
+    return ac;
+}
+
+__device__ __forceinline__ void check_pair_store(double rw, double rb, double (*csum)[2], double* __restrict__ chk_part) {
+    rw = wave_sum_dpp(rw);
+    rb = wave_sum_dpp(rb);
+    const int wave = threadIdx.x >> 6;
+    if ((threadIdx.x & 63) == 0) {
+        csum[wave][0] = rw;
+        csum[wave][1] = rb;
+    }
+    __syncthreads();
+    if (threadIdx.x < 2) chk_part[2 * blockIdx.x + threadIdx.x] = (csum[0][threadIdx.x] + csum[1][threadIdx.x]) + (csum[2][threadIdx.x] + csum[3][threadIdx.x]);
+}
+
+template <typename MT, int LPR, bool DELAYED = false, bool CHECK = false>
 __global__ __launch_bounds__(kThreads) void cgs_tail_kernel(int32_t n, const int32_t* __restrict__ rp, const int32_t* __restrict__ ci,
-                                                            const MT* __restrict__ mval, const cplx* __restrict__ cval,
-                                                            const cplx* __restrict__ w, const cplx* __restrict__ y,
-                                                            const double* __restrict__ nrm_part, int nparts, cplx* __restrict__ vnext, cplx* t,
-                                                            int j, const cplx* __restrict__ h1, const cplx* __restrict__ h2,
-                                                            cplx* __restrict__ hout, double* __restrict__ chk_part) {
+                                                            const MT* __restrict__ mval, const cplx* __restrict__ w,
+                                                            const double* __restrict__ nrm_part, int nparts, cplx* __restrict__ vnext,
+                                                            cplx* tnext, int j, const cplx* __restrict__ h1,
+                                                            const cplx* __restrict__ h2, cplx* __restrict__ hout, const int32_t* __restrict__ crp,
+                                                            const int32_t* __restrict__ cci, const cplx* __restrict__ cval,
+                                                            const cplx* __restrict__ y, const cplx* t, double* __restrict__ chk_part) {
     __shared__ double smem[4];
     __shared__ double tot_s;
     __shared__ double csum[4][2];
@@ -462,55 +503,65 @@
     const int64_t row_stride = ((int64_t)gridDim.x * blockDim.x) / LPR;
     double rw = 0.0, rb = 0.0;
     for (int64_t row = gid / LPR; row < n; row += row_stride) {
+        cplx ac = cplx{0.0, 0.0};
+        if constexpr (CHECK) ac = check_row_product<LPR>(crp, cci, cval, y, row, lane);
         const int32_t p0 = rp[row], p1 = rp[row + 1];
-        cplx am = cplx{0.0, 0.0}, ac = cplx{0.0, 0.0};
+        cplx am = cplx{0.0, 0.0};
         for (int32_t p = p0 + lane; p < p1; p += 3 * LPR) {
             int32_t c[3];
             MT vm[3];
-            cplx vc[3], xw[3], xy[3];
+            cplx xw[3];
 #pragma unroll
             for (int u = 0; u < 3; ++u) {
                 const bool in = p + u * LPR < p1;
                 c[u] = in ? ci[p + u * LPR] : 0;
                 vm[u] = in ? mval[p + u * LPR] : scalar_traits<MT>::zero();
-                vc[u] = in ? cval[p + u * LPR] : cplx{0.0, 0.0};
             }
 #pragma unroll
             for (int u = 0; u < 3; ++u) {
                 const bool in = p + u * LPR < p1;
                 xw[u] = in ? w[c[u]] : cplx{0.0, 0.0};
-                xy[u] = in ? y[c[u]] : cplx{0.0, 0.0};
             }
 #pragma unroll
             for (int u = 0; u < 3; ++u)
                 if (p + u * LPR < p1) {
                     if constexpr (DELAYED) fma_acc(am, vm[u], xw[u]);
                     else fma_acc(am, vm[u], s_mul(s, xw[u]));
-                    fma_acc(ac, vc[u], xy[u]);
                 }
         }
 #pragma unroll
-        for (int m = LPR / 2; m > 0; m >>= 1) {
-            am = s_add(am, cplx{__shfl_xor(am.re, m, 64), __shfl_xor(am.im, m, 64)});
-            ac = s_add(ac, cplx{__shfl_xor(ac.re, m, 64), __shfl_xor(ac.im, m, 64)});
-        }
+        for (int m = LPR / 2; m > 0; m >>= 1) am = s_add(am, cplx{__shfl_xor(am.re, m, 64), __shfl_xor(am.im, m, 64)});
+        if (lane == 0) {
+            if constexpr (CHECK) {
+                const cplx told = t[row];
+                rw += s_abs2(s_sub(told, ac));
+                rb += s_abs2(told);
+            }
+            tnext[row] = am;
+            if constexpr (!DELAYED) vnext[row] = s_mul(s, w[row]);
+        }
+    }
+    if constexpr (CHECK) check_pair_store(rw, rb, csum, chk_part);
+}
+
+template <int LPR>
+__global__ __launch_bounds__(kThreads) void cgs_check_kernel(int32_t n, const int32_t* __restrict__ rp, const int32_t* __restrict__ ci,
+                                                             const cplx* __restrict__ cval, const cplx* __restrict__ y,
+                                                             const cplx* __restrict__ t, double* __restrict__ chk_part) {
+    __shared__ double csum[4][2];
+    const int64_t gid = (int64_t)blockIdx.x * blockDim.x + threadIdx.x;
+    const int32_t lane = (int32_t)(gid % LPR);
+    const int64_t row_stride = ((int64_t)gridDim.x * blockDim.x) / LPR;
+    double rw = 0.0, rb = 0.0;
+    for (int64_t row = gid / LPR; row < n; row += row_stride) {
+        const cplx ac = check_row_product<LPR>(rp, ci, cval, y, row, lane);
         if (lane == 0) {
             const cplx told = t[row];
             rw += s_abs2(s_sub(told, ac));
             rb += s_abs2(told);
-            t[row] = am;
-            if constexpr (!DELAYED) vnext[row] = s_mul(s, w[row]);
-        }
-    }
-    rw = wave_sum_dpp(rw);
-    rb = wave_sum_dpp(rb);
-    const int wave = threadIdx.x >> 6;
-    if ((threadIdx.x & 63) == 0) {
-        csum[wave][0] = rw;
-        csum[wave][1] = rb;
-    }
-    __syncthreads();
-    if (threadIdx.x < 2) chk_part[2 * blockIdx.x + threadIdx.x] = (csum[0][threadIdx.x] + csum[1][threadIdx.x]) + (csum[2][threadIdx.x] + csum[3][threadIdx.x]);
+        }
+    }
+    check_pair_store(rw, rb, csum, chk_part);
 }
 
 struct DcgsBatchArgs {
@@ -523,9 +574,11 @@
     int32_t first[kKrylovGroupMax];
 };
 struct TailBatchArgs {
+    const int32_t* mrp[kKrylovGroupMax];
+    const int32_t* mci[kKrylovGroupMax];
+    const void* mval[kKrylovGroupMax];
     const int32_t* rp[kKrylovGroupMax];
     const int32_t* ci[kKrylovGroupMax];
-    const void* mval[kKrylovGroupMax];
     const cplx* cval[kKrylovGroupMax];
     const cplx* w[kKrylovGroupMax];
     const cplx* y[kKrylovGroupMax];
@@ -540,6 +593,8 @@
     __shared__ double smem[4];
     __shared__ double csum[4][2];
     const int z = blockIdx.z;
+    const int32_t* __restrict__ mrp = a.mrp[z];
+    const int32_t* __restrict__ mci = a.mci[z];
     const int32_t* __restrict__ rp = a.rp[z];
     const int32_t* __restrict__ ci = a.ci[z];
     const MT* __restrict__ mval = (const MT*)a.mval[z];
@@ -556,37 +611,53 @@
     const int64_t row_stride = ((int64_t)gridDim.x * blockDim.x) / LPR;
     double rw = 0.0, rb = 0.0;
     for (int64_t row = gid / LPR; row < n; row += row_stride) {
-        const int32_t p0 = rp[row], p1 = rp[row + 1];
-        cplx am = cplx{0.0, 0.0}, ac = cplx{0.0, 0.0};
+        cplx ac = cplx{0.0, 0.0};
+        {
+            const int32_t p0 = rp[row], p1 = rp[row + 1];
+            for (int32_t p = p0 + lane; p < p1; p += 3 * LPR) {
+                int32_t c[3];
+                cplx vc[3], xy[3];
+#pragma unroll
+                for (int u = 0; u < 3; ++u) {
+                    const bool in = p + u * LPR < p1;
+                    c[u] = in ? ci[p + u * LPR] : 0;
+                    vc[u] = in ? cval[p + u * LPR] : cplx{0.0, 0.0};
+                }
+#pragma unroll
+                for (int u = 0; u < 3; ++u) {
+                    const bool in = p + u * LPR < p1;
+                    xy[u] = in ? y[c[u]] : cplx{0.0, 0.0};
+                }
+#pragma unroll
+                for (int u = 0; u < 3; ++u)
+                    if (p + u * LPR < p1) fma_acc(ac, vc[u], xy[u]);
+            }
+        }
+#pragma unroll
+        for (int m = LPR / 2; m > 0; m >>= 1) ac = s_add(ac, cplx{__shfl_xor(ac.re, m, 64), __shfl_xor(ac.im, m, 64)});
+        const int32_t p0 = mrp[row], p1 = mrp[row + 1];
+        cplx am = cplx{0.0, 0.0};
         for (int32_t p = p0 + lane; p < p1; p += 3 * LPR) {
             int32_t c[3];
             MT vm[3];
-            cplx vc[3], xw[3], xy[3];
+            cplx xw[3];
 #pragma unroll
             for (int u = 0; u < 3; ++u) {
                 const bool in = p + u * LPR < p1;
-                c[u] = in ? ci[p + u * LPR] : 0;
+                c[u] = in ? mci[p + u * LPR] : 0;
                 vm[u] = in ? mval[p + u * LPR] : scalar_traits<MT>::zero();
-                vc[u] = in ? cval[p + u * LPR] : cplx{0.0, 0.0};
             }
 #pragma unroll
             for (int u = 0; u < 3; ++u) {
                 const bool in = p + u * LPR < p1;
                 xw[u] = in ? w[c[u]] : cplx{0.0, 0.0};
-                xy[u] = in ? y[c[u]] : cplx{0.0, 0.0};
             }
 #pragma unroll
             for (int u = 0; u < 3; ++u)
-                if (p + u * LPR < p1) {
-                    fma_acc(am, vm[u], xw[u]);
-                    fma_acc(ac, vc[u], xy[u]);
-                }
-        }
-#pragma unroll
-        for (int m = LPR / 2; m > 0; m >>= 1) {
-            am = s_add(am, cplx{__shfl_xor(am.re, m, 64), __shfl_xor(am.im, m, 64)});
-            ac = s_add(ac, cplx{__shfl_xor(ac.re, m, 64), __shfl_xor(ac.im, m, 64)});
-        }
+                if (p + u * LPR < p1) fma_acc(am, vm[u], xw[u]);
+        }
+#pragma unroll
+        for (int m = LPR / 2; m > 0; m >>= 1) am = s_add(am, cplx{__shfl_xor(am.re, m, 64), __shfl_xor(am.im, m, 64)});
         if (lane == 0) {
             const cplx told = t[row];
             rw += s_abs2(s_sub(told, ac));
@@ -1396,20 +1467,35 @@
     return check_launch(ctx, "cgs2_fused");
 }
 
+template <bool DELAYED>
+static void launch_tail(lsa_ctx* ctx, int64_t n, const lsa_mat* M, const cplx* w, const double* nrm_part, int blocks, cplx* vnext, cplx* tnext, int j,
+                        const cplx* h1, const cplx* h2, cplx* hout, const lsa_mat* C, const cplx* y, const cplx* t, double* tail_part) {
+    const dim3 grid(k_cgs2_tail_parts(n)), block(kThreads);
+#define LSA_TAIL_LAUNCH(MT, CHK)                                                                                                                  \
+    hipLaunchKernelGGL((cgs_tail_kernel<MT, 16, DELAYED, CHK>), grid, block, 0, ctx->stream, (int32_t)n, M->rp, M->ci, (const MT*)M->val, w, nrm_part, \
+                       blocks, vnext, tnext, j, h1, h2, hout, CHK ? C->rp : (const int32_t*)nullptr, CHK ? C->ci : (const int32_t*)nullptr,         \
+                       CHK ? (const cplx*)C->val : (const cplx*)nullptr, y, t, tail_part)
+    if (M->dtype == LSA_C128) {
+        if (C) LSA_TAIL_LAUNCH(cplx, true);
+        else LSA_TAIL_LAUNCH(cplx, false);
+    } else {
+        if (C) LSA_TAIL_LAUNCH(double, true);
+        else LSA_TAIL_LAUNCH(double, false);
+    }
+#undef LSA_TAIL_LAUNCH
+}
+
 bool k_cgs2_tail_fits(lsa_ctx* ctx, int64_t n, int jmax, const lsa_mat* M, const lsa_mat* C) {
     (void)ctx;
     if (!M || !C || !cgs2_fused_shape(n, jmax, nullptr)) return false;
     if (C->dtype != LSA_C128 || M->n != n || C->n != n || M->ncols != n || C->ncols != n || M->row0 != 0 || C->row0 != 0) return false;
-    const bool same_dev = M->rp == C->rp && M->ci == C->ci;
-    const bool same_host = M->h_rp.size() > 0 && M->h_rp.same_object(C->h_rp) && M->h_ci.same_object(C->h_ci);
-    if (M->nnz != C->nnz || !(same_dev || same_host)) return false;
     return k_spmv_plain_subwave_lanes(M) == 16 && k_spmv_plain_subwave_lanes(C) == 16;
 }
 
 int k_cgs2_tail_parts(int64_t n) { return (int)((n * 16 + kThreads - 1) / kThreads); }
 
 int k_cgs2_fused_tail(lsa_ctx* ctx, int64_t n, int j, const void* V, int64_t ldv, const void* y, void* w, void* vnext, void* hcol_dev, void* work,
-                      const lsa_mat* M, const lsa_mat* C, void* t, double* tail_part) {
+                      const lsa_mat* M, void* tnext, const lsa_mat* C, const void* t, double* tail_part) {
     typedef cplx T;
     int64_t rpb = 0;
     if (!cgs2_fused_shape(n, j, &rpb)) return lsa_set_error(ctx, LSA_ERR_ARG, "k_cgs2_fused_tail: shape outside the fused form");
@@ -1427,16 +1513,15 @@
                        (const T*)nullptr, (const T*)nullptr, (double*)nullptr);
     hipLaunchKernelGGL((cgs_axpy_kernel<T>), dim3(blocks), dim3(kThreads), 0, ctx->stream, n, j, (const T*)V, ldv, (const T*)part2, nchunks, kFuseCols,
                        (const T*)w, (T*)w, (T*)h2, nrm_part, (const double*)nullptr, (double*)nullptr);
-    const int tparts = k_cgs2_tail_parts(n);
-    if (M->dtype == LSA_C128)
-        hipLaunchKernelGGL((cgs_tail_kernel<cplx, 16>), dim3(tparts), dim3(kThreads), 0, ctx->stream, (int32_t)n, C->rp, C->ci, (const cplx*)M->val,
-                           (const cplx*)C->val, (const T*)w, (const T*)y, (const double*)nrm_part, blocks, (T*)vnext, (T*)t, j, (const T*)h1, (const T*)h2,
-                           (T*)hcol_dev, tail_part);
-    else
-        hipLaunchKernelGGL((cgs_tail_kernel<double, 16>), dim3(tparts), dim3(kThreads), 0, ctx->stream, (int32_t)n, C->rp, C->ci, (const double*)M->val,
-                           (const cplx*)C->val, (const T*)w, (const T*)y, (const double*)nrm_part, blocks, (T*)vnext, (T*)t, j, (const T*)h1, (const T*)h2,
-                           (T*)hcol_dev, tail_part);
+    launch_tail<false>(ctx, n, M, (const T*)w, (const double*)nrm_part, blocks, (T*)vnext, (T*)tnext, j, (const T*)h1, (const T*)h2, (T*)hcol_dev, C, (const T*)y,
+                       (const T*)t, tail_part);
     return check_launch(ctx, "cgs2_fused_tail");
+}
+
+int k_cgs2_check(lsa_ctx* ctx, hipStream_t stream, int64_t n, const lsa_mat* C, const void* y, const void* t, double* tail_part) {
+    hipLaunchKernelGGL((cgs_check_kernel<16>), dim3(k_cgs2_tail_parts(n)), dim3(kThreads), 0, stream, (int32_t)n, C->rp, C->ci, (const cplx*)C->val,
+                       (const cplx*)y, (const cplx*)t, tail_part);
+    return check_launch(ctx, "cgs2_check");
 }
 
 int k_cgs2_tail_checks(lsa_ctx* ctx, int nslots, int nparts, const double* tail_parts, double* checks) {
@@ -1480,21 +1565,14 @@
     return check_launch(ctx, "dcgs2_norm");
 }
 
-int k_dcgs2_tail(lsa_ctx* ctx, int64_t n, int j, const void* V, int64_t ldv, const void* y, void* work, const lsa_mat* M, const lsa_mat* C, void* t,
-                 double* tail_part, void* slot, int lds) {
+int k_dcgs2_tail(lsa_ctx* ctx, int64_t n, int j, const void* V, int64_t ldv, void* work, const lsa_mat* M, void* tnext, void* slot, int lds,
+                 const lsa_mat* C, const void* y, const void* t, double* tail_part) {
     const int blocks = (int)((n + 63) / 64);
     double* nrm_part = FusedWork(work, 16).nrm_part;
     const cplx* w = (const cplx*)V + (size_t)(j + 1) * (size_t)ldv;
     cplx* nout = (cplx*)slot + 2 * (size_t)lds + 2;
-    const int tparts = k_cgs2_tail_parts(n);
-    if (M->dtype == LSA_C128)
-        hipLaunchKernelGGL((cgs_tail_kernel<cplx, 16, true>), dim3(tparts), dim3(kThreads), 0, ctx->stream, (int32_t)n, C->rp, C->ci, (const cplx*)M->val,
-                           (const cplx*)C->val, w, (const cplx*)y, (const double*)nrm_part, blocks, (cplx*)nullptr, (cplx*)t, 0, (const cplx*)nullptr,
-                           (const cplx*)nullptr, nout, tail_part);
-    else
-        hipLaunchKernelGGL((cgs_tail_kernel<double, 16, true>), dim3(tparts), dim3(kThreads), 0, ctx->stream, (int32_t)n, C->rp, C->ci,
-                           (const double*)M->val, (const cplx*)C->val, w, (const cplx*)y, (const double*)nrm_part, blocks, (cplx*)nullptr, (cplx*)t, 0,
-                           (const cplx*)nullptr, (const cplx*)nullptr, nout, tail_part);
+    launch_tail<true>(ctx, n, M, w, (const double*)nrm_part, blocks, (cplx*)nullptr, (cplx*)tnext, 0, (const cplx*)nullptr, (const cplx*)nullptr, nout, C,
+                      (const cplx*)y, (const cplx*)t, tail_part);
     return check_launch(ctx, "dcgs2_tail");
 }
 
@@ -1533,9 +1611,11 @@
     memset(&a, 0, sizeof a);
     for (int z = 0; z < J; ++z) {
         if (M[z]->dtype != M[0]->dtype) return lsa_set_error(ctx, LSA_ERR_ARG, "k_dcgs2_tail_batch: real and complex M in one round (problem %d)", z);
+        a.mrp[z] = M[z]->rp;
+        a.mci[z] = M[z]->ci;
+        a.mval[z] = M[z]->val;
         a.rp[z] = C[z]->rp;
         a.ci[z] = C[z]->ci;
-        a.mval[z] = M[z]->val;
         a.cval[z] = (const cplx*)C[z]->val;
         a.w[z] = (const cplx*)V[z] + (size_t)(j[z] + 1) * (size_t)ldv;
         a.y[z] = (const cplx*)y[z];
diff --git a/lsa-fw_amd/csrc/core.hip b/lsa-fw_amd/csrc/core.hip
--- a/lsa-fw_amd/csrc/core.hip
+++ b/lsa-fw_amd/csrc/core.hip
@@ -239,6 +239,7 @@
     if (m->grp_start) (void)hipFree(m->grp_start);
     if (m->ci16) (void)hipFree(m->ci16);
     if (m->cbase) (void)hipFree(m->cbase);
+    if (m->compact) lsa_mat_destroy(m->compact);
     delete m;
 }
 
@@ -398,3 +399,67 @@
     *out = W;
     return LSA_OK;
 }
+
+int64_t csr_compact_host(int32_t n, const int32_t* rp, const int32_t* ci, const void* val, int dtype, int32_t* rp_out, int32_t* ci_out, void* val_out) {
+    const size_t es = dtype_size(dtype);
+    const double* v = (const double*)val;
+    int64_t q = 0;
+    rp_out[0] = 0;
+    for (int32_t r = 0; r < n; ++r) {
+        for (int32_t p = rp[r]; p < rp[r + 1]; ++p) {
+            const bool zero = dtype == LSA_C128 ? (v[2 * (size_t)p] == 0.0 && v[2 * (size_t)p + 1] == 0.0) : v[p] == 0.0;
+            if (zero) continue;
+            if (ci_out) ci_out[q] = ci[p];
+            if (val_out) memcpy((char*)val_out + (size_t)q * es, (const char*)val + (size_t)p * es, es);
+            ++q;
+        }
+        rp_out[r + 1] = (int32_t)q;
+    }
+    return q;
+}
+
+const lsa_mat* k_csr_compact(lsa_ctx* ctx, const lsa_mat* M) {
+    if (!M || M->compact_state < 0) return M;
+    if (M->compact_state > 0) return M->compact;
+    M->compact_state = -1;
+    const int32_t n = M->n;
+    if (M->row0 != 0 || n != M->ncols || !M->owns_values || M->nnz < 1 || M->nnz >= (int64_t)4 << 20 || (int64_t)M->h_rp.size() != (int64_t)n + 1 ||
+        (int64_t)M->h_ci.size() != M->nnz)
+        return M;
+    const size_t es = dtype_size(M->dtype);
+    std::vector<char> val((size_t)M->nnz * es);
+    if (hipMemcpyAsync(val.data(), M->val, val.size(), hipMemcpyDeviceToHost, ctx->stream) != hipSuccess || hipStreamSynchronize(ctx->stream) != hipSuccess) {
+        (void)hipGetLastError();
+        return M;
+    }
+    std::vector<int32_t> rp((size_t)n + 1);
+    const int64_t kept = csr_compact_host(n, M->h_rp.data(), M->h_ci.data(), val.data(), M->dtype, rp.data(), nullptr, nullptr);
+    if (4 * (M->nnz - kept) < M->nnz) return M;
+    std::vector<int32_t> ci((size_t)std::max<int64_t>(kept, 1));
+    std::vector<char> cval((size_t)std::max<int64_t>(kept, 1) * es);
+    (void)csr_compact_host(n, M->h_rp.data(), M->h_ci.data(), val.data(), M->dtype, rp.data(), ci.data(), cval.data());
+    lsa_mat* Mc = nullptr;
+    const std::string err = ctx->err;
+    if (csr_upload_impl(ctx, n, M->ncols, 0, kept, rp.data(), ci.data(), cval.data(), M->dtype, &Mc) != LSA_OK) {
+        ctx->err = err;
+        return M;
+    }
+    Mc->spmv_lanes = k_spmv_default_lanes(M);
+    Mc->compact_state = -1;
+    M->compact = Mc;
+    M->compact_state = 1;
+    return Mc;
+}
+
+extern "C" int64_t lsa_csr_compact_host(int32_t n, const int32_t* rowptr, const int32_t* col, const void* val, int dtype, int32_t* rowptr_out, int32_t* col_out,
+                                        void* val_out) {
+    if (n < 0 || !rowptr || !rowptr_out || (dtype != LSA_F64 && dtype != LSA_C128) || (rowptr[n] > 0 && (!col || !val))) return -1;
+    return csr_compact_host(n, rowptr, col, val, dtype, rowptr_out, col_out, val_out);
+}
+
+extern "C" int lsa_csr_compact(lsa_ctx* ctx, const lsa_mat* M, const lsa_mat** out, int64_t* nnz_out) {
+    if (!ctx || !M || !out) return lsa_set_error(ctx, LSA_ERR_ARG, "lsa_csr_compact: null argument");
+    *out = k_csr_compact(ctx, M);
+    if (nnz_out) *nnz_out = (*out)->nnz;
+    return LSA_OK;
+}
diff --git a/lsa-fw_amd/csrc/lsa_internal.h b/lsa-fw_amd/csrc/lsa_internal.h
--- a/lsa-fw_amd/csrc/lsa_internal.h
+++ b/lsa-fw_amd/csrc/lsa_internal.h
@@ -171,6 +171,9 @@
     mutable int32_t ngroups = 0;
     mutable int grp_state = 0;
     bool owns_extras = true;
+    mutable lsa_mat* compact = nullptr;
+    mutable int compact_state = 0;
+    int spmv_lanes = 0;
 };
 
 int lsa_set_error(lsa_ctx* ctx, int code, const char* fmt, ...);
@@ -242,6 +245,9 @@
 int k_transpose_index(lsa_ctx* ctx, const lsa_mat* A, const TransposeIndex** out);
 int k_spmv_transpose_batch(lsa_ctx* ctx, int32_t J, const lsa_mat* const* mats, int conj, int xdtype, const void* const* xs, void* const* ys);
 void spmv_share_extras(const lsa_mat* from, lsa_mat* to);
+int k_spmv_default_lanes(const lsa_mat* A);
+const lsa_mat* k_csr_compact(lsa_ctx* ctx, const lsa_mat* M);
+int64_t csr_compact_host(int32_t n, const int32_t* rp, const int32_t* ci, const void* val, int dtype, int32_t* rp_out, int32_t* ci_out, void* val_out);
 
 int k_spmm(lsa_ctx* ctx, const lsa_mat* A, int32_t ncols, const void* X, int64_t ldx, void* Y, int64_t ldy);
 int k_spmm_transpose(lsa_ctx* ctx, const lsa_mat* A, int conj, int32_t ncols, const void* X, int64_t ldx, void* Y, int64_t ldy);
@@ -269,14 +275,15 @@
 bool k_cgs2_tail_fits(lsa_ctx* ctx, int64_t n, int jmax, const lsa_mat* M, const lsa_mat* C);
 int k_cgs2_tail_parts(int64_t n);
 int k_cgs2_fused_tail(lsa_ctx* ctx, int64_t n, int j, const void* V, int64_t ldv, const void* y, void* w, void* vnext, void* hcol_dev, void* work,
-                      const lsa_mat* M, const lsa_mat* C, void* t, double* tail_part);
+                      const lsa_mat* M, void* tnext, const lsa_mat* C, const void* t, double* tail_part);
+int k_cgs2_check(lsa_ctx* ctx, hipStream_t stream, int64_t n, const lsa_mat* C, const void* y, const void* t, double* tail_part);
 int k_cgs2_tail_checks(lsa_ctx* ctx, int nslots, int nparts, const double* tail_parts, double* checks);
 bool k_dcgs2_fits(int64_t n, int ncv);
 int k_dcgs2_step(lsa_ctx* ctx, int64_t n, int j, void* V, int64_t ldv, const void* y, int first, void* slot, int lds, void* work,
                  const void* chk_b, const void* chk_z, double* chk_out);
 int k_dcgs2_norm(lsa_ctx* ctx, int64_t n, void* work, void* slot, int lds);
-int k_dcgs2_tail(lsa_ctx* ctx, int64_t n, int j, const void* V, int64_t ldv, const void* y, void* work, const lsa_mat* M, const lsa_mat* C, void* t,
-                 double* tail_part, void* slot, int lds);
+int k_dcgs2_tail(lsa_ctx* ctx, int64_t n, int j, const void* V, int64_t ldv, void* work, const lsa_mat* M, void* tnext, void* slot, int lds,
+                 const lsa_mat* C, const void* y, const void* t, double* tail_part);
 int k_dcgs2_step_batch(lsa_ctx* ctx, int J, int64_t n, const int32_t* j, void* const* V, int64_t ldv, const void* const* y, const int32_t* first,
                        void* const* slot, int lds, void* const* work);
 int k_dcgs2_tail_batch(lsa_ctx* ctx, int J, int64_t n, const int32_t* j, void* const* V, int64_t ldv, const void* const* y, void* const* work,
diff --git a/lsa-fw_amd/csrc/solver.hip b/lsa-fw_amd/csrc/solver.hip
--- a/lsa-fw_amd/csrc/solver.hip
+++ b/lsa-fw_amd/csrc/solver.hip
@@ -17,13 +17,15 @@
     bool tail;
     bool delayed;
     bool timing;
+    int check_aside;
     bool preapply;
 };
 const KrylovSwitches& krylov_switches() {
     static const KrylovSwitches sw = [] {
         const char* passes = getenv("LSA_KRYLOV_PASSES");
         return KrylovSwitches{env_flag("LSA_KRYLOV_FUSED", true), passes && atoi(passes) == 4, env_flag("LSA_KRYLOV_TAIL", true),
-                              env_flag("LSA_KRYLOV_DELAYED", true), getenv("LSA_KRYLOV_TIMING") != nullptr, env_flag("LSA_KRYLOV_PREAPPLY", true)};
+                              env_flag("LSA_KRYLOV_DELAYED", true), getenv("LSA_KRYLOV_TIMING") != nullptr, getenv("LSA_KRYLOV_CHECK_ASIDE") ? (env_flag("LSA_KRYLOV_CHECK_ASIDE", false) ? 1 : 0) : -1,
+                              env_flag("LSA_KRYLOV_PREAPPLY", true)};
     }();
     return sw;
 }
@@ -419,6 +421,7 @@
     double sigma[2] = {0.0, 0.0};
     lsa_mat *view_fac = nullptr, *view_mul = nullptr;
     const lsa_mat* M_whole = nullptr;
+    const lsa_mat* Mc = nullptr;
     lsa_op_options opts;
     GmresWork gw;
     bool gw_ready;
@@ -427,6 +430,8 @@
     bool refine = false;
     lsa_stats st;
 };
+
+static const lsa_mat* step_mul(const lsa_op* op) { return op->Mc && op->Kmul == op->M_whole && !op->adjoint ? op->Mc : op->Kmul; }
 
 static PcRef pc_of(const lsa_op* op) {
     PcRef pc;
@@ -458,6 +463,15 @@
     double* tail_parts = nullptr;
     int32_t tail_nparts = 0;
     int32_t t_for = -1;
+    static constexpr int kCheckRingMax = 8;
+    int32_t ring_n = 4;
+    void* ring_t[kCheckRingMax] = {};
+    void* ring_w[kCheckRingMax] = {};
+    int32_t ring = 0;
+    int32_t since_wait = 0;
+    hipEvent_t ev_tail = nullptr, ev_check = nullptr;
+    void* tbuf(int32_t i) const { return i == 0 ? op->t : ring_t[i]; }
+    void* wbuf(int32_t i) const { return i == 0 ? w : ring_w[i]; }
     bool pre_armed = false;
     int32_t pre_col = -1, pre_for = -1;
     const lsa_op* pre_op = nullptr;
@@ -475,7 +489,10 @@
 static void krylov_free(lsa_krylov* k) {
     for (void* p : {k->V, k->V2, k->w, k->qdev, k->Hdev, (void*)k->checks, (void*)k->imag2, k->xtmp, (void*)k->row_perm, k->w2, (void*)k->tail_parts})
         if (p) (void)hipFree(p);
-    for (hipEvent_t e : k->ev_read)
+    for (int i = 1; i < lsa_krylov::kCheckRingMax; ++i)
+        for (void* p : {k->ring_t[i], k->ring_w[i]})
+            if (p) (void)hipFree(p);
+    for (hipEvent_t e : {k->ev_read[0], k->ev_read[1], k->ev_tail, k->ev_check})
         if (e) (void)hipEventDestroy(e);
     k->ow.release();
     delete k;
@@ -582,6 +599,10 @@
         op->Kfac = C;
         op->Kmul = M;
         op->M_whole = M;
+        if (M && mode == 0 && !sharded && !tree && ctx->nranks == 1) {
+            const lsa_mat* Mc = k_csr_compact(ctx, M);
+            op->Mc = Mc != M ? Mc : nullptr;
+        }
         bool shard_rows = false;
         if (tree) {
             const char* e = getenv("LSA_DIST_SPMV");
@@ -1002,9 +1023,11 @@
     p.pipelined = k->pipeline && (k->batch > 1 || p.orth == Orth::dcgs2) && op->Kfac && op->nd && !op->pc &&
                   !(ctx->nranks > 1 && (!op->nd_dist || ctx->host_gather));
     p.tail = p.pipelined && sw.tail && sw.fused && op->Kmul && !op->adjoint && !op->keep && !op->refine && op->n == k->n &&
-             k_cgs2_tail_fits(ctx, k->n, k->ncv, op->Kmul, op->Kfac);
+             k_cgs2_tail_fits(ctx, k->n, k->ncv, step_mul(op), op->Kfac);
     return p;
 }
+
+static hipStream_t check_stream(const lsa_krylov* k) { return krylov_switches().check_aside == 1 && k->op->nd ? k->op->nd->side : nullptr; }
 
 static int krylov_enqueue_step(lsa_ctx* ctx, lsa_krylov* k, const StepPlan& plan, int32_t j, int32_t slot, bool first) {
     lsa_op* op = k->op;
@@ -1019,23 +1042,44 @@
     const bool ahead = plan.tail && dcgs2 && first && k->pre_for == j && k->pre_op == op;
     k->drop_preapply();
     if (plan.tail) {
-        if (!ahead && k->t_for != j) LSA_CHECK(spmv_global(ctx, op->Kmul, dtype, vj, op->t, false));
+        const lsa_mat* Mm = step_mul(op);
+        const hipStream_t side = check_stream(k);
+        const bool rides = krylov_switches().check_aside < 0;
+        const int32_t nxt = rides ? k->ring : (k->ring + 1) % k->ring_n;
+        void *t = k->tbuf(k->ring), *y = k->wbuf(k->ring), *tnext = k->tbuf(nxt);
+        if (!ahead && k->t_for != j) LSA_CHECK(spmv_global(ctx, Mm, dtype, vj, t, false));
         k->t_for = -1;
-        if (!ahead) LSA_CHECK(pc_global(ctx, pc_of(op), op->Kfac->row0, op->n, dtype, op->t, k->w));
+        if (!ahead) LSA_CHECK(pc_global(ctx, pc_of(op), op->Kfac->row0, op->n, dtype, t, y));
         double* parts = k->tail_parts + (size_t)slot * 2 * (size_t)k->tail_nparts;
+        const bool wait = side && k->since_wait >= k->ring_n - 1;
         if (dcgs2) {
-            LSA_CHECK(k_dcgs2_step(ctx, k->n, j, k->V, k->n, k->w, first ? 1 : 0, sl, k->ncv, k->ow.fused, nullptr, nullptr, nullptr));
-            LSA_CHECK(k_dcgs2_tail(ctx, k->n, j, k->V, k->n, k->w, k->ow.fused, op->Kmul, op->Kfac, op->t, parts, sl, k->ncv));
+            LSA_CHECK(k_dcgs2_step(ctx, k->n, j, k->V, k->n, y, first ? 1 : 0, sl, k->ncv, k->ow.fused, nullptr, nullptr, nullptr));
+            if (wait) LSA_HIP_CHECK(ctx, hipStreamWaitEvent(ctx->stream, k->ev_check, 0));
+            LSA_CHECK(k_dcgs2_tail(ctx, k->n, j, k->V, k->n, k->ow.fused, Mm, tnext, sl, k->ncv, rides ? op->Kfac : nullptr, rides ? y : nullptr,
+                                   rides ? t : nullptr, rides ? parts : nullptr));
         } else {
-            LSA_CHECK(k_cgs2_fused_tail(ctx, k->n, j + 1, k->V, k->n, k->w, k->w2, vn, sl, k->ow.fused, op->Kmul, op->Kfac, op->t, parts));
-        }
+            if (wait) LSA_HIP_CHECK(ctx, hipStreamWaitEvent(ctx->stream, k->ev_check, 0));
+            LSA_CHECK(k_cgs2_fused_tail(ctx, k->n, j + 1, k->V, k->n, y, k->w2, vn, sl, k->ow.fused, Mm, tnext, rides ? op->Kfac : nullptr, rides ? t : nullptr,
+                                        rides ? parts : nullptr));
+        }
+        if (wait) k->since_wait = 0;
+        if (side) {
+            LSA_HIP_CHECK(ctx, hipEventRecord(k->ev_tail, ctx->stream));
+            LSA_HIP_CHECK(ctx, hipStreamWaitEvent(side, k->ev_tail, 0));
+            LSA_CHECK(k_cgs2_check(ctx, side, k->n, op->Kfac, y, t, parts));
+            LSA_HIP_CHECK(ctx, hipEventRecord(k->ev_check, side));
+            ++k->since_wait;
+        } else if (!rides) {
+            LSA_CHECK(k_cgs2_check(ctx, ctx->stream, k->n, op->Kfac, y, t, parts));
+        }
+        k->ring = nxt;
         k->t_for = j + 1;
         return LSA_OK;
     }
     k->t_for = -1;
     const void* rhs = vj;
     if (op->Kmul) {
-        LSA_CHECK(spmv_global(ctx, op->Kmul, dtype, vj, op->t, op->adjoint));
+        LSA_CHECK(spmv_global(ctx, step_mul(op), dtype, vj, op->t, op->adjoint));
         rhs = op->t;
     }
     LSA_CHECK(direct_solve_enqueue(ctx, op, dtype, rhs, k->w, op->gw.z, op->gw.w, op->refine, chk));
@@ -1111,10 +1155,26 @@
         LSA_CHECK(op->gw.alloc(ctx, op->n, std::max(1, std::min({op->opts.ksp_restart, op->opts.ksp_maxit, 40})), LSA_C128));
         op->gw_ready = true;
     }
+    if (plan.tail && krylov_switches().check_aside == 1 && op->nd && !op->nd->side) {
+        lsa_ndlu* f = op->nd;
+        int lo_pri = 0, hi_pri = 0;
+        LSA_HIP_CHECK(ctx, hipDeviceGetStreamPriorityRange(&lo_pri, &hi_pri));
+        LSA_HIP_CHECK(ctx, hipStreamCreateWithPriority(&f->side, hipStreamNonBlocking, hi_pri));
+        if (!f->ev_panel) LSA_HIP_CHECK(ctx, hipEventCreateWithFlags(&f->ev_panel, hipEventDisableTiming));
+        if (!f->ev_pivots) LSA_HIP_CHECK(ctx, hipEventCreateWithFlags(&f->ev_pivots, hipEventDisableTiming));
+    }
     if (plan.tail && !k->tail_parts) {
         const int32_t slots = 2 * std::max(k->batch, 1);
         k->tail_nparts = k_cgs2_tail_parts(k->n);
         LSA_HIP_ALLOC(ctx, hipMalloc(&k->w2, (size_t)k->n * 16));
+        if (const char* e = getenv("LSA_KRYLOV_CHECK_RING")) k->ring_n = std::max(2, std::min(atoi(e), lsa_krylov::kCheckRingMax));
+        if (krylov_switches().check_aside < 0) k->ring_n = 1;
+        for (int i = 1; i < k->ring_n; ++i) {
+            LSA_HIP_ALLOC(ctx, hipMalloc(&k->ring_t[i], (size_t)k->n * 16));
+            LSA_HIP_ALLOC(ctx, hipMalloc(&k->ring_w[i], (size_t)k->n * 16));
+        }
+        for (hipEvent_t* e : {&k->ev_tail, &k->ev_check})
+            if (!*e) LSA_HIP_CHECK(ctx, hipEventCreateWithFlags(e, hipEventDisableTiming));
         LSA_HIP_ALLOC(ctx, hipMalloc((void**)&k->tail_parts, (size_t)slots * 2 * (size_t)k->tail_nparts * sizeof(double)));
     }
     return LSA_OK;
@@ -1129,7 +1189,8 @@
     LSA_CHECK(pipelined_prepare(ctx, k, plan));
     lsa_op* op = k->op;
     k->t_for = -1;
-    LSA_CHECK(spmv_global(ctx, op->Kmul, LSA_C128, (char*)k->V + (size_t)m * (size_t)k->n * 16, op->t, false));
+    k->ring = 0;
+    LSA_CHECK(spmv_global(ctx, step_mul(op), LSA_C128, (char*)k->V + (size_t)m * (size_t)k->n * 16, op->t, false));
     LSA_CHECK(pc_global(ctx, pc_of(op), op->Kfac->row0, op->n, LSA_C128, op->t, k->w));
     k->pre_col = m;
     k->pre_op = op;
@@ -1188,6 +1249,8 @@
     const bool ahead = krylov_switches().preapply;
     if (ahead) LSA_CHECK(k->ensure_events(ctx));
     k->t_for = -1;
+    k->ring = 0;
+    k->since_wait = 0;
     struct Queued {
         int32_t j, nb, set;
     };
@@ -1215,6 +1278,10 @@
             }
         }
         double* chk = k->checks + 2 * (size_t)set * (size_t)slots;
+        if (p.tail && check_stream(k)) {
+            LSA_HIP_CHECK(ctx, hipStreamWaitEvent(ctx->stream, k->ev_check, 0));
+            k->since_wait = 0;
+        }
         if (p.tail) LSA_CHECK(k_cgs2_tail_checks(ctx, nb, k->tail_nparts, k->tail_parts + (size_t)set * (size_t)slots * 2 * (size_t)k->tail_nparts, chk));
         LSA_HIP_CHECK(ctx, hipMemcpyAsync(host_of(set), slot_of(set), (size_t)nb * colb, hipMemcpyDeviceToHost, ctx->stream));
         LSA_HIP_CHECK(ctx, hipMemcpyAsync(host_of(set) + (size_t)slots * colb, chk, (size_t)nb * 2 * sizeof(double), hipMemcpyDeviceToHost, ctx->stream));
@@ -1235,6 +1302,7 @@
         k->t_for = -1;
         k->drop_preapply();
         LSA_HIP_CHECK(ctx, hipStreamSynchronize(ctx->stream));
+        if (const hipStream_t side = check_stream(k)) LSA_HIP_CHECK(ctx, hipStreamSynchronize(side));
         return LSA_OK;
     };
     Queued cur{0, 0, 0}, next{0, 0, 0};
@@ -1323,6 +1391,32 @@
     k->pre_for = -1;
     if (breakdown) *breakdown = bd;
     k->op->st.seconds_solve += now_s() - t0;
+    return rc;
+}
+
+int lsa_krylov_tail_probe(lsa_ctx* ctx, const lsa_mat* M, const lsa_mat* C, const lsa_vec* w, const lsa_vec* y, const lsa_vec* t, lsa_vec* tnext,
+                          double pairs[2]) {
+    if (!ctx || !M || !C || !w || !y || !t || !tnext || !pairs) return lsa_set_error(ctx, LSA_ERR_ARG, "lsa_krylov_tail_probe: null argument");
+    const int64_t n = M->n;
+    for (const lsa_vec* v : {w, y, t, (const lsa_vec*)tnext})
+        if (v->n != n || v->dtype != LSA_C128) return lsa_set_error(ctx, LSA_ERR_ARG, "lsa_krylov_tail_probe: complex vectors of M's %lld rows", (long long)n);
+    if (tnext->d == t->d || tnext->d == w->d) return lsa_set_error(ctx, LSA_ERR_ARG, "lsa_krylov_tail_probe: tnext aliases an input");
+    const lsa_mat* Mm = k_csr_compact(ctx, M);
+    if (!k_cgs2_tail_fits(ctx, n, 1, Mm, C)) return lsa_set_error(ctx, LSA_ERR_ARG, "lsa_krylov_tail_probe: the matrices are outside the tail form");
+    const int nparts = k_cgs2_tail_parts(n);
+    const size_t wb = k_cgs2_fused_work_bytes(ctx, n, 1), sb = 8 * 16, pb = (size_t)(2 * nparts + 2) * sizeof(double);
+    char* buf = nullptr;
+    LSA_HIP_ALLOC(ctx, hipMalloc((void**)&buf, wb + sb + pb));
+    double* parts = (double*)(buf + wb + sb);
+    int rc = hipMemsetAsync(buf, 0, wb + sb + pb, ctx->stream) == hipSuccess ? (int)LSA_OK : lsa_set_error(ctx, LSA_ERR_HIP, "lsa_krylov_tail_probe: memset failed");
+    if (rc == LSA_OK) rc = k_dcgs2_tail(ctx, n, -1, w->d, n, buf, Mm, tnext->d, buf + wb, 1, nullptr, nullptr, nullptr, nullptr);
+    if (rc == LSA_OK) rc = k_cgs2_check(ctx, ctx->stream, n, C, y->d, t->d, parts);
+    if (rc == LSA_OK) rc = k_cgs2_tail_checks(ctx, 1, nparts, parts, parts + 2 * (size_t)nparts);
+    if (rc == LSA_OK && (hipMemcpyAsync(pairs, parts + 2 * (size_t)nparts, 2 * sizeof(double), hipMemcpyDeviceToHost, ctx->stream) != hipSuccess ||
+                         hipStreamSynchronize(ctx->stream) != hipSuccess))
+        rc = lsa_set_error(ctx, LSA_ERR_HIP, "lsa_krylov_tail_probe: read-back failed");
+    (void)hipStreamSynchronize(ctx->stream);
+    (void)hipFree(buf);
     return rc;
 }
 
@@ -1421,7 +1515,7 @@
             const StepPlan plan = step_plan(ctx, k);
             bool in = plan.pipelined && plan.orth == Orth::dcgs2 && plan.tail;
             if (in && lead >= 0)
-                in = nd_batch_compatible(ks[lead]->op->nd, k->op->nd) && ks[lead]->op->Kmul->dtype == k->op->Kmul->dtype;
+                in = nd_batch_compatible(ks[lead]->op->nd, k->op->nd) && step_mul(ks[lead]->op)->dtype == step_mul(k->op)->dtype;
             if (!in) {
                 m.lock = false;
                 continue;
@@ -1455,14 +1549,14 @@
                 const int32_t j = mem[z].c.j + s;
                 const size_t cell = (size_t)s * (size_t)J + (size_t)z;
                 if (k->t_for != j) {
-                    rc = spmv_global(ctx, op->Kmul, LSA_C128, (char*)k->V + (size_t)j * (size_t)k->n * 16, op->t, false);
+                    rc = spmv_global(ctx, step_mul(op), LSA_C128, (char*)k->V + (size_t)j * (size_t)k->n * 16, op->t, false);
                     ++products;
                 }
                 k->t_for = -1;
                 jr[R] = j;
                 fr[R] = (s == 0 && !mem[z].c.pending) ? 1 : 0;
                 nd[R] = op->nd;
-                Mr[R] = op->Kmul;
+                Mr[R] = step_mul(op);
                 Cr[R] = op->Kfac;
                 rhs[R] = op->t;
                 xr[R] = k->w;
diff --git a/lsa-fw_amd/csrc/spmv.hip b/lsa-fw_amd/csrc/spmv.hip
--- a/lsa-fw_amd/csrc/spmv.hip
+++ b/lsa-fw_amd/csrc/spmv.hip
@@ -275,6 +275,7 @@
 
 static int spmv_lanes_per_row(const lsa_mat* A, int variant) {
     int lpr = variant & 0xff;
+    if (lpr == 0) lpr = A->spmv_lanes;
     if (lpr == 0) {
         const double mean = A->n > 0 ? (double)A->nnz / (double)A->n : 0.0;
         lpr = mean <= 6.0 ? 4 : mean <= 12.0 ? 8 : mean <= 48.0 ? 16 : mean <= 96.0 ? 32 : 64;
@@ -374,6 +375,8 @@
     to->ci16_state = from->ci16_state > 0 ? 1 : -1;
     to->owns_extras = false;
 }
+
+int k_spmv_default_lanes(const lsa_mat* A) { return spmv_lanes_per_row(A, 0); }
 
 int k_spmv_plain_subwave_lanes(const lsa_mat* A) {
     const int variant = spmv_variant();
diff --git a/lsa-fw_amd/lsa_hip/__init__.py b/lsa-fw_amd/lsa_hip/__init__.py
--- a/lsa-fw_amd/lsa_hip/__init__.py
+++ b/lsa-fw_amd/lsa_hip/__init__.py
@@ -200,6 +200,8 @@
     "lsa_mat_download_values": (ctypes.c_int, [_P, _P, _P]),
     "lsa_csr_axpby": (ctypes.c_int, [_P, _P, _P, _DBL * 2, _DBL * 2, ctypes.c_int, _PP]),
     "lsa_csr_window": (ctypes.c_int, [_P, _P, _P, _P, _PP]),
+    "lsa_csr_compact": (ctypes.c_int, [_P, _P, _PP, ctypes.POINTER(_I64)]),
+    "lsa_csr_compact_host": (_I64, [_I32, _P, _P, _P, ctypes.c_int, _P, _P, _P]),
     "lsa_spmv": (ctypes.c_int, [_P, _P, _P, _P]),
     "lsa_spmv_transpose": (ctypes.c_int, [_P, _P, ctypes.c_int, _P, _P]),
     "lsa_spmv_transpose_batch": (ctypes.c_int, [_P, _I32, _PP, ctypes.c_int, _PP, _PP]),
@@ -265,6 +267,7 @@
     "lsa_krylov_set_start": (ctypes.c_int, [_P, _P, _P]),
     "lsa_krylov_inject": (ctypes.c_int, [_P, _P, _I32, _P]),
     "lsa_krylov_extend": (ctypes.c_int, [_P, _P, _I32, _I32, _P, _I32, ctypes.POINTER(_I32)]),
+    "lsa_krylov_tail_probe": (ctypes.c_int, [_P, _P, _P, _P, _P, _P, _P, _DBL * 2]),
     "lsa_krylov_restart": (ctypes.c_int, [_P, _P, _I32, _I32, _P, _I32]),
     "lsa_krylov_ritz_vectors": (ctypes.c_int, [_P, _P, _I32, _I32, _P, _I32, ctypes.c_int, _P]),
     "lsa_krylov_imag_norms": (ctypes.c_int, [_P, _I32, _P]),
@@ -605,6 +608,13 @@
         self.ctx.check(self.ctx._lib.lsa_mat_download_values(self.ctx.handle, self.handle, _ptr(out)))
         return out
 
+    def compacted(self) -> "CsrMatrix":
+        h, nnz = ctypes.c_void_p(), _I64(0)
+        self.ctx.check(self.ctx._lib.lsa_csr_compact(self.ctx.handle, self.handle, ctypes.byref(h), ctypes.byref(nnz)))
+        if h.value == (self.handle.value if isinstance(self.handle, ctypes.c_void_p) else self.handle):
+            return self
+        return _BorrowedCsrMatrix(self.ctx, h, self.shape, nnz.value, self.dtype, keep=(self,))
+
     def matvec(self, x: DeviceVector, y: DeviceVector) -> None:
         self.ctx.check(self.ctx._lib.lsa_spmv(self.ctx.handle, self.handle, x.handle, y.handle))
 
@@ -648,6 +658,37 @@
         if getattr(self, "handle", None) and getattr(self.ctx, "handle", None):
             self.ctx._lib.lsa_mat_destroy(self.handle)
             self.handle = None
+
+
+class _BorrowedCsrMatrix(CsrMatrix):
+
+    def __del__(self):
+        self.handle = None
+
+
+def krylov_tail_probe(ctx: Context, M: CsrMatrix, C: CsrMatrix, w: DeviceVector, y: DeviceVector, t: DeviceVector, tnext: DeviceVector):
+    pairs = (_DBL * 2)()
+    ctx.check(ctx._lib.lsa_krylov_tail_probe(ctx.handle, M.handle, C.handle, w.handle, y.handle, t.handle, tnext.handle, pairs))
+    return float(pairs[0]), float(pairs[1])
+
+
+def csr_compact_host(A):
+    import scipy.sparse as sp
+
+    A = sp.csr_matrix(A)
+    dt = np.complex128 if A.dtype.kind == "c" else np.float64
+    rp = np.ascontiguousarray(A.indptr, dtype=np.int32)
+    ci = np.ascontiguousarray(A.indices, dtype=np.int32)
+    val = np.ascontiguousarray(A.data, dtype=dt)
+    n = A.shape[0]
+    lib = load_library()
+    rp_out = np.empty(n + 1, dtype=np.int32)
+    kept = lib.lsa_csr_compact_host(n, _ptr(rp), _ptr(ci), _ptr(val), _dtype_code(dt), _ptr(rp_out), None, None)
+    if kept < 0:
+        raise ValueError("lsa_csr_compact_host: bad argument")
+    ci_out, val_out = np.empty(max(kept, 1), dtype=np.int32), np.empty(max(kept, 1), dtype=dt)
+    lib.lsa_csr_compact_host(n, _ptr(rp), _ptr(ci), _ptr(val), _dtype_code(dt), _ptr(rp_out), _ptr(ci_out), _ptr(val_out))
+    return rp_out, ci_out[:kept], val_out[:kept]
 
 
 class Ilu:
```
